# clinfo/kGCN

Hardware: AMD Instinct MI355X
Metric: graphs/sec GraphConv fwd+bwd, 32-node mol graphs x64 feat (higher is better)
Workload: dtype f32

## Files before the change

include/kgcn_hip.h:

```cpp
#ifndef KGCN_HIP_H_
#define KGCN_HIP_H_

#include <stdint.h>

#ifdef __cplusplus
extern "C" {
#endif

#define KGCN_HIP_ABI_VERSION 2

#define KGCN_PAD_COL 32

#define KGCN_ROW_PAD_COMPACT 0x104
#define KGCN_CSR_UNIT_VALUES 1


typedef struct kgcn_csr_batch {
  int32_t num_graphs;
  int32_t rows;
  int32_t cols;
  int32_t max_nnz_per_graph;
  int32_t row_pad;
  int32_t reserved_;
  int64_t nnz;
// ... 72 lines not shown
                        int64_t workspace_bytes, void* stream);

int kgcn_graph_maxpool_fwd_f32(const kgcn_csr_batch* a, const float* x, int32_t d, float* out,
                               float beta, void* stream);
int64_t kgcn_graph_maxpool_bwd_workspace_bytes(int32_t num_graphs, int32_t rows, int32_t d);
int kgcn_graph_maxpool_bwd_f32(const kgcn_csr_batch* a, const kgcn_csr_batch* at, const float* x,
                               const float* dout_grad, int32_t d, float* dx, float beta,
                               void* workspace, int64_t workspace_bytes, void* stream);

int64_t kgcn_gat_workspace_bytes(int32_t num_graphs, int32_t n_nodes, int32_t d);
int kgcn_gat_fwd_f32(const kgcn_csr_batch* a, const float* x, int32_t d, const float* weight_a, float* out,
                     float beta, void* workspace, int64_t workspace_bytes, void* stream);
int kgcn_gat_bwd_f32(const kgcn_csr_batch* a, const kgcn_csr_batch* at, const float* x, int32_t d,
                     const float* weight_a, const float* dout_grad, float* dx, float beta, float* dweight_a,
                     void* workspace, int64_t workspace_bytes, void* stream);

int64_t kgcn_gram_workspace_bytes(int32_t d);
int kgcn_gram_fwd_f32(const float* x, int32_t num_graphs, int32_t n_nodes, int32_t d, const float* w, float* out,
                      void* stream);
int kgcn_gram_bwd_f32(const float* x, int32_t num_graphs, int32_t n_nodes, int32_t d, const float* w,
                      const float* dout_grad, float* dx, float beta, float* dw, void* workspace,
                      int64_t workspace_bytes, void* stream);

int kgcn_graph_gather_fwd_f32(const float* x, int64_t batch, int32_t n_nodes, int32_t d,
                              float* out, void* stream);
int kgcn_graph_gather_fwd_ld_f32(const float* x, int64_t batch, int32_t n_nodes, int32_t d, float* out, int64_t out_ld,
                                 void* stream);
int kgcn_graph_gather_bwd_f32(const float* dout_grad, int64_t batch, int32_t n_nodes, int32_t d,
                              float* dx, void* stream);

int kgcn_graph_gather_bwd_add_f32(const float* dout_grad, const float* dx_in, int64_t batch, int32_t n_nodes, int32_t d,
                                  float* dx, void* stream);

int64_t kgcn_dot_workspace_bytes(int64_t n);
int kgcn_dot_f32(const float* a, const float* b, int64_t n, float* out, void* workspace,
                 int64_t workspace_bytes, void* stream);

#define KGCN_ACT_NONE 0
#define KGCN_ACT_SIGMOID 1
#define KGCN_ACT_RELU 2
#define KGCN_ACT_TANH 3
int kgcn_bconv_act_f32(const kgcn_csr_batch* a_ch, int32_t num_channels, const float* rhs, int64_t rhs_ld,
                       int64_t rhs_graph_stride, int64_t rhs_channel_stride, int32_t d, float* out, int64_t out_ld,
                       int64_t out_graph_stride, int32_t act, void* stream);

int kgcn_bconv_fanout_f32(const kgcn_csr_batch* at_ch, int32_t num_channels, const float* grad, const float* act_out, int64_t ld,
                          int64_t graph_stride, int32_t d, int32_t act, float* out, int64_t out_ld, int64_t out_graph_stride,
                          int64_t out_channel_stride, void* stream);
int kgcn_bspmm_dact_f32(const kgcn_csr_batch* a, const float* grad, const float* act_out, int64_t ld,
                        int64_t graph_stride, int32_t d, int32_t act, float* out, int64_t out_ld,
                        int64_t out_graph_stride, float beta, void* stream);
int kgcn_dense_fwd_act_f32(const float* x, int64_t m, int32_t din, int64_t x_ld, const float* w, int64_t w_ld,
                           int32_t trans_w, const float* bias, float* y, int32_t dout, int64_t y_ld, int32_t act,
                           void* stream);
int64_t kgcn_dense_fwd_workspace_bytes(int32_t din, int32_t dout);
int kgcn_dense_fwd_ws_f32(const float* x, int64_t m, int32_t din, int64_t x_ld, const float* w, int64_t w_ld,
                          int32_t trans_w, const float* bias, float* y, int32_t dout, int64_t y_ld, int32_t act,
                          void* workspace, int64_t workspace_bytes, void* stream);
#define KGCN_WTABLE_MAX_JOBS 16
typedef struct kgcn_wtable_job {
  const float* w;
  int64_t w_ld;
  int32_t trans_w, k, n;
  int32_t k_w;
  void* table;
  const float* extra_row;
} kgcn_wtable_job;
int kgcn_wtable_split_multi(const kgcn_wtable_job* jobs, int32_t num_jobs, void* stream);
int kgcn_dense_fwd_tab_f32(const float* x, int64_t m, int32_t din, int64_t x_ld, const float* w, int64_t w_ld,
                           int32_t trans_w, const float* bias, float* y, int32_t dout, int64_t y_ld, int32_t act,
                           const void* table, int64_t table_bytes, void* stream);
int kgcn_dense_dx_dact_f32(const float* grad, const float* act_out, int64_t m, int32_t dout, int64_t ld, const float* w,
                           int64_t w_ld, int32_t din, float* dx, int64_t dx_ld, int32_t act, float* dpre,
                           void* workspace, int64_t workspace_bytes, void* stream);
int kgcn_dense_dx_dact_tab_f32(const float* grad, const float* act_out, int64_t m, int32_t dout, int64_t ld, const float* w,
                               int64_t w_ld, int32_t din, float* dx, int64_t dx_ld, int32_t act, float* dpre, const void* table,
                               int64_t table_bytes, void* stream);
int kgcn_dense_dx_dact_gather_supported(int64_t m, int32_t din, int32_t dout);
int kgcn_dense_dx_dact_gather_f32(const float* grad, const float* pooled_grad, int64_t pooled_ld, int32_t n_nodes,
                                  const float* act_out, int64_t m, int32_t dout, int64_t ld, const float* w, int64_t w_ld,
                                  int32_t din, float* dx, int64_t dx_ld, int32_t act, float* dpre, void* table,
                                  int64_t table_bytes, int32_t table_ready, void* stream);
int kgcn_dense_bwd_supported(int64_t m, int32_t din, int32_t dout);
int kgcn_dense_bwd_f32(const float* grad, const float* pooled_grad, int64_t pooled_ld, int32_t n_nodes, const float* act_out,
                       int32_t act, int64_t ld, const float* x, int64_t x_ld, int64_t m, int32_t din, int32_t dout,
                       const float* w, int64_t w_ld, float* dx, int64_t dx_ld, float* dw, float* dbias, void* table,
                       int64_t table_bytes, int32_t table_ready, void* workspace, int64_t workspace_bytes, void* stream);
int kgcn_dense_bwd_dot_f32(const float* grad, const float* act_out, int32_t act, int64_t ld, const float* x, int64_t x_ld, int64_t m,
                           int32_t din, int32_t dout, const float* w, int64_t w_ld, const float* dotx, int64_t dotx_ld, float* dw,
                           float* dbias, float* dot_out, void* table, int64_t table_bytes, int32_t table_ready, void* workspace,
                           int64_t workspace_bytes, void* stream);
int kgcn_dense_dx_dact_dot_supported(int64_t m, int32_t din, int32_t dout);
int64_t kgcn_dense_dx_dact_dot_workspace_bytes(int64_t m, int32_t din);
int kgcn_dense_dx_dact_dot_f32(const float* grad, const float* act_out, int64_t m, int32_t dout, int64_t ld, const float* w,
                               int64_t w_ld, int32_t din, const float* dotx, int64_t dotx_ld, int32_t act, float* dpre,
                               void* table, int64_t table_bytes, int32_t table_ready, float* dot_out, void* workspace,
                               int64_t workspace_bytes, void* stream);
int kgcn_act_fwd_f32(const float* x, int64_t n, int32_t act, float* y, void* stream);
int kgcn_act_bwd_f32(const float* act_out, const float* grad, int64_t n, int32_t act, float* dpre, void* stream);

int64_t kgcn_graph_bn_workspace_bytes(int32_t d);
int kgcn_graph_bn_stats_f32(const float* x, int64_t graphs, int32_t n_nodes, int32_t d, const int32_t* enabled,
                            float* mean, float* var, void* workspace, int64_t workspace_bytes, void* stream);
int kgcn_graph_bn_apply_f32(const float* x, int64_t graphs, int32_t n_nodes, int32_t d, const int32_t* enabled,
                            const float* mean, const float* var, const float* gamma, const float* beta, float eps,
                            float* y, void* stream);
int kgcn_graph_bn_bwd_f32(const float* x, const float* grad, int64_t graphs, int32_t n_nodes, int32_t d,
                          const int32_t* enabled, const float* mean, const float* var, const float* gamma, float eps,
                          int32_t training, float* dx, float* dgamma, float* dbeta, void* workspace,
                          int64_t workspace_bytes, void* stream);

int kgcn_graph_bn_apply_act_f32(const float* x, int64_t graphs, int32_t n_nodes, int32_t d, const int32_t* enabled,
                                const float* mean, const float* var, const float* gamma, const float* beta, float eps,
                                int32_t act, float* y, void* stream);
int kgcn_graph_bn_bwd_dact_f32(const float* x, const float* grad, const float* act_out, int32_t act, int64_t graphs,
                               int32_t n_nodes, int32_t d, const int32_t* enabled, const float* mean, const float* var,
                               const float* gamma, float eps, int32_t training, float* dx, float* dgamma, float* dbeta,
                               void* workspace, int64_t workspace_bytes, void* stream);

int64_t kgcn_coo_pack_workspace_bytes(int64_t nnz, int32_t num_graphs, int32_t rows, int32_t cols);
int kgcn_coo_pack_f32(const int32_t* graph, const int32_t* row, const int32_t* col, const float* val, int64_t nnz,
                      int32_t num_graphs, int32_t rows, int32_t cols, int32_t transposed, int32_t* rowptr_out,
                      void* cv_out, int32_t* perm_out, int32_t* stats_out, void* workspace, int64_t workspace_bytes,
                      void* stream);
int64_t kgcn_csr_pad4_workspace_bytes(int32_t num_graphs, int32_t rows);
int kgcn_csr_pad4(const kgcn_csr_batch* a, int32_t* rowptr4_out, void* cv4_out, int64_t cv4_capacity,
                  int32_t* slots_out, int32_t* graph_ptr_out, int32_t* stats_out, void* workspace,
                  int64_t workspace_bytes, void* stream);
int64_t kgcn_compact_values_offset(int64_t nnz);
int64_t kgcn_compact_cv_words(int64_t nnz, int32_t with_values);
int kgcn_csr_compact4(const kgcn_csr_batch* a4, void* cv_out, int with_values, void* slots_out, int32_t* stats_out,
                      void* stream);
int kgcn_graphconv_fused_reads_compact(int32_t backward, int32_t num_graphs, int32_t n_nodes, int32_t din, int32_t dout,
                                       int32_t max_nnz_per_graph, int32_t with_dx);

int64_t kgcn_ragged_workspace_bytes(int32_t num_sel);
int kgcn_ragged_plan(const kgcn_csr_batch* src, const int32_t* sizes, const int32_t* sel, int32_t num_sel,
                     int32_t* graph_ptr, int32_t* entry_ptr, void* workspace, int64_t workspace_bytes, void* stream);
int kgcn_ragged_compact_csr(const kgcn_csr_batch* src, const int32_t* sel, int32_t num_sel, const int32_t* graph_ptr,
                            const int32_t* entry_ptr, int32_t capacity_rows, int32_t* dst_rowptr, int32_t* dst_cv,
                            int64_t dst_cv_capacity, int32_t* status, void* stream);
int kgcn_ragged_compact_csr_pair(const kgcn_csr_batch* src, const kgcn_csr_batch* src_t, const int32_t* sel, int32_t num_sel,
                                 const int32_t* graph_ptr, const int32_t* entry_ptr, int32_t capacity_rows, int32_t* dst_rowptr,
                                 int32_t* dst_cv, int64_t dst_cv_capacity, int32_t* dst_t_rowptr, int32_t* dst_t_cv,
                                 int64_t dst_t_cv_capacity, int32_t* status, void* stream);
#define KGCN_RAGGED_BLOCK_ROWS 32
int32_t kgcn_ragged_block_rows(void);
int32_t kgcn_ragged_num_blocks(int32_t capacity_rows);
int kgcn_ragged_blocks(const int32_t* graph_ptr, int32_t num_sel, int32_t capacity_rows, int32_t* block_ptr, void* stream);
int kgcn_ragged_compact_rows_f32(const float* src, const int32_t* sel, int32_t num_sel, int32_t n_nodes, int32_t d,
                                 const int32_t* graph_ptr, int32_t capacity_rows, float* dst, void* stream);
int kgcn_ragged_compact_rows_aug_f32(const float* src, const int32_t* sel, int32_t num_sel, int32_t n_nodes, int32_t d,
                                     const int32_t* graph_ptr, int32_t capacity_rows, float* dst, int32_t dst_ld, void* stream);
int kgcn_ragged_expand_rows_f32(const float* src, int32_t num_graphs, int32_t n_nodes, int32_t d,
                                const int32_t* graph_ptr, int32_t fill_row, float* dst, void* stream);
int kgcn_ragged_gather_fwd_f32(const float* x, const int32_t* graph_ptr, int64_t batch, int32_t n_nodes, int32_t d,
                               int32_t pad_row, float* out, void* stream);
int64_t kgcn_ragged_gather_bwd_workspace_bytes(int32_t d);
int kgcn_ragged_gather_bwd_f32(const float* dout_grad, const int32_t* graph_ptr, int64_t batch, int32_t n_nodes, int32_t d,
                               int32_t pad_row, int32_t capacity_rows, float* dx, void* workspace, int64_t workspace_bytes,
                               void* stream);

int64_t kgcn_loss_workspace_bytes(int64_t batch);
int kgcn_masked_sigmoid_ce_f32(const float* logits, const float* labels, const float* mask, const float* mask_label,
                               int64_t batch, int32_t tasks, int32_t weighted, float pos_weight,
                               const float* pos_weight_per_task, float* cost, float* dlogits, float* sums, void* workspace,
                               int64_t workspace_bytes, void* stream);
int kgcn_masked_softmax_ce_f32(const float* logits, const float* labels, const float* mask, int64_t batch, int32_t classes,
                               float* cost, float* dlogits, float* sums, void* workspace, int64_t workspace_bytes,
                               void* stream);
int kgcn_sparse_softmax_ce_f32(const float* logits, const int64_t* label_idx, const float* mask, int64_t batch,
                               int32_t classes, float* cost, float* dlogits, float* sums, void* workspace,
                               int64_t workspace_bytes, void* stream);
int kgcn_loss_grad_f32(const float* dlogits, const float* g_opt, const float* g_sum, int64_t batch, int64_t n, float* out,
                       void* stream);
int kgcn_adam_tf_f32(float* params, const float* grads, float* m, float* v, int64_t n, float lr, float beta1, float beta2,
                     float eps, int64_t* step_counter, void* stream);
#define KGCN_ADAM_MAX_SEGMENTS 32
typedef struct kgcn_adam_segment {
  const float* grad;
  int64_t offset, numel;
} kgcn_adam_segment;
int kgcn_adam_tf_multi_f32(float* params, float* m, float* v, int64_t n, const kgcn_adam_segment* segments, int32_t num_segments,
                           float lr, float beta1, float beta2, float eps, int64_t* step_counter, void* stream);

int kgcn_augment_ones_f32(const float* x, int64_t m, int32_t din, int64_t x_ld, float* out, int64_t out_ld, void* stream);
int kgcn_augment_ones_bwd_f32(const float* dout_grad, int64_t m, int32_t din, int64_t g_ld, float* dx, int64_t dx_ld,
                              void* stream);

#define KGCN_STACK_MAX_LAYERS 8
typedef struct kgcn_stack_layer {
  int32_t kind, act, din, dout;
  const float* w;
  const float* b;
  const float* mean;
  const float* var;
  float eps;
  int32_t route;
} kgcn_stack_layer;
int kgcn_gcn_stack_supported(int32_t n_nodes, int32_t max_nnz_per_graph, const kgcn_stack_layer* layers, int32_t num_layers);
int64_t kgcn_gcn_stack_param_floats(const kgcn_stack_layer* layers, int32_t num_layers);
int kgcn_gcn_stack_fwd_f32(const kgcn_csr_batch* a, const float* x, const int32_t* enabled, const kgcn_stack_layer* layers,
                           int32_t num_layers, float* const* layer_out, float* pooled, void* stream);
int64_t kgcn_gcn_stack_bwd_workspace_bytes(int32_t num_graphs, const kgcn_stack_layer* layers, int32_t num_layers);
int kgcn_gcn_stack_bwd_f32(const kgcn_csr_batch* at, const float* x, const int32_t* enabled, const kgcn_stack_layer* layers,
                           int32_t num_layers, float* const* layer_out, const float* dlast, int32_t gather, float* dx,
                           float* dparams, void* workspace, int64_t workspace_bytes, void* stream);

int kgcn_reduce_defer(int32_t on);
int kgcn_reduce_pending(void);
int kgcn_reduce_flush(void* stream);

int kgcn_dense_mfma_products(int32_t kind, int64_t m, int32_t din, int32_t dout);

enum {
  KGCN_SPMM_NONE = 0,
  KGCN_SPMM_TILE = 1,
  KGCN_SPMM_TILE_DOT = 2,
  KGCN_SPMM_SLICES = 3,
  KGCN_SPMM_BLOCK = 4,
  KGCN_SPMM_ROWS = 5,
  KGCN_SPMM_GATHER = 6,
  KGCN_SPMM_BCONV_LOOP = 7,
  KGCN_SPMM_BCONV_FANOUT = 8
};
#define KGCN_SPMM_DACT 1
#define KGCN_SPMM_SELF_SCALE 2
#define KGCN_SPMM_DOT 4
#define KGCN_SPMM_FANOUT 8
typedef struct kgcn_spmm_route {
  int32_t kernel;
  int32_t template_args[4];
  int32_t ds, slices;
  int32_t workgroup;
  int64_t grid;
  int64_t lds_bytes;
} kgcn_spmm_route;
int kgcn_spmm_route_query(const kgcn_csr_batch* a_ch, int32_t num_channels, int32_t d, int64_t rhs_ld, int64_t rhs_graph_stride,
                          int64_t channel_stride, int64_t out_ld, int64_t out_graph_stride, int32_t align_bytes, int32_t flags,
                          kgcn_spmm_route* route);

#define KGCN_COPY2D_MAX_JOBS 16
typedef struct kgcn_copy2d_job {
  const float* src;
  float* dst;
  int64_t rows, cols, src_ld, dst_ld;
} kgcn_copy2d_job;
int kgcn_copy2d_multi_f32(const kgcn_copy2d_job* jobs, int32_t num_jobs, void* stream);

int kgcn_hbm_probe(int32_t mix, const void* a, const void* a2, void* b, int64_t bytes, void* stream);

int kgcn_dense_wgrad_dact_supported(int32_t din, int32_t dout);
int kgcn_dense_wgrad_dact_f32(const float* x, int64_t x_ld, const float* dy, const float* act_out, int64_t dy_ld, int32_t act,
                              int64_t m, int32_t din, int32_t dout, float* dw, float* dbias, void* workspace,
                              int64_t workspace_bytes, void* stream);

int64_t kgcn_gin_aggregate_bwd_workspace_bytes(int32_t num_graphs, int32_t n_nodes, int32_t d);
int kgcn_gin_aggregate_bwd_f32(const kgcn_csr_batch* at_ch, int32_t num_channels, const float* grad, int32_t d,
                               const float* eps, const float* x, float* dx, float* deps, void* workspace,
                               int64_t workspace_bytes, void* stream);

#define KGCN_VAE_MAX_NODES 128
#define KGCN_VAE_MAX_CHANNELS 8
#define KGCN_VAE_MAX_DIM 64
int kgcn_philox4x64_raw(uint64_t seed, const int64_t* step, int64_t num_blocks, uint64_t* out, void* stream);
int kgcn_normal_f32(uint64_t seed, const int64_t* step, int64_t n, float* out, void* stream);
int kgcn_vae_sample_fwd_f32(const float* m_pre, const float* s_pre, int32_t num_graphs, int32_t n_nodes, int32_t d, int32_t ld,
                            const float* eps, uint64_t seed, const int64_t* step, float* z, float* kl, void* stream);
int kgcn_vae_sample_bwd_f32(const float* m_pre, const float* s_pre, int32_t num_graphs, int32_t n_nodes, int32_t d, int32_t ld,
                            const float* eps, uint64_t seed, const int64_t* step, const float* const* dz, int32_t num_dz,
                            const float* dkl, float* dm_pre, float* ds_pre, void* stream);
int64_t kgcn_vae_recon_workspace_bytes(int32_t num_graphs, int32_t num_channels, int32_t d);
int kgcn_vae_recon_fwd_f32(const kgcn_csr_batch* adj_ch, int32_t num_channels, const float* const* y, const float* const* w,
                           int32_t d, const float* feat_logits, const float* feat_target, int32_t f, const float* mask,
                           const float* kl, float* per_graph, float* sums, void* stream);
int kgcn_vae_recon_bwd_f32(const kgcn_csr_batch* adj_ch, int32_t num_channels, const float* const* y, const float* const* w,
                           int32_t d, const float* feat_logits, const float* feat_target, int32_t f, const float* mask,
                           const float* g_opt, const float* g_sum, float* const* dy, float* const* dw, float* dfeat,
                           float* dkl, void* workspace, int64_t workspace_bytes, void* stream);

#define KGCN_SEQ_MAX_EMBED 32
#define KGCN_SEQ_MAX_FILTERS 64
#define KGCN_SEQ_MAX_KERNEL 8
#define KGCN_SEQ_MAX_POOL 8
#define KGCN_SEQ_MAX_UNITS 64
#define KGCN_SEQ_MAX_LSTM_INPUT 64
#define KGCN_SEQ_MAX_SYMBOLS 1024
#define KGCN_SEQ_MAX_LENGTH 8192
#define KGCN_SEQ_ACT_HARD_SIGMOID 0
#define KGCN_SEQ_ACT_SIGMOID 1
int64_t kgcn_seq_convpool_workspace_bytes(int32_t batch, int32_t length, int32_t symbols, int32_t embed_dim, int32_t kernel_size,
                                          int32_t filters, int32_t pool);
int kgcn_seq_convpool_fwd_f32(const int32_t* tokens, int32_t batch, int32_t length, const float* table, int32_t symbols,
                              int32_t embed_dim, const float* w, const float* bias, int32_t kernel_size, int32_t filters,
// ... 100 lines not shown
```

kgcn_amd/_lib.py:

```python
import ctypes
import os

_HERE = os.path.dirname(os.path.abspath(__file__))
DEV_ENV_VARS = ("KGCN_HIP_LIB", "KGCN_GIN_JOIN", "KGCN_GIN_DOT")
LIB_PATH = os.environ.get("KGCN_HIP_LIB") or os.path.join(_HERE, "csrc", "libkgcn_hip.so")


def active_overrides():
    return {k: os.environ[k] for k in DEV_ENV_VARS if os.environ.get(k)}


if active_overrides():
    import warnings
    warnings.warn("kgcn_amd: development overrides active: %r (KGCN_HIP_LIB swaps the native library, the others "
                  "change kernel routing)" % (active_overrides(),), RuntimeWarning, stacklevel=2)

c_f32p = ctypes.c_void_p
c_i32p = ctypes.c_void_p
c_i64 = ctypes.c_int64
c_i32 = ctypes.c_int32


ABI_VERSION = 2

# ... 117 lines not shown
    "kgcn_gram_fwd_f32": (ctypes.c_int, [c_f32p, c_i32, c_i32, c_i32, c_f32p, c_f32p, ctypes.c_void_p]),
    "kgcn_gram_bwd_f32": (ctypes.c_int, [c_f32p, c_i32, c_i32, c_i32, c_f32p, c_f32p, c_f32p, ctypes.c_float, c_f32p,
                                         ctypes.c_void_p, c_i64, ctypes.c_void_p]),
    "kgcn_graph_gather_fwd_f32": (ctypes.c_int, [c_f32p, c_i64, c_i32, c_i32, c_f32p,
                                                 ctypes.c_void_p]),
    "kgcn_graph_gather_fwd_ld_f32": (ctypes.c_int, [c_f32p, c_i64, c_i32, c_i32, c_f32p, c_i64, ctypes.c_void_p]),
    "kgcn_graph_gather_bwd_f32": (ctypes.c_int, [c_f32p, c_i64, c_i32, c_i32, c_f32p,
                                                 ctypes.c_void_p]),
    "kgcn_bconv_fanout_f32": (ctypes.c_int, [_CSRP, c_i32, c_f32p, c_f32p, c_i64, c_i64, c_i32, c_i32, c_f32p, c_i64, c_i64, c_i64,
                                             ctypes.c_void_p]),
    "kgcn_bconv_act_f32": (ctypes.c_int, [_CSRP, c_i32, c_f32p, c_i64, c_i64, c_i64, c_i32, c_f32p, c_i64, c_i64, c_i32,
                                          ctypes.c_void_p]),
    "kgcn_bspmm_dact_f32": (ctypes.c_int, [_CSRP, c_f32p, c_f32p, c_i64, c_i64, c_i32, c_i32, c_f32p, c_i64, c_i64,
                                           ctypes.c_float, ctypes.c_void_p]),
    "kgcn_dense_fwd_act_f32": (ctypes.c_int, [c_f32p, c_i64, c_i32, c_i64, c_f32p, c_i64, c_i32, c_f32p, c_f32p, c_i32,
                                              c_i64, c_i32, ctypes.c_void_p]),
    "kgcn_dense_fwd_workspace_bytes": (c_i64, [c_i32, c_i32]),
    "kgcn_dense_fwd_ws_f32": (ctypes.c_int, [c_f32p, c_i64, c_i32, c_i64, c_f32p, c_i64, c_i32, c_f32p, c_f32p, c_i32,
                                             c_i64, c_i32, ctypes.c_void_p, c_i64, ctypes.c_void_p]),
    "kgcn_dense_dx_dact_f32": (ctypes.c_int, [c_f32p, c_f32p, c_i64, c_i32, c_i64, c_f32p, c_i64, c_i32, c_f32p, c_i64, c_i32,
                                              c_f32p, ctypes.c_void_p, c_i64, ctypes.c_void_p]),
    "kgcn_dense_dx_dact_tab_f32": (ctypes.c_int, [c_f32p, c_f32p, c_i64, c_i32, c_i64, c_f32p, c_i64, c_i32, c_f32p, c_i64,
                                                  c_i32, c_f32p, ctypes.c_void_p, c_i64, ctypes.c_void_p]),
    "kgcn_dense_dx_dact_gather_supported": (ctypes.c_int, [c_i64, c_i32, c_i32]),
    "kgcn_dense_dx_dact_gather_f32": (ctypes.c_int, [c_f32p, c_f32p, c_i64, c_i32, c_f32p, c_i64, c_i32, c_i64, c_f32p, c_i64, c_i32,
                                                     c_f32p, c_i64, c_i32, c_f32p, ctypes.c_void_p, c_i64, c_i32, ctypes.c_void_p]),
    "kgcn_dense_dx_dact_dot_supported": (ctypes.c_int, [c_i64, c_i32, c_i32]),
    "kgcn_dense_dx_dact_dot_workspace_bytes": (c_i64, [c_i64, c_i32]),
    "kgcn_dense_dx_dact_dot_f32": (ctypes.c_int, [c_f32p, c_f32p, c_i64, c_i32, c_i64, c_f32p, c_i64, c_i32, c_f32p, c_i64, c_i32,
                                                  c_f32p, ctypes.c_void_p, c_i64, c_i32, c_f32p, ctypes.c_void_p, c_i64,
                                                  ctypes.c_void_p]),
    "kgcn_dense_fwd_tab_f32": (ctypes.c_int, [c_f32p, c_i64, c_i32, c_i64, c_f32p, c_i64, c_i32, c_f32p, c_f32p, c_i32,
                                              c_i64, c_i32, ctypes.c_void_p, c_i64, ctypes.c_void_p]),
    "kgcn_wtable_split_multi": (ctypes.c_int, [ctypes.c_void_p, c_i32, ctypes.c_void_p]),
    "kgcn_act_fwd_f32": (ctypes.c_int, [c_f32p, c_i64, c_i32, c_f32p, ctypes.c_void_p]),
    "kgcn_act_bwd_f32": (ctypes.c_int, [c_f32p, c_f32p, c_i64, c_i32, c_f32p, ctypes.c_void_p]),
    "kgcn_graph_bn_workspace_bytes": (c_i64, [c_i32]),
    "kgcn_graph_bn_stats_f32": (ctypes.c_int, [c_f32p, c_i64, c_i32, c_i32, c_i32p, c_f32p, c_f32p, ctypes.c_void_p, c_i64,
                                               ctypes.c_void_p]),
    "kgcn_graph_bn_apply_f32": (ctypes.c_int, [c_f32p, c_i64, c_i32, c_i32, c_i32p, c_f32p, c_f32p, c_f32p, c_f32p,
                                               ctypes.c_float, c_f32p, ctypes.c_void_p]),
    "kgcn_graph_bn_bwd_f32": (ctypes.c_int, [c_f32p, c_f32p, c_i64, c_i32, c_i32, c_i32p, c_f32p, c_f32p, c_f32p,
                                             ctypes.c_float, c_i32, c_f32p, c_f32p, c_f32p, ctypes.c_void_p, c_i64,
                                             ctypes.c_void_p]),
    "kgcn_coo_pack_workspace_bytes": (c_i64, [c_i64, c_i32, c_i32, c_i32]),
    "kgcn_coo_pack_f32": (ctypes.c_int, [c_i32p, c_i32p, c_i32p, c_f32p, c_i64, c_i32, c_i32, c_i32, c_i32, c_i32p,
                                         ctypes.c_void_p, c_i32p, c_i32p, ctypes.c_void_p, c_i64, ctypes.c_void_p]),
    "kgcn_compact_values_offset": (c_i64, [c_i64]),
    "kgcn_compact_cv_words": (c_i64, [c_i64, c_i32]),
    "kgcn_csr_compact4": (ctypes.c_int, [_CSRP, ctypes.c_void_p, ctypes.c_int, ctypes.c_void_p, c_i32p, ctypes.c_void_p]),
    "kgcn_graphconv_fused_reads_compact": (ctypes.c_int, [c_i32, c_i32, c_i32, c_i32, c_i32, c_i32, c_i32]),
    "kgcn_csr_pad4_workspace_bytes": (c_i64, [c_i32, c_i32]),
    "kgcn_csr_pad4": (ctypes.c_int, [_CSRP, c_i32p, ctypes.c_void_p, c_i64, c_i32p, c_i32p, c_i32p, ctypes.c_void_p,
                                     c_i64, ctypes.c_void_p]),
    "kgcn_graph_bn_apply_act_f32": (ctypes.c_int, [c_f32p, c_i64, c_i32, c_i32, c_i32p, c_f32p, c_f32p, c_f32p, c_f32p,
                                                   ctypes.c_float, c_i32, c_f32p, ctypes.c_void_p]),
    "kgcn_graph_bn_bwd_dact_f32": (ctypes.c_int, [c_f32p, c_f32p, c_f32p, c_i32, c_i64, c_i32, c_i32, c_i32p, c_f32p, c_f32p,
                                                  c_f32p, ctypes.c_float, c_i32, c_f32p, c_f32p, c_f32p, ctypes.c_void_p,
                                                  c_i64, ctypes.c_void_p]),
    "kgcn_ragged_workspace_bytes": (c_i64, [c_i32]),
    "kgcn_ragged_plan": (ctypes.c_int, [_CSRP, c_i32p, c_i32p, c_i32, c_i32p, c_i32p, ctypes.c_void_p, c_i64,
                                        ctypes.c_void_p]),
    "kgcn_ragged_compact_csr": (ctypes.c_int, [_CSRP, c_i32p, c_i32, c_i32p, c_i32p, c_i32, c_i32p, c_i32p, c_i64, c_i32p,
                                               ctypes.c_void_p]),
    "kgcn_ragged_compact_csr_pair": (ctypes.c_int, [_CSRP, _CSRP, c_i32p, c_i32, c_i32p, c_i32p, c_i32, c_i32p, c_i32p, c_i64, c_i32p,
                                                    c_i32p, c_i64, c_i32p, ctypes.c_void_p]),
    "kgcn_ragged_block_rows": (c_i32, []),
    "kgcn_ragged_num_blocks": (c_i32, [c_i32]),
    "kgcn_ragged_blocks": (ctypes.c_int, [c_i32p, c_i32, c_i32, c_i32p, ctypes.c_void_p]),
    "kgcn_ragged_compact_rows_f32": (ctypes.c_int, [c_f32p, c_i32p, c_i32, c_i32, c_i32, c_i32p, c_i32, c_f32p,
                                                    ctypes.c_void_p]),
    "kgcn_ragged_compact_rows_aug_f32": (ctypes.c_int, [c_f32p, c_i32p, c_i32, c_i32, c_i32, c_i32p, c_i32, c_f32p, c_i32,
                                                        ctypes.c_void_p]),
    "kgcn_ragged_expand_rows_f32": (ctypes.c_int, [c_f32p, c_i32, c_i32, c_i32, c_i32p, c_i32, c_f32p, ctypes.c_void_p]),
    "kgcn_ragged_gather_fwd_f32": (ctypes.c_int, [c_f32p, c_i32p, c_i64, c_i32, c_i32, c_i32, c_f32p, ctypes.c_void_p]),
    "kgcn_ragged_gather_bwd_workspace_bytes": (c_i64, [c_i32]),
    "kgcn_ragged_gather_bwd_f32": (ctypes.c_int, [c_f32p, c_i32p, c_i64, c_i32, c_i32, c_i32, c_i32, c_f32p,
                                                  ctypes.c_void_p, c_i64, ctypes.c_void_p]),
    "kgcn_dense_mfma_products": (ctypes.c_int, [c_i32, c_i64, c_i32, c_i32]),
    "kgcn_spmm_route_query": (ctypes.c_int, [_CSRP, c_i32, c_i32, c_i64, c_i64, c_i64, c_i64, c_i64, c_i32, c_i32,
                                             ctypes.POINTER(SpmmRoute)]),
    "kgcn_copy2d_multi_f32": (ctypes.c_int, [ctypes.c_void_p, c_i32, ctypes.c_void_p]),
    "kgcn_hbm_probe": (ctypes.c_int, [c_i32, ctypes.c_void_p, ctypes.c_void_p, ctypes.c_void_p, c_i64, ctypes.c_void_p]),
    "kgcn_reduce_defer": (ctypes.c_int, [c_i32]),
    "kgcn_reduce_pending": (ctypes.c_int, []),
    "kgcn_reduce_flush": (ctypes.c_int, [ctypes.c_void_p]),
    "kgcn_loss_workspace_bytes": (c_i64, [c_i64]),
    "kgcn_masked_sigmoid_ce_f32": (ctypes.c_int, [c_f32p, c_f32p, c_f32p, c_f32p, c_i64, c_i32, c_i32, ctypes.c_float, c_f32p,
                                                  c_f32p, c_f32p, c_f32p, ctypes.c_void_p, c_i64, ctypes.c_void_p]),
    "kgcn_masked_softmax_ce_f32": (ctypes.c_int, [c_f32p, c_f32p, c_f32p, c_i64, c_i32, c_f32p, c_f32p, c_f32p,
                                                  ctypes.c_void_p, c_i64, ctypes.c_void_p]),
    "kgcn_sparse_softmax_ce_f32": (ctypes.c_int, [c_f32p, ctypes.c_void_p, c_f32p, c_i64, c_i32, c_f32p, c_f32p, c_f32p,
                                                  ctypes.c_void_p, c_i64, ctypes.c_void_p]),
    "kgcn_adam_tf_multi_f32": (ctypes.c_int, [c_f32p, c_f32p, c_f32p, c_i64, ctypes.c_void_p, c_i32, ctypes.c_float,
                                              ctypes.c_float, ctypes.c_float, ctypes.c_float, ctypes.c_void_p, ctypes.c_void_p]),
    "kgcn_loss_grad_f32": (ctypes.c_int, [c_f32p, c_f32p, c_f32p, c_i64, c_i64, c_f32p, ctypes.c_void_p]),
    "kgcn_adam_tf_f32": (ctypes.c_int, [c_f32p, c_f32p, c_f32p, c_f32p, c_i64, ctypes.c_float, ctypes.c_float,
                                        ctypes.c_float, ctypes.c_float, ctypes.c_void_p, ctypes.c_void_p]),
    "kgcn_augment_ones_f32": (ctypes.c_int, [c_f32p, c_i64, c_i32, c_i64, c_f32p, c_i64, ctypes.c_void_p]),
    "kgcn_augment_ones_bwd_f32": (ctypes.c_int, [c_f32p, c_i64, c_i32, c_i64, c_f32p, c_i64, ctypes.c_void_p]),
    "kgcn_gcn_stack_supported": (ctypes.c_int, [c_i32, c_i32, _STKP, c_i32]),
    "kgcn_gcn_stack_param_floats": (c_i64, [_STKP, c_i32]),
    "kgcn_gcn_stack_fwd_f32": (ctypes.c_int, [_CSRP, c_f32p, c_i32p, _STKP, c_i32, _PTRP, c_f32p, ctypes.c_void_p]),
    "kgcn_gcn_stack_bwd_workspace_bytes": (c_i64, [c_i32, _STKP, c_i32]),
    "kgcn_gcn_stack_bwd_f32": (ctypes.c_int, [_CSRP, c_f32p, c_i32p, _STKP, c_i32, _PTRP, c_f32p, c_i32, c_f32p, c_f32p,
                                              ctypes.c_void_p, c_i64, ctypes.c_void_p]),
    "kgcn_dense_wgrad_dact_supported": (ctypes.c_int, [c_i32, c_i32]),
    "kgcn_dense_wgrad_dact_f32": (ctypes.c_int, [c_f32p, c_i64, c_f32p, c_f32p, c_i64, c_i32, c_i64, c_i32, c_i32, c_f32p,
                                                 c_f32p, ctypes.c_void_p, c_i64, ctypes.c_void_p]),
    "kgcn_gin_aggregate_bwd_workspace_bytes": (c_i64, [c_i32, c_i32, c_i32]),
    "kgcn_gin_aggregate_bwd_f32": (ctypes.c_int, [_CSRP, c_i32, c_f32p, c_i32, c_f32p, c_f32p, c_f32p, c_f32p, ctypes.c_void_p,
                                                  c_i64, ctypes.c_void_p]),
    "kgcn_philox4x64_raw": (ctypes.c_int, [ctypes.c_uint64, ctypes.c_void_p, c_i64, ctypes.c_void_p, ctypes.c_void_p]),
    "kgcn_normal_f32": (ctypes.c_int, [ctypes.c_uint64, ctypes.c_void_p, c_i64, c_f32p, ctypes.c_void_p]),
    "kgcn_vae_sample_fwd_f32": (ctypes.c_int, [c_f32p, c_f32p, c_i32, c_i32, c_i32, c_i32, c_f32p, ctypes.c_uint64, ctypes.c_void_p,
                                               c_f32p, c_f32p, ctypes.c_void_p]),
    "kgcn_vae_sample_bwd_f32": (ctypes.c_int, [c_f32p, c_f32p, c_i32, c_i32, c_i32, c_i32, c_f32p, ctypes.c_uint64, ctypes.c_void_p,
                                               _PTRP, c_i32, c_f32p, c_f32p, c_f32p, ctypes.c_void_p]),
    "kgcn_vae_recon_workspace_bytes": (c_i64, [c_i32, c_i32, c_i32]),
    "kgcn_vae_recon_fwd_f32": (ctypes.c_int, [_CSRP, c_i32, _PTRP, _PTRP, c_i32, c_f32p, c_f32p, c_i32, c_f32p, c_f32p, c_f32p,
                                              c_f32p, ctypes.c_void_p]),
    "kgcn_vae_recon_bwd_f32": (ctypes.c_int, [_CSRP, c_i32, _PTRP, _PTRP, c_i32, c_f32p, c_f32p, c_i32, c_f32p, c_f32p, c_f32p,
                                              _PTRP, _PTRP, c_f32p, c_f32p, ctypes.c_void_p, c_i64, ctypes.c_void_p]),
    "kgcn_seq_convpool_workspace_bytes": (c_i64, [c_i32, c_i32, c_i32, c_i32, c_i32, c_i32, c_i32]),
    "kgcn_seq_convpool_fwd_f32": (ctypes.c_int, [ctypes.c_void_p, c_i32, c_i32, c_f32p, c_i32, c_i32, c_f32p, c_f32p, c_i32, c_i32,
                                                 c_i32, c_f32p, ctypes.c_void_p, ctypes.c_void_p]),
    "kgcn_seq_convpool_bwd_f32": (ctypes.c_int, [ctypes.c_void_p, c_i32, c_i32, c_f32p, c_i32, c_i32, c_f32p, c_i32, c_i32, c_i32,
                                                 c_f32p, ctypes.c_void_p, c_f32p, c_f32p, c_f32p, ctypes.c_void_p, c_i64,
                                                 ctypes.c_void_p]),
    "kgcn_seq_convpool_scaled_fwd_f32": (ctypes.c_int, [ctypes.c_void_p, c_i32, c_i32, c_f32p, c_i32, c_f32p, c_i32, c_i32, c_f32p,
                                                        c_f32p, c_i32, c_i32, c_i32, c_f32p, ctypes.c_void_p, ctypes.c_void_p]),
    "kgcn_seq_convpool_perturbed_fwd_f32": (ctypes.c_int, [ctypes.c_void_p, c_i32, c_i32, c_f32p, c_f32p, c_i32p, c_i32p, ctypes.c_uint64,
                                                           c_i32, c_f32p, c_i32, c_i32, c_f32p, c_f32p, c_i32, c_i32, c_i32, c_f32p,
                                                           ctypes.c_void_p, ctypes.c_void_p]),
    "kgcn_ig_perturb_rows_f32": (ctypes.c_int, [c_f32p, c_i64, c_i32, c_i32, c_i32, c_f32p, c_f32p, c_i32p, c_i32p, ctypes.c_uint32,
                                                ctypes.c_uint64, c_f32p, ctypes.c_void_p]),
    "kgcn_ig_perturb_values_f32": (ctypes.c_int, [c_i32p, c_i32, c_i32, c_i64, c_i32, c_f32p, c_f32p, c_f32p, c_i32p, c_i32p,
                                                  ctypes.c_uint32, ctypes.c_uint64, c_f32p, ctypes.c_void_p]),
    "kgcn_seq_convpool_input_grad_f32": (ctypes.c_int, [ctypes.c_void_p, c_i32, c_i32, c_i32, c_f32p, c_i32, c_i32, c_f32p, c_i32,
                                                        c_i32, c_i32, c_f32p, ctypes.c_void_p, c_f32p, c_i32, c_f32p,
                                                        ctypes.c_void_p]),
    "kgcn_seq_lstm_stash_floats": (c_i64, [c_i32, c_i32, c_i32]),
    "kgcn_seq_lstm_workspace_bytes": (c_i64, [c_i32, c_i32, c_i32, c_i32]),
    "kgcn_seq_lstm_fwd_f32": (ctypes.c_int, [c_f32p, c_i32, c_i32, c_i32, c_f32p, c_f32p, c_f32p, c_i32, c_i32, c_f32p, c_i64, c_f32p,
                                             ctypes.c_void_p]),
    "kgcn_seq_lstm_bwd_f32": (ctypes.c_int, [c_f32p, c_i32, c_i32, c_i32, c_f32p, c_f32p, c_f32p, c_i32, c_i32, c_f32p, c_i64, c_f32p,
                                             c_f32p, c_f32p, c_f32p, c_f32p, ctypes.c_void_p, c_i64, ctypes.c_void_p]),
    "kgcn_conv1d_pool_workspace_bytes": (c_i64, [c_i32, c_i32, c_i32, c_i32, c_i32, c_i32]),
    "kgcn_conv1d_pool_fwd_f32": (ctypes.c_int, [c_f32p, c_i32p, c_f32p, c_i32, c_i32, c_i32, c_i32, c_f32p, c_f32p, c_i32, c_i32,
                                                c_i32, c_i32, c_f32p, ctypes.c_void_p, ctypes.c_void_p]),
    "kgcn_conv1d_pool_bwd_f32": (ctypes.c_int, [c_f32p, c_i32p, c_f32p, c_i32, c_i32, c_i32, c_i32, c_f32p, c_i32, c_i32, c_i32,
                                                c_i32, c_f32p, ctypes.c_void_p, c_f32p, c_f32p, c_f32p, c_f32p, ctypes.c_void_p,
                                                c_i64, ctypes.c_void_p]),
    "kgcn_embedding_grad_f32": (ctypes.c_int, [c_i32p, c_i32, c_i32, c_f32p, c_i32, c_i32, c_f32p, ctypes.c_void_p]),
    "kgcn_linkpred_workspace_bytes": (c_i64, [c_i64, c_i32, c_i32, c_i32, c_i32]),
    "kgcn_linkpred_fwd_f32": (ctypes.c_int, [c_f32p, c_i64, c_i32, c_f32p, c_i32, c_i32, c_i32p, c_i32p, c_i64, c_i32, c_i32p, c_i32,
                                             ctypes.c_uint64, ctypes.c_void_p, c_i32p, c_f32p, c_f32p, c_f32p, ctypes.c_void_p]),
    "kgcn_linkpred_bwd_f32": (ctypes.c_int, [c_f32p, c_i64, c_i32, c_f32p, c_i32, c_i32, c_i32p, c_f32p, c_f32p, c_f32p, c_i32,
                                             c_f32p, c_f32p, c_f32p, c_f32p, ctypes.c_void_p, c_i64, ctypes.c_void_p]),
    "kgcn_kg_ig_f32": (ctypes.c_int, [c_i32p, c_i32p, c_f32p, c_i64, c_i32, c_i32, c_f32p, c_f32p, c_f32p, c_f32p, c_f32p, c_f32p,
                                      c_f32p, c_f32p, c_i32, c_i32p, c_i32, c_i32, c_i32, c_f32p, c_f32p, c_f32p, ctypes.c_void_p]),
    "kgcn_pair_rank_workspace_bytes": (c_i64, [c_i32, c_i32, c_i64, c_i64]),
    "kgcn_pair_rank_select_f32": (ctypes.c_int, [c_f32p, c_i32, c_i32, c_f32p, c_i64, ctypes.c_void_p, ctypes.c_void_p, c_i64,
                                                 ctypes.c_void_p]),
    "kgcn_pair_rank_emit_f32": (ctypes.c_int, [c_f32p, c_i32, c_i32, c_f32p, c_i64, ctypes.c_void_p, c_i64, c_f32p, c_i32p, c_i32p,
                                               ctypes.c_void_p, c_i64, ctypes.c_void_p]),
    "kgcn_pair_rank_table_i32": (ctypes.c_int, [c_f32p, c_i32p, c_i32p, c_i64, ctypes.c_void_p, c_i64, ctypes.c_void_p, c_i64,
                                                ctypes.POINTER(c_i64), c_i32, ctypes.c_void_p, ctypes.c_void_p, ctypes.c_void_p,
                                                ctypes.c_void_p, ctypes.c_void_p, ctypes.c_void_p, ctypes.c_void_p, c_i64,
                                                ctypes.c_void_p]),
    "kgcn_graph_gather_bwd_ld_f32": (ctypes.c_int, [c_f32p, c_i64, c_i64, c_i32, c_i32, c_f32p, ctypes.c_void_p]),
    "kgcn_graph_gather_bwd_add_f32": (ctypes.c_int, [c_f32p, c_f32p, c_i64, c_i32, c_i32, c_f32p, ctypes.c_void_p]),
    "kgcn_dot_workspace_bytes": (c_i64, [c_i64]),
    "kgcn_dot_f32": (ctypes.c_int, [c_f32p, c_f32p, c_i64, c_f32p, ctypes.c_void_p, c_i64,
                                    ctypes.c_void_p]),
}


# ... 63 lines not shown
```

kgcn_amd/csrc/dense.hip:

```cpp
#include <atomic>
#include <mutex>

#include "dense_kernels.h"

namespace kgcn {

constexpr int BM = 128;
constexpr int BN = 64;
constexpr int BK = 32;
constexpr int XS_LD = BK + 4;

__global__ __launch_bounds__(256) void dense_fwd_kernel(
    const float* __restrict__ x, long m, int din, long x_ld, const float* __restrict__ w,
    long w_ld, int trans_w, const float* __restrict__ bias, float* __restrict__ y, int dout,
    long y_ld, int act) {
  __shared__ __attribute__((aligned(16))) float Xs[BM * XS_LD];
  __shared__ __attribute__((aligned(16))) float Ws[BK * BN];

  const int tid = threadIdx.x;
  const int wave = tid >> 6, lane = tid & 63;
  const int li = lane & 31, hi = lane >> 5;
  const long m0 = (long)blockIdx.x * BM;
  const int n0 = blockIdx.y * BN;
  const bool x_vec = ((din & 3) == 0) && ((x_ld & 3) == 0) &&
// ... 252 lines not shown
  const long nwaves = (long)gridDim.x * P_WAVES;
  long tile = (long)blockIdx.x * P_WAVES + wave;
  if (tile < ntiles) {
    XChunk<VEC> fx, fg;
    issue_xchunk<VEC>(fx, x, m, din, x_ld, tile * 32, i0, lane);
    issue_xchunk<VEC>(fg, dy, m, dout, dy_ld, tile * 32, j0, lane);
    for (;;) {
      land_xchunk<VEC>(fx, xs, 64, lane);
      land_xchunk<VEC>(fg, gs, 64, lane);
      lds_handoff();
      const long tn = tile + nwaves;
      const bool more = tn < ntiles;
      issue_xchunk<VEC>(fx, x, m, din, x_ld, (more ? tn : tile) * 32, i0, lane);
      issue_xchunk<VEC>(fg, dy, m, dout, dy_ld, (more ? tn : tile) * 32, j0, lane);
#pragma unroll 4
      for (int s = 0; s < 16; ++s) {
        const int n = hi * 16 + s;
        const float a0 = xs[n * 64 + li], a1 = xs[n * 64 + 32 + li];
        const float f0 = gs[n * 64 + li], f1 = gs[n * 64 + 32 + li];
        d00 = __builtin_amdgcn_mfma_f32_32x32x2f32(a0, f0, d00, 0, 0, 0);
        d01 = __builtin_amdgcn_mfma_f32_32x32x2f32(a0, f1, d01, 0, 0, 0);
        d10 = __builtin_amdgcn_mfma_f32_32x32x2f32(a1, f0, d10, 0, 0, 0);
        d11 = __builtin_amdgcn_mfma_f32_32x32x2f32(a1, f1, d11, 0, 0, 0);
        cs0 += f0;
        cs1 += f1;
      }
      lds_handoff();
      if (!more) break;
      tile = tn;
    }
  }
  __syncthreads();
  float* park = reinterpret_cast<float*>(dsm) + (size_t)wave * (64 * 64 + 64);
#pragma unroll
  for (int r = 0; r < 16; ++r) {
    const int row = (r & 3) + 8 * (r >> 2) + 4 * hi;
    park[row * 64 + li] = d00[r];
    park[row * 64 + 32 + li] = d01[r];
    park[(32 + row) * 64 + li] = d10[r];
    park[(32 + row) * 64 + 32 + li] = d11[r];
  }
  cs0 += __shfl_xor(cs0, 32, 64);
  cs1 += __shfl_xor(cs1, 32, 64);
  if (hi == 0) { park[64 * 64 + li] = cs0; park[64 * 64 + 32 + li] = cs1; }
  __syncthreads();
  const float* base = reinterpret_cast<const float*>(dsm);
  float* pw = part_dw + (long)blockIdx.x * din * dout;
  for (int i = tid; i < 64 * 64; i += blockDim.x) {
    float sum = 0.f;
#pragma unroll
    for (int wv = 0; wv < P_WAVES; ++wv) sum += base[(size_t)wv * (64 * 64 + 64) + i];
    const int row = i0 + (i >> 6), col = j0 + (i & 63);
    if (row < din && col < dout) pw[(long)row * dout + col] = sum;
  }
  if (part_db && blockIdx.y == 0 && tid < 64) {
    float sum = 0.f;
#pragma unroll
    for (int wv = 0; wv < P_WAVES; ++wv) sum += base[(size_t)wv * (64 * 64 + 64) + 64 * 64 + tid];
    if (j0 + tid < dout) part_db[(long)blockIdx.x * dout + j0 + tid] = sum;
  }
}

static int persist_blocks(long m) {
  long tiles = (m + 31) / 32;
  long b = (tiles + P_WAVES - 1) / P_WAVES;
  if (b > kNumCU) b = kNumCU;
  return b < 1 ? 1 : (int)b;
}

int launch_reduce_partials(const float* part, int nparts, long n, float* out, hipStream_t s) {
  hipLaunchKernelGGL(reduce_partials_kernel, dim3((unsigned)((n + 31) / 32)), dim3(256), 0, s,
                     part, nparts, n, out, nullptr, 0L, nullptr);
  return check_launch("reduce_partials_kernel");
}

constexpr int kMaxReduceJobs = 24;
struct ReduceJobs {
  const float* part[kMaxReduceJobs];
  float* out[kMaxReduceJobs];
  long n[kMaxReduceJobs];
  int nparts[kMaxReduceJobs];
  int block0[kMaxReduceJobs + 1];
  int njobs;
};

__global__ __launch_bounds__(256) void reduce_partials_multi_kernel(ReduceJobs jb) {
  __shared__ float red[8][33];
  int j = 0;
  while (j + 1 < jb.njobs && (int)blockIdx.x >= jb.block0[j + 1]) ++j;
  const float* __restrict__ src = jb.part[j];
  const long nn = jb.n[j];
  const int nparts = jb.nparts[j];
  const int oi = threadIdx.x & 31, pg = threadIdx.x >> 5;
  const long o = (long)((int)blockIdx.x - jb.block0[j]) * 32 + oi;
  float s[8];
#pragma unroll
  for (int u = 0; u < 8; ++u) s[u] = 0.f;
  if (o < nn) {
    int p = pg;
    for (; p + 56 < nparts; p += 64) {
#pragma unroll
      for (int u = 0; u < 8; ++u) s[u] += src[(long)(p + 8 * u) * nn + o];
    }
    for (; p < nparts; p += 8) s[0] += src[(long)p * nn + o];
  }
  red[pg][oi] = ((s[0] + s[1]) + (s[2] + s[3])) + ((s[4] + s[5]) + (s[6] + s[7]));
  __syncthreads();
  if (pg == 0 && o < nn) {
    float t = 0.f;
#pragma unroll
    for (int q = 0; q < 8; ++q) t += red[q][oi];
    jb.out[j][o] = t;
  }
}

struct PendingReduce { const float* part; int nparts; long n; float* out; };
static std::atomic<bool> g_defer_reduce{false};
static std::mutex g_pending_mutex;
static PendingReduce g_pending[256];
static int g_npending = 0;

static int flush_pending_locked(hipStream_t s) {
  int done = 0;
  while (done < g_npending) {
    ReduceJobs jb{};
    int blocks = 0, nj = 0;
    for (; nj < kMaxReduceJobs && done + nj < g_npending; ++nj) {
      const PendingReduce& p = g_pending[done + nj];
      jb.part[nj] = p.part; jb.out[nj] = p.out; jb.n[nj] = p.n; jb.nparts[nj] = p.nparts; jb.block0[nj] = blocks;
      blocks += (int)((p.n + 31) / 32);
    }
    jb.block0[nj] = blocks;
    jb.njobs = nj;
    if (blocks > 0) {
      hipLaunchKernelGGL(reduce_partials_multi_kernel, dim3((unsigned)blocks), dim3(256), 0, s, jb);
      if (int rc = check_launch("reduce_partials_multi_kernel")) { g_npending = 0; return rc; }
    }
    done += nj;
  }
  g_npending = 0;
  return 0;
}

int reduce_or_defer(const float* part, int nparts, long n, float* out, hipStream_t s) {
  if (!g_defer_reduce.load()) return launch_reduce_partials(part, nparts, n, out, s);
  std::lock_guard<std::mutex> lock(g_pending_mutex);
  if (g_npending == 256)
    if (int rc = flush_pending_locked(s)) return rc;
  g_pending[g_npending++] = PendingReduce{part, nparts, n, out};
  return 0;
}

}

using namespace kgcn;

extern "C" int kgcn_reduce_defer(int32_t on) { return g_defer_reduce.exchange(on != 0) ? 1 : 0; }
extern "C" int kgcn_reduce_pending(void) { return g_npending; }
extern "C" int kgcn_reduce_flush(void* stream) {
  std::lock_guard<std::mutex> lock(g_pending_mutex);
  return flush_pending_locked(as_stream(stream));
}

struct RowFacts { bool a16; long a_ld; bool b16; long b_ld; };
static RowFacts aligned_rows(int din, int dout) { return RowFacts{true, (long)((din + 3) & ~3), true, (long)dout}; }
constexpr long kManyRows = 1L << 20;

enum class FwdRoute {
  SkinnyN, SkinnyK,
  Gemmh,
  Gemm3Table, Gemm3,
  Gemmn,
  Narrow,
  Persist, Tiled
};

static bool wide_layer(int din, int dout) { return dout > 128 && din >= 32; }
static size_t persist_fwd_lds(int din) { return (size_t)((din + 63) / 64) * 64 * 64 * 4 + (size_t)P_WAVES * PT_FLOATS * 4; }

static FwdRoute fwd_route(long m, int din, int dout, int trans_w, const RowFacts& f, bool have_table) {
  if (skinny_n_ok(din, dout, trans_w)) return FwdRoute::SkinnyN;
  if (skinny_k_ok(din, dout)) return FwdRoute::SkinnyK;
  const bool table = have_table && m >= 1024;
  if (wide_layer(din, dout)) {
    if (!table) return FwdRoute::Gemm3;
    return gemmh_fwd_ok(f.a16, m, din, f.a_ld, dout) ? FwdRoute::Gemmh : FwdRoute::Gemm3Table;
  }
  if (table && gemmn_pays(f.a16, din, f.a_ld, dout)) return FwdRoute::Gemmn;
  if (narrow_fwd_ok(f.a16, din, f.a_ld, f.b16, dout, f.b_ld)) return FwdRoute::Narrow;
  return persist_fwd_lds(din) <= (size_t)kLdsBytes ? FwdRoute::Persist : FwdRoute::Tiled;
}
static bool wide_table_route(FwdRoute r) { return r == FwdRoute::Gemmh || r == FwdRoute::Gemm3Table; }
static bool reads_table(FwdRoute r) { return wide_table_route(r) || r == FwdRoute::Gemmn; }

static int launch_fwd_persist(const float* x, long m, int din, long x_ld, const float* w, long w_ld, int trans_w,
                              const float* bias, float* y, int dout, long y_ld, int act, hipStream_t s) {
  const int kp = ((din + 63) / 64) * 64;
  const size_t lds = persist_fwd_lds(din);
  const bool vec = (din % 4 == 0) && (x_ld % 4 == 0) && aligned16(x);
  if (int rc = allow_full_lds<dense_fwd_persist_kernel<true>>(lds, "dense_fwd_persist_kernel")) return rc;
  if (int rc = allow_full_lds<dense_fwd_persist_kernel<false>>(lds, "dense_fwd_persist_kernel")) return rc;
  int blocks = persist_blocks(m);
  if (2 * lds <= (size_t)kLdsBytes && blocks == kNumCU) blocks = 2 * kNumCU;
  dim3 grid((unsigned)blocks, (unsigned)((dout + 63) / 64));
  hipLaunchKernelGGL(vec ? dense_fwd_persist_kernel<true> : dense_fwd_persist_kernel<false>, grid, dim3(64 * P_WAVES), lds, s, x,
                     m, din, x_ld, w, w_ld, trans_w, bias, y, dout, y_ld, kp, act);
  return check_launch("dense_fwd_persist_kernel");
}

static int dense_fwd_impl(const float* x, int64_t m, int32_t din, int64_t x_ld, const float* w, int64_t w_ld,
                          int32_t trans_w, const float* bias, float* y, int32_t dout, int64_t y_ld, int act,
                          void* workspace, int64_t workspace_bytes, void* stream, bool table_ready = false) {
  if (act < KGCN_ACT_NONE || act > KGCN_ACT_TANH) return fail("kgcn_dense_fwd_f32: unknown activation code %d", act);
  if (m < 0 || din <= 0 || dout <= 0)
    return fail("kgcn_dense_fwd_f32: bad shape m=%lld din=%d dout=%d", (long long)m, din, dout);
  if (m == 0) return 0;
  if (!x || !w || !y) return fail("kgcn_dense_fwd_f32: NULL operand");
  if (x_ld < din || y_ld < dout) return fail("kgcn_dense_fwd_f32: leading dimension too small");
  if (w_ld < (trans_w ? din : dout)) return fail("kgcn_dense_fwd_f32: w_ld too small");
  hipStream_t s = as_stream(stream);
  const FwdRoute route = fwd_route((long)m, din, dout, trans_w, RowFacts{aligned16(x), (long)x_ld, aligned16(y), (long)y_ld},
                                   workspace && workspace_bytes >= wtable_bytes(din, dout));
  if (reads_table(route) && !table_ready) launch_wtable_split(w, (long)w_ld, trans_w, din, dout, workspace, s);
  switch (route) {
    case FwdRoute::SkinnyN:
      return launch_skinny_n_fwd(x, (long)m, din, (long)x_ld, w, (long)w_ld, bias, y, dout, (long)y_ld, act, s);
    case FwdRoute::SkinnyK:
      return launch_skinny_k_fwd(x, (long)m, din, (long)x_ld, w, (long)w_ld, trans_w, bias, y, dout, (long)y_ld, act, s);
    case FwdRoute::Gemmh:
      return launch_gemmh_fwd(x, (long)m, din, (long)x_ld, static_cast<const char*>(workspace) + wtable_bf16_bytes(din, dout),
                              bias, y, dout, (long)y_ld, act, s);
    case FwdRoute::Gemm3Table:
    case FwdRoute::Gemm3:
      return launch_gemm3_fwd(x, (long)m, din, (long)x_ld, w, (long)w_ld, trans_w, bias, y, dout, (long)y_ld, act,
                              route == FwdRoute::Gemm3Table ? workspace : nullptr, s);
    case FwdRoute::Gemmn:
      return launch_gemmn_fwd(x, (long)m, din, (long)x_ld, workspace, bias, y, dout, (long)y_ld, act, s);
    case FwdRoute::Narrow:
      return launch_narrow_fwd(x, (long)m, din, w, (long)w_ld, trans_w, bias, y, dout, act, s);
    case FwdRoute::Persist:
      return launch_fwd_persist(x, (long)m, din, (long)x_ld, w, (long)w_ld, trans_w, bias, y, dout, (long)y_ld, act, s);
    case FwdRoute::Tiled: break;
  }
  const long gx = (m + BM - 1) / BM;
// ... 270 lines not shown
  const RowFacts f = aligned_rows(din, dout);
  if (kind == 0 || kind == 1) {
    switch (fwd_route((long)m, din, dout, kind, f, true)) {
      case FwdRoute::SkinnyN: case FwdRoute::SkinnyK: return kind == 0 ? 0 : 1;
      case FwdRoute::Gemmh: return 3;
      case FwdRoute::Gemm3Table: case FwdRoute::Gemm3: case FwdRoute::Gemmn: return 6;
      case FwdRoute::Narrow: case FwdRoute::Persist: case FwdRoute::Tiled: return 1;
    }
  }
  switch (wgrad_route((long)m, din, dout, false, f).route) {
    case WgradRoute::Skinny: return 0;
    case WgradRoute::Gemmh: return 3;
    case WgradRoute::Wgradx: case WgradRoute::Gemm3: case WgradRoute::Wgradn: return 6;
    case WgradRoute::Narrow: case WgradRoute::Persist: return 1;
  }
  return 1;
}

extern "C" int64_t kgcn_dense_wgrad_workspace_bytes(int64_t m, int32_t din, int32_t dout) {
  if (m <= 0 || din <= 0 || dout <= 0) return 0;
  const long target = (long)kNumCU * 4;
  long rpc = (((m + target - 1) / target + 31) / 32) * 32;
  if (rpc < 32) rpc = 32;
  int nchunks = (int)((m + rpc - 1) / rpc);
  if (nchunks < kNumCU) nchunks = kNumCU;
  if (wgrad_route((long)m, din, dout, false, aligned_rows(din, dout)).route == WgradRoute::Skinny && nchunks < 4 * kNumCU)
    nchunks = 4 * kNumCU;
  return (int64_t)nchunks * ((int64_t)din * dout + dout) * 4;
}

static int launch_wgrad_persist(const float* x, long x_ld, const float* dy, long dy_ld, long m, int din, int dout,
                                float* part_dw, float* part_db, int nblocks, hipStream_t s) {
  const size_t lds = (size_t)P_WAVES * (64 * 64 + 64) * 4;
  if (int rc = allow_full_lds<dense_wgrad_persist_kernel<true>>(lds, "dense_wgrad_persist_kernel")) return rc;
  if (int rc = allow_full_lds<dense_wgrad_persist_kernel<false>>(lds, "dense_wgrad_persist_kernel")) return rc;
  const bool vec = (din % 4 == 0) && (dout % 4 == 0) && (x_ld % 4 == 0) && (dy_ld % 4 == 0) && aligned16(x) && aligned16(dy);
  dim3 grid((unsigned)nblocks, (unsigned)((din + 63) / 64), (unsigned)((dout + 63) / 64));
  hipLaunchKernelGGL(vec ? dense_wgrad_persist_kernel<true> : dense_wgrad_persist_kernel<false>, grid, dim3(64 * P_WAVES), lds, s,
                     x, x_ld, dy, dy_ld, m, din, dout, part_dw, part_db);
  return check_launch("dense_wgrad_persist_kernel");
}

static int dense_wgrad_impl(const float* x, int64_t x_ld, const float* dy, int64_t dy_ld, int64_t m, int32_t din,
                            int32_t dout, float* dw, float* dbias, void* workspace, int64_t workspace_bytes, void* stream,
                            const float* yact, int act) {
  if (m < 0 || din <= 0 || dout <= 0)
    return fail("kgcn_dense_wgrad_f32: bad shape m=%lld din=%d dout=%d", (long long)m, din, dout);
  if (!dw && !dbias) return 0;
  hipStream_t s = as_stream(stream);
  if (m == 0) {
    if (dw) (void)hipMemsetAsync(dw, 0, (size_t)din * dout * 4, s);
    if (dbias) (void)hipMemsetAsync(dbias, 0, (size_t)dout * 4, s);
    return 0;
  }
  if (!x || !dy) return fail("kgcn_dense_wgrad_f32: NULL operand");
  const int64_t need = kgcn_dense_wgrad_workspace_bytes(m, din, dout);
  if (!workspace || workspace_bytes < need)
    return fail("kgcn_dense_wgrad_f32: workspace %lld < %lld bytes", (long long)workspace_bytes, (long long)need);
  const long M = (long)m, xl = (long)x_ld, gl = (long)dy_ld;
  const WgradPlan plan = wgrad_route(M, din, dout, yact != nullptr, RowFacts{aligned16(x), xl, aligned16(dy), gl});
  const int np = plan.nparts;
  float* part_dw = static_cast<float*>(workspace);
  float* part_db = part_dw + (long)np * din * dout;
  int rc = 0;
  switch (plan.route) {
    case WgradRoute::Skinny: rc = launch_skinny_n_wgrad(x, M, din, xl, dy, gl, dout, part_dw, part_db, np, s); break;
    case WgradRoute::Wgradx: rc = launch_wgradx(x, xl, dy, gl, M, din, dout, part_dw, part_db, np, s, yact, act); break;
    case WgradRoute::Gemmh: rc = launch_gemmh_wgrad(x, xl, dy, gl, M, din, dout, part_dw, part_db, np, s, yact, act); break;
    case WgradRoute::Gemm3: rc = launch_gemm3_wgrad(x, xl, dy, gl, M, din, dout, part_dw, part_db, np, s, yact, act); break;
    case WgradRoute::Wgradn: rc = launch_wgradn(x, xl, dy, gl, M, din, dout, part_dw, part_db, np, s); break;
    case WgradRoute::Narrow: rc = launch_narrow_wgrad(x, dy, M, din, dout, part_dw, part_db, np, s); break;
    case WgradRoute::Persist: rc = launch_wgrad_persist(x, xl, dy, gl, M, din, dout, part_dw, part_db, np, s); break;
  }
  return rc ? rc : launch_reduce_pair(part_dw, (long)din * dout, dw, part_db, dout, dbias, np, s);
}

extern "C" int kgcn_dense_wgrad_f32(const float* x, int64_t x_ld, const float* dy, int64_t dy_ld,
                                    int64_t m, int32_t din, int32_t dout, float* dw, float* dbias,
                                    void* workspace, int64_t workspace_bytes, void* stream) {
  return dense_wgrad_impl(x, x_ld, dy, dy_ld, m, din, dout, dw, dbias, workspace, workspace_bytes, stream, nullptr,
                          KGCN_ACT_NONE);
}

extern "C" int kgcn_dense_wgrad_dact_supported(int32_t din, int32_t dout) {
  return fuses_dact(wgrad_route(kManyRows, din, dout, true, aligned_rows(din, dout)).route) ? 1 : 0;
}

extern "C" int kgcn_dense_wgrad_dact_f32(const float* x, int64_t x_ld, const float* dy, const float* act_out, int64_t dy_ld,
                                         int32_t act, int64_t m, int32_t din, int32_t dout, float* dw, float* dbias,
                                         void* workspace, int64_t workspace_bytes, void* stream) {
  if (act <= KGCN_ACT_NONE || act > KGCN_ACT_TANH) return fail("kgcn_dense_wgrad_dact_f32: activation code %d", act);
  if (!kgcn_dense_wgrad_dact_supported(din, dout))
    return fail("kgcn_dense_wgrad_dact_f32: shape %d x %d is not a wide layer (run kgcn_act_bwd_f32 + kgcn_dense_wgrad_f32)",
                din, dout);
  if (m > 0 && !act_out) return fail("kgcn_dense_wgrad_dact_f32: act_out is NULL");
  return dense_wgrad_impl(x, x_ld, dy, dy_ld, m, din, dout, dw, dbias, workspace, workspace_bytes, stream, act_out, act);
}
```

kgcn_amd/csrc/dense_kernels.h:

```cpp
#pragma once

#include "kgcn_common.h"

namespace kgcn {

int64_t wtable_bf16_bytes(int din, int dout);
int64_t wtable_bytes(int din, int dout);
void launch_wtable_split(const float* w, long w_ld, int trans_w, int din, int dout, void* workspace, hipStream_t s);

int launch_gemm3_fwd(const float* x, long m, int din, long x_ld, const float* w, long w_ld, int trans_w, const float* bias,
                     float* y, int dout, long y_ld, int act, const void* table, hipStream_t s);
int launch_gemm3_dx_dact(const float* grad, const float* act_out, float* dpre, long m, int k, long ld, const void* table,
                         float* dx, int n, long dx_ld, int dact, hipStream_t s, const float* pooled_grad = nullptr,
                         int n_nodes = 0, long pooled_ld = 0);
int launch_gemm3_wgrad(const float* x, long x_ld, const float* dy, long dy_ld, long m, int din, int dout, float* part_dw,
                       float* part_db, int nblocks, hipStream_t s, const float* yact = nullptr, int act = KGCN_ACT_NONE);

bool gemmh_fwd_ok(bool x16, long m, int din, long x_ld, int dout);
int launch_gemmh_fwd(const float* x, long m, int din, long x_ld, const void* tabh, const float* bias, float* y, int dout,
                     long y_ld, int act, hipStream_t s);
int launch_gemmh_dx_dact(const float* grad, const float* act_out, float* dpre, long m, int k, long ld, const void* tabh,
                         float* dx, int n, long dx_ld, int dact, hipStream_t s, const float* pooled_grad, int n_nodes,
                         long pooled_ld, float* dot_part);
int gemmh_dot_parts(long m, int dout);
bool gemmh_wgrad_ok(int din, int dout, long m);
int launch_gemmh_wgrad(const float* x, long x_ld, const float* dy, long dy_ld, long m, int din, int dout, float* part_dw,
                       float* part_db, int nblocks, hipStream_t s, const float* yact, int act);

int launch_gemmb(const float* grad, const float* act_out, long m, int din, int dout, long ld, const float* x, long x_ld,
                 const void* tabh, float* dx, long dx_ld, float* part_dw, float* part_db, int dact, const float* pooled_grad,
                 int n_nodes, long pooled_ld, hipStream_t s, float* dot_part);

bool gemmn_pays(bool x16, int din, long x_ld, int dout);
int launch_gemmn_fwd(const float* x, long m, int din, long x_ld, const void* table, const float* bias, float* y, int dout,
                     long y_ld, int act, hipStream_t s);
bool wgradn_ok(bool x16, int din, long x_ld, int dout);
int launch_wgradn(const float* x, long x_ld, const float* dy, long dy_ld, long m, int din, int dout, float* part_dw,
                  float* part_db, int nblocks, hipStream_t s);

bool wgradx_ok(int din, int dout);
int launch_wgradx(const float* x, long x_ld, const float* dy, long dy_ld, long m, int din, int dout, float* part_dw,
                  float* part_db, int nparts, hipStream_t s, const float* yact, int act);

bool narrow_fwd_ok(bool x16, int din, long x_ld, bool y16, int dout, long y_ld);
int launch_narrow_fwd(const float* x, long m, int din, const float* w, long w_ld, int trans_w, const float* bias, float* y,
                      int dout, int act, hipStream_t s);
bool narrow_wgrad_ok(bool x16, int din, long x_ld, bool dy16, int dout, long dy_ld);
int launch_narrow_wgrad(const float* x, const float* dy, long m, int din, int dout, float* part_dw, float* part_db,
                        int nblocks, hipStream_t s);

bool skinny_n_ok(int din, int dout, int trans_w);
bool skinny_k_ok(int din, int dout);
int launch_skinny_n_fwd(const float* x, long m, int din, long x_ld, const float* w, long w_ld, const float* bias, float* y,
                        int dout, long y_ld, int act, hipStream_t s);
int launch_skinny_k_fwd(const float* x, long m, int din, long x_ld, const float* w, long w_ld, int trans_w, const float* bias,
                        float* y, int dout, long y_ld, int act, hipStream_t s);
int skinny_wgrad_parts(long m);
int launch_skinny_n_wgrad(const float* x, long m, int din, long x_ld, const float* g, long g_ld, int dout, float* part_dw,
                          float* part_db, int nparts, hipStream_t s);

}
```

kgcn_amd/csrc/pack.hip:

```cpp
#include "kgcn_common.h"

namespace kgcn {

constexpr int kScanBlock = 256;

__device__ __forceinline__ int graph_entries(const int* __restrict__ src_rowptr, int g, int M, int dummy_cnt) {
  return g < 0 ? dummy_cnt : src_rowptr[(long)(g + 1) * M] - src_rowptr[(long)g * M];
}

__device__ __forceinline__ int block_exclusive_scan(int v, int* total) {
  __shared__ int wave_tot[kScanBlock / kWave];
  const int lane = threadIdx.x & (kWave - 1), wave = threadIdx.x / kWave;
  int inc = v;
#pragma unroll
  for (int o = 1; o < kWave; o <<= 1) {
    int up = __shfl_up(inc, o, kWave);
    if (lane >= o) inc += up;
  }
  if (lane == kWave - 1) wave_tot[wave] = inc;
  __syncthreads();
  int base = 0, tot = 0;
#pragma unroll
  for (int w = 0; w < kScanBlock / kWave; ++w) {
    const int t = wave_tot[w];
// ... 41 lines not shown
  for (long t = wave0; t < T; t += nwaves) {
    const int g = sel[t];
    const int out_base = graph_ptr[t] + block_sums[t / kScanBlock];
    int* rp_out = dst_rowptr + t * M;
    int cnt;
    if (g >= 0) {
      const int* rp_in = src_rowptr + (long)g * M;
      const int src_base = rp_in[0];
      cnt = rp_in[M] - src_base;
      for (int r = lane; r < M; r += kWave) rp_out[r] = rp_in[r] - src_base + out_base;
      const int2* in = src_cv + src_base;
      int2* out = dst_cv + out_base;
      for (int i = lane; i < cnt; i += kWave) out[i] = in[i];
      if (row_pad) {
        const int* sl = src_slots + (long)g * M;
        for (int r = lane; r < M; r += kWave) dst_slots[t * M + r] = sl[r];
      }
    } else if (row_pad) {
      cnt = 4 * M;
      for (int r = lane; r < M; r += kWave) {
        rp_out[r] = out_base + 4 * r;
        dst_slots[t * M + r] = (4 * r) | (4 << 16) | (r << 24);
      }
      int2* out = dst_cv + out_base;
      for (int i = lane; i < cnt; i += kWave) out[i] = make_int2(KGCN_PAD_COL, 0);
    } else {
      cnt = 0;
      for (int r = lane; r < M; r += kWave) rp_out[r] = out_base;
    }
    if (lane == 0) {
      graph_ptr[t] = out_base;
      if (t == T - 1) dst_rowptr[(long)T * M] = out_base + cnt;
    }
  }
}


struct AssemblePlan {
  int num_csr, num_tables, nb;
  const int* src_rowptr[KGCN_ASSEMBLE_MAX_CSR];
  const int2* src_cv[KGCN_ASSEMBLE_MAX_CSR];
  const int* src_slots[KGCN_ASSEMBLE_MAX_CSR];
  int M[KGCN_ASSEMBLE_MAX_CSR], row_pad[KGCN_ASSEMBLE_MAX_CSR];
  int* graph_ptr[KGCN_ASSEMBLE_MAX_CSR];
  int* dst_rowptr[KGCN_ASSEMBLE_MAX_CSR];
  int2* dst_cv[KGCN_ASSEMBLE_MAX_CSR];
  int* dst_slots[KGCN_ASSEMBLE_MAX_CSR];
  const float* table[KGCN_ASSEMBLE_MAX_TABLES];
  float* table_out[KGCN_ASSEMBLE_MAX_TABLES];
  long row_floats[KGCN_ASSEMBLE_MAX_TABLES];
};

__global__ __launch_bounds__(kScanBlock) void assemble_count_kernel(AssemblePlan p, const int* __restrict__ sel, int T,
                                                                    int* __restrict__ block_sums) {
  const int c = blockIdx.y;
  const int t = blockIdx.x * kScanBlock + threadIdx.x;
  const int cnt = t < T ? graph_entries(p.src_rowptr[c], sel[t], p.M[c], p.row_pad[c] ? 4 * p.M[c] : 0) : 0;
  int tot;
  const int ex = block_exclusive_scan(cnt, &tot);
  if (t < T) p.graph_ptr[c][t] = ex;
  if (threadIdx.x == 0) block_sums[c * p.nb + blockIdx.x] = tot;
}

__global__ __launch_bounds__(256) void assemble_copy_kernel(AssemblePlan p, const int* __restrict__ sel, int T,
                                                            const int* __restrict__ block_sums) {
  const int lane = threadIdx.x & (kWave - 1);
  const long wave0 = ((long)blockIdx.x * 256 + threadIdx.x) / kWave;
  const long nwaves = (long)gridDim.x * 256 / kWave;
  if ((int)blockIdx.y >= p.num_csr) {
    const int k = blockIdx.y - p.num_csr;
    const long rf = p.row_floats[k];
    const float* __restrict__ src = p.table[k];
    float* __restrict__ dst = p.table_out[k];
    for (long t = wave0; t < T; t += nwaves) {
      const int g = sel[t];
      const float* in = src + (long)(g < 0 ? 0 : g) * rf;
      float* out = dst + t * rf;
      for (long i = lane; i < rf; i += kWave) out[i] = g < 0 ? 0.f : in[i];
    }
    return;
  }
  const int c = blockIdx.y, M = p.M[c], row_pad = p.row_pad[c];
  const int* __restrict__ src_rowptr = p.src_rowptr[c];
  const int* bs = block_sums + c * p.nb;
  int* graph_ptr = p.graph_ptr[c];
  int* dst_rowptr = p.dst_rowptr[c];
  int* dst_slots = p.dst_slots[c];
  for (long t = wave0; t < T; t += nwaves) {
    const int g = sel[t];
    const int b = (int)(t / kScanBlock);
    int off = 0;
    for (int i = lane; i < b; i += kWave) off += bs[i];
#pragma unroll
    for (int o = kWave / 2; o > 0; o >>= 1) off += __shfl_xor(off, o, kWave);
    const int out_base = graph_ptr[t] + off;
    int* rp_out = dst_rowptr + t * M;
    int cnt;
    if (g >= 0) {
      const int* rp_in = src_rowptr + (long)g * M;
      const int src_base = rp_in[0];
      cnt = rp_in[M] - src_base;
      for (int r = lane; r < M; r += kWave) rp_out[r] = rp_in[r] - src_base + out_base;
      const int2* in = p.src_cv[c] + src_base;
      int2* out = p.dst_cv[c] + out_base;
      for (int i = lane; i < cnt; i += kWave) out[i] = in[i];
      if (row_pad) {
        const int* sl = p.src_slots[c] + (long)g * M;
        for (int r = lane; r < M; r += kWave) dst_slots[t * M + r] = sl[r];
      }
    } else if (row_pad) {
      cnt = 4 * M;
      for (int r = lane; r < M; r += kWave) {
        rp_out[r] = out_base + 4 * r;
        dst_slots[t * M + r] = (4 * r) | (4 << 16) | (r << 24);
      }
      int2* out = p.dst_cv[c] + out_base;
      for (int i = lane; i < cnt; i += kWave) out[i] = make_int2(KGCN_PAD_COL, 0);
    } else {
      cnt = 0;
      for (int r = lane; r < M; r += kWave) rp_out[r] = out_base;
    }
    __builtin_amdgcn_wave_barrier();
    if (lane == 0) {
      graph_ptr[t] = out_base;
      if (t == T - 1) {
        dst_rowptr[(long)T * M] = out_base + cnt;
        graph_ptr[T] = out_base + cnt;
      }
    }
  }
}

}

using namespace kgcn;

extern "C" int64_t kgcn_csr_gather_workspace_bytes(int32_t num_sel) {
  if (num_sel <= 0) return 0;
  return (int64_t)((num_sel + kScanBlock - 1) / kScanBlock) * 4;
}

extern "C" int kgcn_csr_gather_graphs(const kgcn_csr_batch* src, const int32_t* sel, int32_t num_sel,
                                      int32_t* dst_rowptr, int32_t* dst_cv, int64_t dst_cv_capacity,
                                      int32_t* dst_slots, int32_t* dst_graph_ptr, void* workspace,
                                      int64_t workspace_bytes, void* stream) {
  if (int rc = validate_csr(src, "kgcn_csr_gather_graphs", true)) return rc;
  if (num_sel < 0) return fail("kgcn_csr_gather_graphs: negative num_sel");
  if (!dst_rowptr || !dst_graph_ptr) return fail("kgcn_csr_gather_graphs: dst_rowptr / dst_graph_ptr is NULL");
  if (src->row_pad == 4 && (!src->slots || (num_sel > 0 && src->rows > 0 && !dst_slots)))
    return fail("kgcn_csr_gather_graphs: a row-padded source needs slots and dst_slots");
  if ((int64_t)num_sel * src->rows >= (int64_t)INT32_MAX)
    return fail("kgcn_csr_gather_graphs: T*M exceeds int32 row indexing");
  hipStream_t s = as_stream(stream);
  if (num_sel == 0) {
    hipError_t e = hipMemsetAsync(dst_rowptr, 0, 4, s);
    if (e == hipSuccess) e = hipMemsetAsync(dst_graph_ptr, 0, 4, s);
    return e == hipSuccess ? 0 : fail("kgcn_csr_gather_graphs: memset failed: %s", hipGetErrorString(e));
  }
  if (!sel) return fail("kgcn_csr_gather_graphs: sel is NULL");
  const int64_t need = kgcn_csr_gather_workspace_bytes(num_sel);
  if (!workspace || workspace_bytes < need)
    return fail("kgcn_csr_gather_graphs: workspace %lld < %lld bytes", (long long)workspace_bytes, (long long)need);
  if (dst_cv_capacity < 0 || (dst_cv_capacity > 0 && !dst_cv))
    return fail("kgcn_csr_gather_graphs: dst_cv is NULL with capacity %lld", (long long)dst_cv_capacity);
  const int nb = (num_sel + kScanBlock - 1) / kScanBlock;
  int* block_sums = static_cast<int*>(workspace);
  const int dummy_cnt = src->row_pad ? 4 * src->rows : 0;
  hipLaunchKernelGGL(gather_count_kernel, dim3(nb), dim3(kScanBlock), 0, s, src->rowptr, sel, num_sel, src->rows,
                     dummy_cnt, dst_graph_ptr, block_sums);
  if (int rc = check_launch("gather_count_kernel")) return rc;
  hipLaunchKernelGGL(gather_scan_blocks_kernel, dim3(1), dim3(kScanBlock), 0, s, block_sums, nb,
                     dst_graph_ptr + num_sel);
  if (int rc = check_launch("gather_scan_blocks_kernel")) return rc;
  long blocks = ((long)num_sel + 3) / 4;
  if (blocks > (long)kNumCU * 32) blocks = (long)kNumCU * 32;
  hipLaunchKernelGGL(gather_copy_kernel, dim3((unsigned)blocks), dim3(256), 0, s, src->rowptr,
                     reinterpret_cast<const int2*>(src->cv), src->slots, sel, num_sel, src->rows, src->row_pad,
                     block_sums, dst_graph_ptr, dst_rowptr, reinterpret_cast<int2*>(dst_cv), dst_slots);
  return check_launch("gather_copy_kernel");
}

extern "C" int64_t kgcn_batch_assemble_workspace_bytes(int32_t num_sel) {
  if (num_sel <= 0) return 0;
  return (int64_t)KGCN_ASSEMBLE_MAX_CSR * ((num_sel + kScanBlock - 1) / kScanBlock) * 4;
}

extern "C" int kgcn_batch_assemble(const kgcn_assemble_plan* plan, const int32_t* sel, int32_t num_sel, void* workspace,
                                   int64_t workspace_bytes, void* stream) {
  if (!plan) return fail("kgcn_batch_assemble: plan is NULL");
  if (plan->num_csr < 0 || plan->num_csr > KGCN_ASSEMBLE_MAX_CSR || plan->num_tables < 0 ||
      plan->num_tables > KGCN_ASSEMBLE_MAX_TABLES)
    return fail("kgcn_batch_assemble: %d containers / %d tables (at most %d / %d)", plan->num_csr, plan->num_tables,
                KGCN_ASSEMBLE_MAX_CSR, KGCN_ASSEMBLE_MAX_TABLES);
  if (num_sel < 0) return fail("kgcn_batch_assemble: negative num_sel");
  AssemblePlan p{};
  p.num_csr = plan->num_csr;
  p.num_tables = plan->num_tables;
  p.nb = (num_sel + kScanBlock - 1) / kScanBlock;
  for (int c = 0; c < plan->num_csr; ++c) {
    const kgcn_csr_batch* src = plan->src[c];
    if (int rc = validate_csr(src, "kgcn_batch_assemble", true)) return rc;
    if (!plan->dst_rowptr[c] || !plan->dst_graph_ptr[c]) return fail("kgcn_batch_assemble: container %d: dst_rowptr / dst_graph_ptr is NULL", c);
    if (src->row_pad == 4 && (!src->slots || (num_sel > 0 && src->rows > 0 && !plan->dst_slots[c])))
      return fail("kgcn_batch_assemble: container %d: a row-padded source needs slots and dst_slots", c);
    if ((int64_t)num_sel * src->rows >= (int64_t)INT32_MAX) return fail("kgcn_batch_assemble: T*M exceeds int32 row indexing");
    const int64_t worst = (int64_t)num_sel * (src->row_pad && 4 * src->rows > src->max_nnz_per_graph ? 4 * src->rows
                                                                                                       : src->max_nnz_per_graph);
    if (plan->dst_cv_capacity[c] < worst || (worst > 0 && !plan->dst_cv[c]))
      return fail("kgcn_batch_assemble: container %d: dst_cv holds %lld entries, the worst case is %lld", c,
                  (long long)plan->dst_cv_capacity[c], (long long)worst);
    p.src_rowptr[c] = src->rowptr;
    p.src_cv[c] = reinterpret_cast<const int2*>(src->cv);
    p.src_slots[c] = src->slots;
    p.M[c] = src->rows;
    p.row_pad[c] = src->row_pad;
    p.graph_ptr[c] = plan->dst_graph_ptr[c];
    p.dst_rowptr[c] = plan->dst_rowptr[c];
    p.dst_cv[c] = reinterpret_cast<int2*>(plan->dst_cv[c]);
    p.dst_slots[c] = plan->dst_slots[c];
  }
  for (int k = 0; k < plan->num_tables; ++k) {
    if (plan->row_floats[k] < 0) return fail("kgcn_batch_assemble: table %d: negative row length", k);
    if (num_sel > 0 && plan->row_floats[k] > 0 && (!plan->table[k] || !plan->table_out[k]))
      return fail("kgcn_batch_assemble: table %d: NULL pointer", k);
    p.table[k] = plan->table[k];
    p.table_out[k] = plan->table_out[k];
    p.row_floats[k] = plan->row_floats[k];
  }
  hipStream_t s = as_stream(stream);
  if (num_sel == 0) {
    for (int c = 0; c < plan->num_csr; ++c) {
      hipError_t e = hipMemsetAsync(plan->dst_rowptr[c], 0, 4, s);
      if (e == hipSuccess) e = hipMemsetAsync(plan->dst_graph_ptr[c], 0, 4, s);
      if (e != hipSuccess) return fail("kgcn_batch_assemble: memset failed: %s", hipGetErrorString(e));
    }
    return 0;
  }
  if (!sel) return fail("kgcn_batch_assemble: sel is NULL");
  if (plan->num_csr + plan->num_tables == 0) return 0;
  const int64_t need = kgcn_batch_assemble_workspace_bytes(num_sel);
  if (!workspace || workspace_bytes < need)
    return fail("kgcn_batch_assemble: workspace %lld < %lld bytes", (long long)workspace_bytes, (long long)need);
  int* block_sums = static_cast<int*>(workspace);
  if (plan->num_csr > 0) {
    hipLaunchKernelGGL(assemble_count_kernel, dim3(p.nb, plan->num_csr), dim3(kScanBlock), 0, s, p, sel, num_sel, block_sums);
    if (int rc = check_launch("assemble_count_kernel")) return rc;
  }
  long blocks = ((long)num_sel + 3) / 4;
  if (blocks > (long)kNumCU * 8) blocks = (long)kNumCU * 8;
  hipLaunchKernelGGL(assemble_copy_kernel, dim3((unsigned)blocks, plan->num_csr + plan->num_tables), dim3(256), 0, s, p, sel,
                     num_sel, block_sums);
  return check_launch("assemble_copy_kernel");
}
```

kgcn_amd/csrc/skinny.hip:

```cpp
#include "dense_kernels.h"

namespace kgcn {

constexpr int SKN = 16;
constexpr int SK_KPL = 16;

template <int N>
__global__ __launch_bounds__(256) void skinny_n_fwd_kernel(const float* __restrict__ x, long m, int k, long x_ld,
                                                           const float* __restrict__ w, long w_ld, const float* __restrict__ bias,
                                                           float* __restrict__ y, long y_ld, int act, int n) {
  const int lane = threadIdx.x & 63;
  const long wave = ((long)blockIdx.x * 256 + threadIdx.x) >> 6, nwaves = ((long)gridDim.x * 256) >> 6;
  for (long r = wave; r < m; r += nwaves) {
    float acc[N];
#pragma unroll
    for (int j = 0; j < N; ++j) acc[j] = 0.f;
    const float* xr = x + r * x_ld;
    for (int c = lane; c < k; c += 64) {
      const float xv = xr[c];
      const float* wr = w + (long)c * w_ld;
#pragma unroll
      for (int j = 0; j < N; ++j) acc[j] = __builtin_fmaf(xv, j < n ? wr[j] : 0.f, acc[j]);
    }
#pragma unroll
    for (int j = 0; j < N; ++j) {
#pragma unroll
      for (int o = 32; o > 0; o >>= 1) acc[j] += __shfl_xor(acc[j], o, 64);
    }
    float out = 0.f;
#pragma unroll
    for (int j = 0; j < N; ++j) out = lane == j ? acc[j] : out;
    if (lane < n) y[r * y_ld + lane] = act_fwd(out + (bias ? bias[lane] : 0.f), act);
  }
}

template <int K>
__global__ __launch_bounds__(256) void skinny_k_fwd_kernel(const float* __restrict__ x, long m, long x_ld,
                                                           const float* __restrict__ w, long w_ld, int trans, int n,
                                                           const float* __restrict__ bias, float* __restrict__ y, long y_ld,
                                                           int act) {
  const int lane = threadIdx.x & 63;
  const long wave = ((long)blockIdx.x * 256 + threadIdx.x) >> 6, nwaves = ((long)gridDim.x * 256) >> 6;
  for (int c0 = 0; c0 < n; c0 += 64 * 4) {
    float wv[4][K], bv[4];
#pragma unroll
    for (int q = 0; q < 4; ++q) {
      const int c = c0 + 64 * q + lane;
      bv[q] = (bias && c < n) ? bias[c] : 0.f;
#pragma unroll
      for (int j = 0; j < K; ++j) wv[q][j] = c < n ? (trans ? w[(long)c * w_ld + j] : w[(long)j * w_ld + c]) : 0.f;
    }
    for (long r = wave; r < m; r += nwaves) {
      float xv[K];
#pragma unroll
      for (int j = 0; j < K; ++j) xv[j] = x[r * x_ld + j];
#pragma unroll
      for (int q = 0; q < 4; ++q) {
        const int c = c0 + 64 * q + lane;
        float s = bv[q];
#pragma unroll
        for (int j = 0; j < K; ++j) s = __builtin_fmaf(xv[j], wv[q][j], s);
        if (c < n) y[r * y_ld + c] = act_fwd(s, act);
      }
    }
  }
}

template <int N, int QK>
__global__ __launch_bounds__(256) void skinny_n_wgrad_kernel(const float* __restrict__ x, long m, int k, long x_ld,
                                                             const float* __restrict__ g, long g_ld,
                                                             float* __restrict__ part_dw, float* __restrict__ part_db, int n) {
  extern __shared__ float red[];
  const int lane = threadIdx.x & 63, wv = threadIdx.x >> 6;
  const long wave = ((long)blockIdx.x * 256 + threadIdx.x) >> 6, nwaves = ((long)gridDim.x * 256) >> 6;
  float acc[QK][N], bs[N];
#pragma unroll
  for (int q = 0; q < QK; ++q)
#pragma unroll
    for (int j = 0; j < N; ++j) acc[q][j] = 0.f;
#pragma unroll
  for (int j = 0; j < N; ++j) bs[j] = 0.f;
  for (long r = wave; r < m; r += 2 * nwaves) {
    const long r2 = r + nwaves;
    const bool two = r2 < m;
    float gv[N], gw[N];
#pragma unroll
    for (int j = 0; j < N; ++j) {
      gv[j] = j < n ? g[r * g_ld + j] : 0.f;
      gw[j] = (two && j < n) ? g[r2 * g_ld + j] : 0.f;
    }
    const float* xr = x + r * x_ld;
    const float* xs = x + (two ? r2 : r) * x_ld;
    float xa[QK], xb[QK];
#pragma unroll
    for (int q = 0; q < QK; ++q) {
      const int c = lane + 64 * q;
      xa[q] = c < k ? xr[c] : 0.f;
      xb[q] = c < k ? xs[c] : 0.f;
    }
#pragma unroll
    for (int q = 0; q < QK; ++q) {
#pragma unroll
      for (int j = 0; j < N; ++j) acc[q][j] = __builtin_fmaf(xb[q], gw[j], __builtin_fmaf(xa[q], gv[j], acc[q][j]));
    }
#pragma unroll
    for (int j = 0; j < N; ++j) bs[j] += gv[j] + gw[j];
  }
  float* mine = red + (long)wv * (k * n + n);
#pragma unroll
  for (int q = 0; q < QK; ++q) {
    const int c = lane + 64 * q;
    if (c < k) {
#pragma unroll
      for (int j = 0; j < N; ++j)
        if (j < n) mine[c * n + j] = acc[q][j];
    }
  }
  if (lane == 0) {
#pragma unroll
    for (int j = 0; j < N; ++j)
      if (j < n) mine[k * n + j] = bs[j];
  }
  __syncthreads();
  const int tot = k * n;
  for (int i = threadIdx.x; i < tot + n; i += 256) {
    const float s = (red[i] + red[(tot + n) + i]) + (red[2 * (tot + n) + i] + red[3 * (tot + n) + i]);
    if (i < tot) part_dw[(long)blockIdx.x * tot + i] = s;
    else if (part_db) part_db[(long)blockIdx.x * n + (i - tot)] = s;
  }
}

static int skinny_blocks(long m) {
  long b = (m + 3) / 4;
  if (b > (long)kNumCU * 8) b = (long)kNumCU * 8;
  return (int)(b < 1 ? 1 : b);
}

static int round_n(int n) { return n <= 2 ? 2 : (n <= 4 ? 4 : (n <= 8 ? 8 : (n <= 12 ? 12 : 16))); }
static int round_qk(int k) { const int q = (k + 63) / 64; return q <= 1 ? 1 : (q <= 2 ? 2 : (q <= 4 ? 4 : (q <= 8 ? 8 : 16))); }

bool skinny_n_ok(int din, int dout, int trans_w) {
  if (trans_w || dout > SKN || din < 32 || din > 64 * SK_KPL) return false;
  return round_qk(din) * round_n(dout) <= 128 && (size_t)4 * ((size_t)din * dout + dout) * 4 <= 64 * 1024;
}
bool skinny_k_ok(int din, int dout) { return din <= SKN && dout >= 32; }

int launch_skinny_n_fwd(const float* x, long m, int din, long x_ld, const float* w, long w_ld, const float* bias, float* y,
                        int dout, long y_ld, int act, hipStream_t s) {
  const dim3 grid(skinny_blocks(m));
#define KGCN_CASE(NN) case NN: hipLaunchKernelGGL(skinny_n_fwd_kernel<NN>, grid, dim3(256), 0, s, x, m, din, x_ld, w, w_ld, bias, y, y_ld, act, dout); break;
  switch (round_n(dout)) {
    KGCN_CASE(2) KGCN_CASE(4) KGCN_CASE(8) KGCN_CASE(12) KGCN_CASE(16)
    default: return fail("skinny_n_fwd: dout=%d", dout);
  }
#undef KGCN_CASE
  return check_launch("skinny_n_fwd_kernel");
}

int launch_skinny_k_fwd(const float* x, long m, int din, long x_ld, const float* w, long w_ld, int trans_w, const float* bias,
                        float* y, int dout, long y_ld, int act, hipStream_t s) {
  const dim3 grid(skinny_blocks(m));
#define KGCN_CASE(KK) case KK: hipLaunchKernelGGL(skinny_k_fwd_kernel<KK>, grid, dim3(256), 0, s, x, m, x_ld, w, w_ld, trans_w, dout, bias, y, y_ld, act); break;
  switch (din) {
    KGCN_CASE(1) KGCN_CASE(2) KGCN_CASE(3) KGCN_CASE(4) KGCN_CASE(5) KGCN_CASE(6) KGCN_CASE(7) KGCN_CASE(8)
    KGCN_CASE(9) KGCN_CASE(10) KGCN_CASE(11) KGCN_CASE(12) KGCN_CASE(13) KGCN_CASE(14) KGCN_CASE(15) KGCN_CASE(16)
    default: return fail("skinny_k_fwd: din=%d", din);
  }
#undef KGCN_CASE
  return check_launch("skinny_k_fwd_kernel");
}

int skinny_wgrad_parts(long m) {
  long b = (m + 15) / 16;
  if (b > 4L * kNumCU) b = 4L * kNumCU;
  return (int)(b < 1 ? 1 : b);
}

int launch_skinny_n_wgrad(const float* x, long m, int din, long x_ld, const float* g, long g_ld, int dout, float* part_dw,
                          float* part_db, int nparts, hipStream_t s) {
  const dim3 grid(nparts);
  const size_t lds = (size_t)4 * ((size_t)din * dout + dout) * 4;
  const int nn = round_n(dout), qk = round_qk(din);
#define KGCN_W(NN, QQ)                                                                                                \
  if (nn == NN && qk == QQ) {                                                                                         \
    hipLaunchKernelGGL((skinny_n_wgrad_kernel<NN, QQ>), grid, dim3(256), lds, s, x, m, din, x_ld, g, g_ld, part_dw,   \
                       part_db, dout);                                                                                \
    return check_launch("skinny_n_wgrad_kernel");                                                                     \
  }
  KGCN_W(2, 1) KGCN_W(2, 2) KGCN_W(2, 4) KGCN_W(2, 8) KGCN_W(2, 16)
  KGCN_W(4, 1) KGCN_W(4, 2) KGCN_W(4, 4) KGCN_W(4, 8) KGCN_W(4, 16)
  KGCN_W(8, 1) KGCN_W(8, 2) KGCN_W(8, 4) KGCN_W(8, 8) KGCN_W(8, 16)
  KGCN_W(12, 1) KGCN_W(12, 2) KGCN_W(12, 4) KGCN_W(12, 8)
  KGCN_W(16, 1) KGCN_W(16, 2) KGCN_W(16, 4) KGCN_W(16, 8)
#undef KGCN_W
  return fail("skinny_n_wgrad: unsupported shape %d x %d", din, dout);
}

}
```

kgcn_amd/csrc/train.hip:

```cpp
#include "kgcn_common.h"

namespace kgcn {

constexpr int kLossBlock = 256;

__device__ __forceinline__ float block_sum_256(float v, float* red) {
  red[threadIdx.x] = v;
  __syncthreads();
#pragma unroll
  for (int off = 128; off > 0; off >>= 1) {
    if ((int)threadIdx.x < off) red[threadIdx.x] += red[threadIdx.x + off];
    __syncthreads();
  }
  const float s = red[0];
  __syncthreads();
  return s;
}

__global__ __launch_bounds__(kLossBlock) void sigmoid_ce_kernel(const float* __restrict__ logits, const float* __restrict__ labels,
                                                               const float* __restrict__ mask, const float* __restrict__ mask_label,
                                                               long B, int T, int weighted, float q,
                                                               const float* __restrict__ qvec, float* __restrict__ cost,
                                                               float* __restrict__ dlogits, float* __restrict__ part,
                                                               float* __restrict__ sums_direct) {
  __shared__ float red[kLossBlock];
  const long b = (long)blockIdx.x * kLossBlock + threadIdx.x;
  float c = 0.f;
  if (b < B) {
    const float mk = mask[b];
    for (int t = 0; t < T; ++t) {
      const long i = b * T + t;
      const float x = logits[i], z = labels[i], ml = mask_label ? mask_label[i] : 1.f;
      const float sp = log1pf(__expf(-fabsf(x)));
      const float sg = 1.0f / (1.0f + __expf(-x));
      float ce, dce;
      if (!weighted) {
        ce = fmaxf(x, 0.f) - x * z + sp;
        dce = sg - z;
      } else {
        const float lw = 1.f + ((qvec ? qvec[t] : q) - 1.f) * z;
        ce = (1.f - z) * x + lw * (sp + fmaxf(-x, 0.f));
        dce = (1.f - z) - lw * (1.f - sg);
      }
      c += ml * ce;
      dlogits[i] = mk * ml * dce;
    }
    c *= mk;
    if (cost) cost[b] = c;
  }
  const float s = block_sum_256(c, red);
  if (threadIdx.x == 0) {
    part[blockIdx.x] = s;
    if (sums_direct) {
      sums_direct[0] = s;
      sums_direct[1] = s / (float)B;
    }
  }
}

__global__ __launch_bounds__(kLossBlock) void softmax_ce_kernel(const float* __restrict__ logits, const float* __restrict__ labels,
                                                               const long long* __restrict__ label_idx,
                                                               const float* __restrict__ mask, long B, int C,
                                                               float* __restrict__ cost, float* __restrict__ dlogits,
                                                               float* __restrict__ part, float* __restrict__ sums_direct) {
  __shared__ float red[kLossBlock];
  const long b = (long)blockIdx.x * kLossBlock + threadIdx.x;
  float c = 0.f;
  if (b < B) {
    const float* x = logits + b * C;
    const float* z = labels ? labels + b * C : nullptr;
    const int li = label_idx ? (int)label_idx[b] : -1;
    float mx = -INFINITY;
    for (int k = 0; k < C; ++k) mx = fmaxf(mx, x[k]);
    float se = 0.f, zs = 0.f, zx = 0.f;
    for (int k = 0; k < C; ++k) {
      const float zk = z ? z[k] : (k == li ? 1.f : 0.f);
      se += __expf(x[k] - mx);
      zs += zk;
      zx += zk * (x[k] - mx);
    }
    const float lse = __logf(se);
    const float mk = mask ? mask[b] : 1.f;
    c = mk * (zs * lse - zx);
    const float inv = 1.0f / se;
    for (int k = 0; k < C; ++k)
      dlogits[b * C + k] = mk * (__expf(x[k] - mx) * inv * zs - (z ? z[k] : (k == li ? 1.f : 0.f)));
    if (cost) cost[b] = c;
  }
  const float s = block_sum_256(c, red);
  if (threadIdx.x == 0) {
    part[blockIdx.x] = s;
    if (sums_direct) {
      sums_direct[0] = s;
      sums_direct[1] = s / (float)B;
    }
  }
}

__global__ __launch_bounds__(kLossBlock) void loss_finish_kernel(const float* __restrict__ part, int nparts, long B,
                                                                float* __restrict__ sums) {
  __shared__ float red[kLossBlock];
  float a = 0.f;
  for (int i = threadIdx.x; i < nparts; i += kLossBlock) a += part[i];
  const float s = block_sum_256(a, red);
  if (threadIdx.x == 0) {
    sums[0] = s;
    sums[1] = s / (float)B;
  }
}

__global__ __launch_bounds__(256) void loss_grad_kernel(const float* __restrict__ dlogits, const float* __restrict__ g_opt,
                                                        const float* __restrict__ g_sum, float inv_batch, long n,
                                                        float* __restrict__ out) {
  const float sc = (g_opt ? *g_opt * inv_batch : 0.f) + (g_sum ? *g_sum : 0.f);
  for (long i = (long)blockIdx.x * 256 + threadIdx.x; i < n; i += (long)gridDim.x * 256) out[i] = dlogits[i] * sc;
}

__device__ __forceinline__ void adam_tf_update(float& p, float& m, float& v, float g, float lr_t, float b1, float b2, float c1,
                                               float c2, float eps) {
  m = __builtin_fmaf(m, b1, g * c1);
  v = __builtin_fmaf(v, b2, (g * g) * c2);
  p = __builtin_fmaf(-lr_t, m / (__builtin_sqrtf(v) + eps), p);
}

__device__ __forceinline__ long long adam_step_of(const long long* counter) { return *counter + 1; }

template <bool VEC>
__global__ __launch_bounds__(256) void adam_tf_kernel(float* __restrict__ p, const float* __restrict__ g, float* __restrict__ m,
                                                      float* __restrict__ v, long n, float lr, float b1, float b2, float eps,
                                                      const long long* __restrict__ counter) {
  __shared__ float lr_s;
  if (threadIdx.x == 0) {
    const double t = (double)adam_step_of(counter);
    lr_s = (float)((double)lr * sqrt(1.0 - pow((double)b2, t)) / (1.0 - pow((double)b1, t)));
  }
  __syncthreads();
  const float lr_t = lr_s;
  const float c1 = 1.0f - b1, c2 = 1.0f - b2;
  if constexpr (VEC) {
    const long n4 = n >> 2;
    for (long i = (long)blockIdx.x * 256 + threadIdx.x; i < n4; i += (long)gridDim.x * 256) {
      f32x4 pv = reinterpret_cast<f32x4*>(p)[i], mv = reinterpret_cast<f32x4*>(m)[i], vv = reinterpret_cast<f32x4*>(v)[i];
      const f32x4 gv = reinterpret_cast<const f32x4*>(g)[i];
#pragma unroll
      for (int j = 0; j < 4; ++j) {
        float pj = pv[j], mj = mv[j], vj = vv[j];
        adam_tf_update(pj, mj, vj, gv[j], lr_t, b1, b2, c1, c2, eps);
        pv[j] = pj; mv[j] = mj; vv[j] = vj;
      }
      reinterpret_cast<f32x4*>(p)[i] = pv;
      reinterpret_cast<f32x4*>(m)[i] = mv;
      reinterpret_cast<f32x4*>(v)[i] = vv;
    }
  } else {
    for (long i = (long)blockIdx.x * 256 + threadIdx.x; i < n; i += (long)gridDim.x * 256) {
      float pj = p[i], mj = m[i], vj = v[i];
      adam_tf_update(pj, mj, vj, g[i], lr_t, b1, b2, c1, c2, eps);
      p[i] = pj; m[i] = mj; v[i] = vj;
    }
  }
}

__global__ void adam_tick_kernel(long long* counter) { *counter += 1; }

}

using namespace kgcn;

extern "C" int64_t kgcn_loss_workspace_bytes(int64_t batch) {
  if (batch <= 0) return 4;
  return ((batch + kLossBlock - 1) / kLossBlock) * 4;
}

static int loss_args(const char* who, const void* logits, const void* labels, const void* mask, int64_t batch, int32_t width,
                     const void* dlogits, const void* sums, const void* ws, int64_t wsb) {
  if (batch <= 0 || width <= 0) return fail("%s: bad shape batch=%lld width=%d", who, (long long)batch, width);
  if (!logits || !labels || !mask || !dlogits || !sums) return fail("%s: NULL operand", who);
  if (!ws || wsb < kgcn_loss_workspace_bytes(batch))
    return fail("%s: workspace %lld < %lld bytes", who, (long long)wsb, (long long)kgcn_loss_workspace_bytes(batch));
  if ((batch + kLossBlock - 1) / kLossBlock > 0x7fffffffLL) return fail("%s: batch too large", who);
  return 0;
}

extern "C" int kgcn_masked_sigmoid_ce_f32(const float* logits, const float* labels, const float* mask,
                                          const float* mask_label, int64_t batch, int32_t tasks, int32_t weighted,
                                          float pos_weight, const float* pos_weight_per_task, float* cost, float* dlogits,
                                          float* sums, void* workspace, int64_t workspace_bytes, void* stream) {
  if (int rc = loss_args("kgcn_masked_sigmoid_ce_f32", logits, labels, mask, batch, tasks, dlogits, sums, workspace,
                         workspace_bytes))
    return rc;
  const int nb = (int)((batch + kLossBlock - 1) / kLossBlock);
  float* part = static_cast<float*>(workspace);
  hipStream_t s = as_stream(stream);
  hipLaunchKernelGGL(sigmoid_ce_kernel, dim3(nb), dim3(kLossBlock), 0, s, logits, labels, mask, mask_label, (long)batch, tasks,
                     weighted ? 1 : 0, pos_weight, weighted ? pos_weight_per_task : nullptr, cost, dlogits, part,
                     nb == 1 ? sums : nullptr);
  if (int rc = check_launch("sigmoid_ce_kernel")) return rc;
  if (nb == 1) return 0;
  hipLaunchKernelGGL(loss_finish_kernel, dim3(1), dim3(kLossBlock), 0, s, part, nb, (long)batch, sums);
  return check_launch("loss_finish_kernel");
}

extern "C" int kgcn_masked_softmax_ce_f32(const float* logits, const float* labels, const float* mask, int64_t batch,
                                          int32_t classes, float* cost, float* dlogits, float* sums, void* workspace,
                                          int64_t workspace_bytes, void* stream) {
  if (int rc = loss_args("kgcn_masked_softmax_ce_f32", logits, labels, mask, batch, classes, dlogits, sums, workspace,
                         workspace_bytes))
    return rc;
  const int nb = (int)((batch + kLossBlock - 1) / kLossBlock);
  float* part = static_cast<float*>(workspace);
  hipStream_t s = as_stream(stream);
  hipLaunchKernelGGL(softmax_ce_kernel, dim3(nb), dim3(kLossBlock), 0, s, logits, labels, nullptr, mask, (long)batch, classes,
                     cost, dlogits, part, nb == 1 ? sums : nullptr);
  if (int rc = check_launch("softmax_ce_kernel")) return rc;
  if (nb == 1) return 0;
  hipLaunchKernelGGL(loss_finish_kernel, dim3(1), dim3(kLossBlock), 0, s, part, nb, (long)batch, sums);
  return check_launch("loss_finish_kernel");
}

extern "C" int kgcn_sparse_softmax_ce_f32(const float* logits, const int64_t* label_idx, const float* mask, int64_t batch,
                                          int32_t classes, float* cost, float* dlogits, float* sums, void* workspace,
                                          int64_t workspace_bytes, void* stream) {
  if (batch <= 0 || classes <= 0) return fail("kgcn_sparse_softmax_ce_f32: bad shape batch=%lld classes=%d", (long long)batch, classes);
  if (!logits || !label_idx || !dlogits || !sums) return fail("kgcn_sparse_softmax_ce_f32: NULL operand");
  if (!workspace || workspace_bytes < kgcn_loss_workspace_bytes(batch)) return fail("kgcn_sparse_softmax_ce_f32: workspace too small");
  const int nb = (int)((batch + kLossBlock - 1) / kLossBlock);
  float* part = static_cast<float*>(workspace);
  hipStream_t s = as_stream(stream);
  hipLaunchKernelGGL(softmax_ce_kernel, dim3(nb), dim3(kLossBlock), 0, s, logits, nullptr,
                     reinterpret_cast<const long long*>(label_idx), mask, (long)batch, classes, cost, dlogits, part,
                     nb == 1 ? sums : nullptr);
  if (int rc = check_launch("softmax_ce_kernel")) return rc;
  if (nb == 1) return 0;
  hipLaunchKernelGGL(loss_finish_kernel, dim3(1), dim3(kLossBlock), 0, s, part, nb, (long)batch, sums);
  return check_launch("loss_finish_kernel");
}

extern "C" int kgcn_loss_grad_f32(const float* dlogits, const float* g_opt, const float* g_sum, int64_t batch, int64_t n,
                                  float* out, void* stream) {
  if (n < 0 || batch <= 0) return fail("kgcn_loss_grad_f32: bad shape n=%lld batch=%lld", (long long)n, (long long)batch);
  if (n == 0) return 0;
  if (!dlogits || !out) return fail("kgcn_loss_grad_f32: NULL operand");
  long blocks = (n + 255) / 256;
  if (blocks > 4L * kNumCU) blocks = 4L * kNumCU;
  hipLaunchKernelGGL(loss_grad_kernel, dim3((unsigned)blocks), dim3(256), 0, as_stream(stream), dlogits, g_opt, g_sum,
                     1.0f / (float)batch, (long)n, out);
  return check_launch("loss_grad_kernel");
}

struct AdamSegs {
  const float* grad[KGCN_ADAM_MAX_SEGMENTS];
  long offset[KGCN_ADAM_MAX_SEGMENTS], numel[KGCN_ADAM_MAX_SEGMENTS];
};

__global__ __launch_bounds__(256) void adam_tf_multi_kernel(float* __restrict__ p, float* __restrict__ m, float* __restrict__ v,
                                                            AdamSegs sg, float lr, float b1, float b2, float eps,
                                                            const long long* __restrict__ counter) {
  __shared__ float lr_s;
  if (threadIdx.x == 0) {
    const double t = (double)adam_step_of(counter);
    lr_s = (float)((double)lr * sqrt(1.0 - pow((double)b2, t)) / (1.0 - pow((double)b1, t)));
  }
  __syncthreads();
  const float lr_t = lr_s;
  const float c1 = 1.0f - b1, c2 = 1.0f - b2;
  const int q = blockIdx.y;
  const float* __restrict__ g = sg.grad[q];
  const long off = sg.offset[q], n = sg.numel[q];
  for (long i = (long)blockIdx.x * 256 + threadIdx.x; i < n; i += (long)gridDim.x * 256) {
    float pj = p[off + i], mj = m[off + i], vj = v[off + i];
    adam_tf_update(pj, mj, vj, g[i], lr_t, b1, b2, c1, c2, eps);
    p[off + i] = pj; m[off + i] = mj; v[off + i] = vj;
  }
}

extern "C" int kgcn_adam_tf_multi_f32(float* params, float* m, float* v, int64_t n, const kgcn_adam_segment* segments,
                                      int32_t num_segments, float lr, float beta1, float beta2, float eps, int64_t* step_counter,
                                      void* stream) {
  if (n < 0 || num_segments < 0) return fail("kgcn_adam_tf_multi_f32: negative size");
  if (!step_counter) return fail("kgcn_adam_tf_multi_f32: step_counter is NULL");
  if (num_segments > 0 && (!params || !m || !v || !segments)) return fail("kgcn_adam_tf_multi_f32: NULL operand");
  hipStream_t s = as_stream(stream);
  for (int base = 0; base < num_segments; base += KGCN_ADAM_MAX_SEGMENTS) {
    const int cnt = num_segments - base < KGCN_ADAM_MAX_SEGMENTS ? num_segments - base : KGCN_ADAM_MAX_SEGMENTS;
    AdamSegs sg{};
    long most = 1;
    for (int q = 0; q < cnt; ++q) {
      const kgcn_adam_segment& e = segments[base + q];
      if (e.offset < 0 || e.numel < 0 || e.offset + e.numel > n || (e.numel > 0 && !e.grad))
        return fail("kgcn_adam_tf_multi_f32: segment %d: offset %lld + %lld floats of %lld", base + q, (long long)e.offset,
                    (long long)e.numel, (long long)n);
      sg.grad[q] = e.grad; sg.offset[q] = (long)e.offset; sg.numel[q] = (long)e.numel;
      if (e.numel > most) most = (long)e.numel;
    }
    long blocks = (most + 255) / 256;
    if (blocks > 2L * kNumCU) blocks = 2L * kNumCU;
    hipLaunchKernelGGL(adam_tf_multi_kernel, dim3((unsigned)blocks, cnt), dim3(256), 0, s, params, m, v, sg, lr, beta1, beta2, eps,
                       reinterpret_cast<const long long*>(step_counter));
    if (int rc = check_launch("adam_tf_multi_kernel")) return rc;
  }
  hipLaunchKernelGGL(adam_tick_kernel, dim3(1), dim3(1), 0, s, reinterpret_cast<long long*>(step_counter));
  return check_launch("adam_tick_kernel");
}

extern "C" int kgcn_adam_tf_f32(float* params, const float* grads, float* m, float* v, int64_t n, float lr, float beta1,
                                float beta2, float eps, int64_t* step_counter, void* stream) {
  if (n < 0) return fail("kgcn_adam_tf_f32: n < 0");
  if (!step_counter) return fail("kgcn_adam_tf_f32: step_counter is NULL");
  hipStream_t s = as_stream(stream);
  if (n > 0) {
    if (!params || !grads || !m || !v) return fail("kgcn_adam_tf_f32: NULL operand");
    const bool vec = (n % 4 == 0) && aligned16(params) && aligned16(grads) && aligned16(m) && aligned16(v);
    long blocks = ((vec ? n / 4 : n) + 255) / 256;
    if (blocks > (long)kNumCU * 8) blocks = (long)kNumCU * 8;
    if (blocks < 1) blocks = 1;
    const long long* ctr = reinterpret_cast<const long long*>(step_counter);
    if (vec)
      hipLaunchKernelGGL(adam_tf_kernel<true>, dim3((unsigned)blocks), dim3(256), 0, s, params, grads, m, v, (long)n, lr,
                         beta1, beta2, eps, ctr);
    else
      hipLaunchKernelGGL(adam_tf_kernel<false>, dim3((unsigned)blocks), dim3(256), 0, s, params, grads, m, v, (long)n, lr,
                         beta1, beta2, eps, ctr);
    if (int rc = check_launch("adam_tf_kernel")) return rc;
  }
  hipLaunchKernelGGL(adam_tick_kernel, dim3(1), dim3(1), 0, s, reinterpret_cast<long long*>(step_counter));
  return check_launch("adam_tick_kernel");
}
```

kgcn_amd/ops.py:

```python
import contextlib
import ctypes

import torch

from . import _lib
from ._lib import check, current_stream, lib, ptr, require_gpu
from .batched_csr import BatchedAdjacency, BatchedCSR


ACT_CODES = {None: 0, "none": 0, "linear": 0, "sigmoid": 1, "relu": 2, "tanh": 3}
wgrad_dact_fusion = True
side_stream_wgrad = False
side_wgrad_min_rows = 16384
_side_streams = {}
_side_pending = set()


def _side_stream(device):
    key = (device.type, device.index)
    if key not in _side_streams:
        _side_streams[key] = torch.cuda.Stream(device=device)
    return _side_streams[key]


_deferred_keep = []


class deferred_reductions:

    def __init__(self, root=None):
        self.root = root

    def __enter__(self):
        _no_defer_params.clear()
        if self.root is not None:
            _no_defer_params.update(_readers_inside_backward(self.root))
        self.prev = lib.kgcn_reduce_defer(1)
        return self

    def __exit__(self, *exc):
        try:
            flush_reductions()
        finally:
            lib.kgcn_reduce_defer(self.prev)
            _no_defer_params.clear()
        return False


_no_defer_params = set()


def _readers_inside_backward(root):
    roots = root if isinstance(root, (list, tuple)) else (root,)
    edges, seen, stack = {}, set(), [t.grad_fn for t in roots if t is not None and t.grad_fn is not None]
    while stack:
        fn = stack.pop()
        if fn in seen:
            continue
        seen.add(fn)
        for nxt, _ in fn.next_functions:
            if nxt is None:
                continue
            if hasattr(nxt, "variable"):
                edges[nxt] = edges.get(nxt, 0) + 1
            elif nxt not in seen:
                stack.append(nxt)
    out = set()
    for acc, n in edges.items():
        v = acc.variable
        if n > 1 or v.grad is not None or getattr(v, "_backward_hooks", None) or getattr(v, "_post_accumulate_grad_hooks", None):
            out.add(id(v))
    return out


def flush_reductions():
    check(lib.kgcn_reduce_flush(current_stream()), "kgcn_reduce_flush")
    _deferred_keep.clear()


_param_uses = {}


def _record_params(ctx, *params, when=True):
    ps = []
    for p in params:
        if p is not None:
            ps.extend(getattr(p, "_kgcn_defer_params", (p,)))
    for p in ps:
        _param_uses[id(p)] = _param_uses.get(id(p), 0) + 1
    ctx.defer_params = tuple(ps) if when else ()


class _param_grad_stage:

    __slots__ = ("ok", "ws", "prev")

    def __init__(self, ctx, nbytes, device, when=True):
        self.ws = _lib.workspace(nbytes, device)
        ps = ctx.defer_params
        self.ok = bool(when and ps and not torch.is_grad_enabled() and all(
            p.is_leaf and p.requires_grad and _param_uses.get(id(p), 0) == 1 and id(p) not in _no_defer_params for p in ps))

    def __enter__(self):
        self.prev = None if self.ok else lib.kgcn_reduce_defer(0)
        return self.ws

    def __exit__(self, *exc):
        if self.prev is not None:
            lib.kgcn_reduce_defer(self.prev)
        if lib.kgcn_reduce_pending() > 0:
            _deferred_keep.append(self.ws)
        return False


def join_side_streams():
    for key in list(_side_pending):
        torch.cuda.current_stream(torch.device(*key)).wait_stream(_side_streams[key])
    _side_pending.clear()


def _fork_side(device):
    side = _side_stream(device)
    side.wait_stream(torch.cuda.current_stream(device))
    key = (device.type, device.index)
    if key not in _side_pending:
        _side_pending.add(key)
        try:
            torch.autograd.Variable._execution_engine.queue_callback(join_side_streams)
        except RuntimeError:
            pass
    return side


def act_code(activation):
    try:
        return ACT_CODES[activation]
    except KeyError:
        raise ValueError("unsupported activation %r (None, 'sigmoid', 'relu', 'tanh')" % (activation,)) from None


def _f32c(t, name):
    require_gpu(t, name)
    if t.dtype != torch.float32:
        raise _lib.KgcnHipError("%s must be float32 (the path computes in fp32), got %s" % (name, t.dtype))
    return t.contiguous()


def bspmm_raw(csr, rhs2d, d, out2d, rhs_ld=None, rhs_gs=None, out_ld=None, out_gs=None, beta=0.0,
              rhs_col=0, out_col=0):
    rhs_ld = rhs2d.stride(0) if rhs_ld is None else rhs_ld
    out_ld = out2d.stride(0) if out_ld is None else out_ld
    rhs_gs = csr.cols * rhs_ld if rhs_gs is None else rhs_gs
    out_gs = csr.rows * out_ld if out_gs is None else out_gs
    check(lib.kgcn_bspmm_f32(csr.desc(), rhs2d.data_ptr() + 4 * rhs_col, rhs_ld, rhs_gs, d,
                             out2d.data_ptr() + 4 * out_col, out_ld, out_gs, float(beta),
                             current_stream()), "kgcn_bspmm_f32")
    return out2d


class _SpMM(torch.autograd.Function):
# ... 374 lines not shown

enabled_weight_tables = True
weight_tables = WeightTables()


dense_bwd_fusion = True


def _dense_bwd_fused_ok(x2d, w, gy, yact, gp=None, gp_ld=0, n_nodes=0, act_is_smooth=False):
    m, din = x2d.shape
    dout = w.shape[1]
    if not (dense_bwd_fusion and lib.kgcn_dense_bwd_supported(m, din, dout)):
        return False
    ts = [t for t in (x2d, gy, yact) if t is not None]
    if not all(t.is_contiguous() and t.data_ptr() % 16 == 0 for t in ts):
        return False
    if gp is None:
        return True
    if gy is not None and yact is not None and act_is_smooth:
        return False
    return gp.data_ptr() % 16 == 0 and gp_ld % 4 == 0 and n_nodes >= 8


def _dense_bwd_fused(ctx, x2d, w, gy, yact, act, need_b, gp=None, gp_ld=0, n_nodes=0):
    m, din = x2d.shape
    dout = w.shape[1]
    dx = torch.empty_like(x2d)
    dw = torch.empty_like(w)
    db = torch.empty((dout,), device=x2d.device, dtype=torch.float32) if need_b else None
    tab, tb = weight_tables.lookup(w, 1)
    ready = 1
    if tab is None:
        tb, tab = _dense_ws(dout, din, x2d.device)
        ready = 0
    wsb = lib.kgcn_dense_wgrad_workspace_bytes(m, din, dout)
    with _param_grad_stage(ctx, wsb, x2d.device) as wsp:
        check(lib.kgcn_dense_bwd_f32(ptr(gy), None if gp is None else gp.data_ptr(), gp_ld, n_nodes, ptr(yact) if act else None,
                                     int(act), dout, ptr(x2d), din, m, din, dout, ptr(w), dout, ptr(dx), din, ptr(dw), ptr(db),
                                     ptr(tab), tb, ready, ptr(wsp), wsb, current_stream()), "kgcn_dense_bwd_f32")
    if db is not None:
        db = db.reshape(ctx.bias_shape)
    return dx, dw, db


class _Dense(torch.autograd.Function):
    @staticmethod
    def forward(ctx, x2d, w, bias, act=0):
        _record_params(ctx, w, bias)
        x2d, w = _f32c(x2d, "x"), _f32c(w, "w")
        m, din = x2d.shape
        dout = w.shape[1]
        if w.shape[0] != din:
            raise _lib.KgcnHipError("kernel is %s but inputs have %d features" % (tuple(w.shape), din))
        b = None if bias is None else _f32c(bias, "bias").reshape(-1)
        if b is not None and b.numel() != dout:
            raise _lib.KgcnHipError("bias has %d elements, expected %d" % (b.numel(), dout))
        y = torch.empty((m, dout), device=x2d.device, dtype=torch.float32)
        tab, tb = weight_tables.lookup(w, 0)
        if tab is not None:
            check(lib.kgcn_dense_fwd_tab_f32(ptr(x2d), m, din, din, ptr(w), dout, 0, ptr(b), ptr(y), dout,
                                             dout, int(act), ptr(tab), tb, current_stream()), "kgcn_dense_fwd_tab_f32")
        else:
            weight_tables.register(w)
            wsb, wsp = _dense_ws(din, dout, x2d.device)
            check(lib.kgcn_dense_fwd_ws_f32(ptr(x2d), m, din, din, ptr(w), dout, 0, ptr(b), ptr(y), dout,
                                            dout, int(act), ptr(wsp), wsb, current_stream()), "kgcn_dense_fwd_ws_f32")
        ctx.act = int(act)
        ctx.save_for_backward(x2d, w, y if act else x2d)
        ctx.bias_shape = None if bias is None else tuple(bias.shape)
        return y

    @staticmethod
    def backward(ctx, gy):
        x2d, w, yact = ctx.saved_tensors
        gy = _f32c(gy, "grad")
        m, din = x2d.shape
        dout = w.shape[1]
        dx = dw = db = None
        need_b = ctx.bias_shape is not None and ctx.needs_input_grad[2]
        if ctx.needs_input_grad[0] and ctx.needs_input_grad[1] and not (side_stream_wgrad and m >= side_wgrad_min_rows) and \
                _dense_bwd_fused_ok(x2d, w, gy, yact if ctx.act else None):
            dx, dw, db = _dense_bwd_fused(ctx, x2d, w, gy, yact, ctx.act, need_b)
            return dx, dw, db, None
        fuse_dact = bool(ctx.act) and not ctx.needs_input_grad[0] and wgrad_dact_fusion and \
            bool(lib.kgcn_dense_wgrad_dact_supported(din, dout))
        if ctx.act and ctx.needs_input_grad[0]:
            dx = torch.empty_like(x2d)
            dpre = torch.empty_like(gy)
            tab, tb = weight_tables.lookup(w, 1)
            if tab is not None:
                check(lib.kgcn_dense_dx_dact_tab_f32(ptr(gy), ptr(yact), m, dout, dout, ptr(w), dout, din, ptr(dx), din, ctx.act,
                                                     ptr(dpre), ptr(tab), tb, current_stream()), "kgcn_dense_dx_dact_tab_f32")
            else:
                wsb, wsp = _dense_ws(dout, din, gy.device)
                check(lib.kgcn_dense_dx_dact_f32(ptr(gy), ptr(yact), m, dout, dout, ptr(w), dout, din, ptr(dx), din, ctx.act,
                                                 ptr(dpre), ptr(wsp), wsb, current_stream()), "kgcn_dense_dx_dact_f32")
            gy = dpre
        else:
            if ctx.act and not fuse_dact:
                gy = activation_backward(yact, gy, ctx.act)
            if ctx.needs_input_grad[0]:
                dx = torch.empty_like(x2d)
                tab, tb = weight_tables.lookup(w, 1)
                if tab is not None:
                    check(lib.kgcn_dense_fwd_tab_f32(ptr(gy), m, dout, dout, ptr(w), dout, 1, None, ptr(dx),
                                                     din, din, 0, ptr(tab), tb, current_stream()), "kgcn_dense_fwd_tab_f32(dx)")
                else:
                    wsb, wsp = _dense_ws(dout, din, gy.device)
                    check(lib.kgcn_dense_fwd_ws_f32(ptr(gy), m, dout, dout, ptr(w), dout, 1, None, ptr(dx),
                                                    din, din, 0, ptr(wsp), wsb, current_stream()), "kgcn_dense_fwd_ws_f32(dx)")
        need_w = ctx.needs_input_grad[1]
        need_b = ctx.bias_shape is not None and ctx.needs_input_grad[2]
        if need_w or need_b:
            side = None
            if side_stream_wgrad and m >= side_wgrad_min_rows:
                side = _fork_side(gy.device)
                for t in (gy, x2d, yact):
                    t.record_stream(side)
            with torch.cuda.stream(side) if side is not None else contextlib.nullcontext():
                dw, db = _Dense._wgrad(ctx, x2d, w, gy, yact, m, din, dout, need_w, need_b, fuse_dact)
        return dx, dw, db, None

    @staticmethod
    def _wgrad(ctx, x2d, w, gy, yact, m, din, dout, need_w, need_b, fuse_dact):
        wsb = lib.kgcn_dense_wgrad_workspace_bytes(m, din, dout)
        dw = torch.empty_like(w) if need_w else None
        db = torch.empty((dout,), device=gy.device, dtype=torch.float32) if need_b else None
        with _param_grad_stage(ctx, wsb, gy.device) as wsp:
            if fuse_dact:
                check(lib.kgcn_dense_wgrad_dact_f32(ptr(x2d), din, ptr(gy), ptr(yact), dout, ctx.act, m, din, dout, ptr(dw),
                                                    ptr(db), ptr(wsp), wsb, current_stream()), "kgcn_dense_wgrad_dact_f32")
            else:
                check(lib.kgcn_dense_wgrad_f32(ptr(x2d), din, ptr(gy), dout, m, din, dout, ptr(dw),
                                               ptr(db), ptr(wsp), wsb, current_stream()),
                      "kgcn_dense_wgrad_f32")
        if db is not None:
            db = db.reshape(ctx.bias_shape)
        return dw, db


class _StackRows(torch.autograd.Function):

    @staticmethod
    def forward(ctx, w, bias, pad):
        ctx.rows = (w.shape[0], bias.shape[0])
        return torch.cat([w, bias, pad], dim=0)

    @staticmethod
    def backward(ctx, g):
        n0, n1 = ctx.rows
        return g[:n0], g[n0:n0 + n1], None


def stack_rows(w, bias, pad):
    out = _StackRows.apply(w, bias, pad)
    out._kgcn_defer_params = (w, bias)
    return out


class _DenseStacked(torch.autograd.Function):

    @staticmethod
    def forward(ctx, x2d, w, bias, act, tab, tb):
        m, rows = x2d.shape
        dout = w.shape[1]
        y = torch.empty((m, dout), device=x2d.device, dtype=torch.float32)
# ... 661 lines not shown


class _AugmentOnes(torch.autograd.Function):
    @staticmethod
    def forward(ctx, x2d, width):
        x2d = _f32c(x2d, "inputs")
        m, din = x2d.shape
        out = torch.empty((m, width), device=x2d.device, dtype=torch.float32)
        check(lib.kgcn_augment_ones_f32(ptr(x2d), m, din, din, ptr(out), width, current_stream()), "kgcn_augment_ones_f32")
        ctx.shape = (m, din)
        return out

    @staticmethod
    def backward(ctx, g):
        g = _f32c(g, "grad")
        m, din = ctx.shape
        dx = torch.empty((m, din), device=g.device, dtype=torch.float32)
        check(lib.kgcn_augment_ones_bwd_f32(ptr(g), m, din, g.shape[1], ptr(dx), din, current_stream()),
              "kgcn_augment_ones_bwd_f32")
        return dx, None


def augment_ones(x2d, width):
    return _AugmentOnes.apply(x2d, width)


def _loss_grad(dlog, g_opt, g_sum, batch):
    if g_opt is None and g_sum is None:
        return None
    go = None if g_opt is None else _f32c(g_opt.reshape(1), "grad")
    gs = None if g_sum is None else _f32c(g_sum.reshape(1), "grad")
    out = torch.empty_like(dlog)
    check(lib.kgcn_loss_grad_f32(ptr(dlog), ptr(go), ptr(gs), batch, dlog.numel(), ptr(out), current_stream()), "kgcn_loss_grad_f32")
    return out


_pos_weight_cache = {}


def _pos_weight_operand(pos_weight, W, device):
    if pos_weight is None:
        return 0.0, None
    if torch.is_tensor(pos_weight) and pos_weight.is_cuda:
        qv = pos_weight.detach().to(torch.float32).reshape(-1)
        if qv.numel() == 1:
            qv = qv.expand(W)
        if qv.numel() != W:
            raise _lib.KgcnHipError("pos_weight has %d entries for %d tasks" % (qv.numel(), W))
        return 0.0, qv.contiguous()
    if not (torch.is_tensor(pos_weight) or hasattr(pos_weight, "__len__")):
        return float(pos_weight), None
    host = torch.as_tensor(pos_weight, dtype=torch.float32).reshape(-1)
    if host.numel() == 1:
        return float(host), None
    if host.numel() != W:
        raise _lib.KgcnHipError("pos_weight has %d entries for %d tasks" % (host.numel(), W))
    content = host.numpy().tobytes()
    hit = _pos_weight_cache.get(id(pos_weight))
    if hit is not None and hit[0] is pos_weight and hit[1] == content and hit[2] == device:
        return 0.0, hit[3]
    if torch.cuda.is_current_stream_capturing():
        raise _lib.KgcnHipError("a host pos_weight was first seen (or changed) while a hipGraph is being captured: pass a device "
                                "tensor, or run one eager step with this pos_weight before the capture")
    if len(_pos_weight_cache) >= 64:
        _pos_weight_cache.clear()
    qv = host.to(device).contiguous()
    _pos_weight_cache[id(pos_weight)] = (pos_weight, content, device, qv)
    return 0.0, qv


class _MaskedCE(torch.autograd.Function):
    @staticmethod
    def forward(ctx, logits, labels, mask, mask_label, kind, pos_weight):
        x = _f32c(logits, "logits")
        if x.dim() != 2:
            raise _lib.KgcnHipError("logits must be [batch, width], got %s" % (tuple(x.shape),))
        B, W = x.shape
        z = _f32c(labels.to(torch.float32), "labels")
        mk = _f32c(mask.to(torch.float32).reshape(-1), "mask")
        ml = None if mask_label is None else _f32c(mask_label.to(torch.float32), "mask_label")
        if tuple(z.shape) != (B, W) or mk.numel() != B or (ml is not None and tuple(ml.shape) != (B, W)):
            raise _lib.KgcnHipError("labels / mask / mask_label do not match logits %s" % (tuple(x.shape),))
        dlog = torch.empty_like(x)
        sums = torch.empty((2,), device=x.device, dtype=torch.float32)
        wsb = lib.kgcn_loss_workspace_bytes(B)
        ws = _lib.workspace(wsb, x.device)
        if kind == "sigmoid":
            qs, qv = _pos_weight_operand(pos_weight, W, x.device)
            check(lib.kgcn_masked_sigmoid_ce_f32(ptr(x), ptr(z), ptr(mk), ptr(ml), B, W, 0 if pos_weight is None else 1,
                                                 qs, ptr(qv), None, ptr(dlog), ptr(sums), ptr(ws), wsb, current_stream()),
                  "kgcn_masked_sigmoid_ce_f32")
        else:
            check(lib.kgcn_masked_softmax_ce_f32(ptr(x), ptr(z), ptr(mk), B, W, None, ptr(dlog), ptr(sums), ptr(ws), wsb,
                                                 current_stream()), "kgcn_masked_softmax_ce_f32")
        ctx.save_for_backward(dlog)
        ctx.batch = B
        ctx.set_materialize_grads(False)
        return sums[1], sums[0]

    @staticmethod
    def backward(ctx, g_opt, g_sum):
        (dlog,) = ctx.saved_tensors
        return _loss_grad(dlog, g_opt, g_sum, ctx.batch), None, None, None, None, None


class _SparseCE(torch.autograd.Function):
    @staticmethod
    def forward(ctx, logits, label_idx):
        x = _f32c(logits, "logits")
        B, W = x.shape
        idx = label_idx.reshape(-1).to(torch.int64).contiguous()
        require_gpu(idx, "labels")
        if idx.numel() != B:
            raise _lib.KgcnHipError("labels have %d entries for %d rows of logits" % (idx.numel(), B))
        dlog = torch.empty_like(x)
        sums = torch.empty((2,), device=x.device, dtype=torch.float32)
        wsb = lib.kgcn_loss_workspace_bytes(B)
        ws = _lib.workspace(wsb, x.device)
        check(lib.kgcn_sparse_softmax_ce_f32(ptr(x), ptr(idx), None, B, W, None, ptr(dlog), ptr(sums), ptr(ws), wsb,
                                             current_stream()), "kgcn_sparse_softmax_ce_f32")
        ctx.save_for_backward(dlog)
        return sums[0]

    @staticmethod
    def backward(ctx, g):
        (dlog,) = ctx.saved_tensors
        return _loss_grad(dlog, None, g, 1), None


def sparse_softmax_ce_sum(logits, label_idx):
    return _SparseCE.apply(logits, label_idx)


def masked_sigmoid_ce(logits, labels, mask, mask_label=None, pos_weight=None):
    return _MaskedCE.apply(logits, labels, mask, mask_label, "sigmoid", pos_weight)


def masked_softmax_ce(logits, labels, mask):
    return _MaskedCE.apply(logits, labels, mask, None, "softmax", None)


__all__ = ["BatchedCSR", "BatchedAdjacency", "bspmm", "bspmm_raw", "bconv", "dense", "activation", "act_code",
           "graphconv_fused", "graphconv_fused_supported", "gin_aggregate", "graph_gather",
           "graph_maxpool", "gat", "gram", "ragged_gather", "ragged_compact_rows",
           "masked_sigmoid_ce", "masked_softmax_ce", "sparse_softmax_ce_sum", "augment_ones",
           "gcn_stack", "gcn_stack_supported", "graph_gather_tee"]


def graph_bn_stats(x, enabled=None):
    x = _f32c(x, "inputs")
    T, N, D = x.shape
    mean = torch.empty((D,), device=x.device, dtype=torch.float32)
    var = torch.empty_like(mean)
    wsb = lib.kgcn_graph_bn_workspace_bytes(D)
    wsp = _lib.workspace(wsb, x.device)
    check(lib.kgcn_graph_bn_stats_f32(ptr(x), T, N, D, ptr(enabled), ptr(mean), ptr(var), ptr(wsp), wsb,
                                      current_stream()), "kgcn_graph_bn_stats_f32")
    return mean, var


class _GraphBN(torch.autograd.Function):
    @staticmethod
    def forward(ctx, x, gamma, beta, mean, var, enabled, eps, training, act=0):
        x = _f32c(x, "inputs")
        T, N, D = x.shape
        _record_params(ctx, gamma, beta, when=not training)
        gamma, beta = _f32c(gamma, "gamma"), _f32c(beta, "beta")
        y = torch.empty_like(x)
        check(lib.kgcn_graph_bn_apply_act_f32(ptr(x), T, N, D, ptr(enabled), ptr(mean), ptr(var), ptr(gamma), ptr(beta),
                                              float(eps), int(act), ptr(y), current_stream()), "kgcn_graph_bn_apply_act_f32")
        ctx.save_for_backward(x, gamma, mean, var, y if act else x)
        ctx.enabled, ctx.eps, ctx.training, ctx.act = enabled, float(eps), bool(training), int(act)
        return y

    @staticmethod
    def backward(ctx, g):
        x, gamma, mean, var, yact = ctx.saved_tensors
        g = _f32c(g, "grad")
        T, N, D = x.shape
        dx = torch.empty_like(x) if ctx.needs_input_grad[0] else None
        dgamma = torch.empty((D,), device=x.device, dtype=torch.float32)
        dbeta = torch.empty_like(dgamma)
        wsb = lib.kgcn_graph_bn_workspace_bytes(D)
        with _param_grad_stage(ctx, wsb, x.device, when=dx is not None) as wsp:
            check(lib.kgcn_graph_bn_bwd_dact_f32(ptr(x), ptr(g), ptr(yact) if ctx.act else None, ctx.act, T, N, D,
                                                 ptr(ctx.enabled), ptr(mean), ptr(var), ptr(gamma), ctx.eps, int(ctx.training),
                                                 ptr(dx), ptr(dgamma), ptr(dbeta), ptr(wsp), wsb, current_stream()),
                  "kgcn_graph_bn_bwd_dact_f32")
        return dx, dgamma, dbeta, None, None, None, None, None, None


def graph_bn(x, gamma, beta, mean, var, enabled=None, eps=1e-3, training=False, activation=None):
    return _GraphBN.apply(x, gamma, beta, mean, var, enabled, eps, training, act_code(activation))


VAE_MAX_NODES, VAE_MAX_CHANNELS, VAE_MAX_DIM = 128, 8, 64


def _step_ptr(step):
    if step is None:
        return None
    if not (torch.is_tensor(step) and step.is_cuda and step.dtype == torch.int64 and step.numel() == 1):
        raise _lib.KgcnHipError("step must be a one-element int64 device tensor (or None)")
    return step


def philox4x64_raw(seed, step, num_blocks, device):
    out = torch.empty((int(num_blocks), 4), device=device, dtype=torch.int64)
    check(lib.kgcn_philox4x64_raw(int(seed) & (2 ** 64 - 1), ptr(_step_ptr(step)), int(num_blocks), ptr(out), current_stream()),
# ... 758 lines not shown
```

kgcn_amd/train.py:

```python
import torch


class FlatParameters:
    ALIGN = 64

    def __init__(self, params):
        self.params = [p for p in params]
        if not self.params:
            raise ValueError("FlatParameters: empty parameter list -- the layers create their parameters on the first forward "
                             "pass (Keras build semantics); run one forward before collecting model.parameters()")
        dev = self.params[0].device
        if dev.type != "cuda":
            raise ValueError("the fused optimiser needs device-resident parameters (kgcn_amd has no CPU path)")
        self.offsets, off = [], 0
        for p in self.params:
            if p.dtype != torch.float32 or p.device != dev:
                raise ValueError("all parameters must be float32 on one device")
            self.offsets.append(off)
            off += -(-p.numel() // self.ALIGN) * self.ALIGN
        self.total = off
        self.data = torch.zeros(off, device=dev, dtype=torch.float32)
        self.grad = torch.zeros(off, device=dev, dtype=torch.float32)
        self.views, self.grad_views = [], []
        with torch.no_grad():
            for p, o in zip(self.params, self.offsets):
                v = self.data[o:o + p.numel()].view(p.shape)
                v.copy_(p.data)
                p.data = v
                self.views.append(v)
                self.grad_views.append(self.grad[o:o + p.numel()].view(p.shape))

    def pack_grads(self):
        from . import ops
        ops.join_side_streams()
        grads = [p.grad for p in self.params]
        if any(g is None for g in grads):
            raise RuntimeError("FlatParameters: a parameter has no gradient")
        torch._foreach_copy_(self.grad_views, grads)
        return self.grad


class TFAdam:

    def __init__(self, params, lr=1e-3, beta1=0.9, beta2=0.999, eps=1e-8, capturable=True):
        params = [p for p in params]
        if not params:
            raise ValueError("TFAdam: empty parameter list -- the layers create their parameters on the first forward "
                             "pass (Keras build semantics); run one forward before collecting model.parameters()")
        self.flat = FlatParameters(params)
        self.params = self.flat.params
        self.lr, self.b1, self.b2, self.eps = lr, beta1, beta2, eps
        self.t = 0
        self._m = torch.zeros_like(self.flat.data)
        self._v = torch.zeros_like(self.flat.data)
        self.m = [self._m[o:o + p.numel()].view(p.shape) for p, o in zip(self.params, self.flat.offsets)]
        self.v = [self._v[o:o + p.numel()].view(p.shape) for p, o in zip(self.params, self.flat.offsets)]
        self.capturable = True
        self._t_dev = torch.zeros((), dtype=torch.int64, device=self.flat.data.device)

    def zero_grad(self, set_to_none=True):
        if set_to_none or any(p.grad is None for p in self.params):
            for p in self.params:
                p.grad = None
        else:
            torch._foreach_zero_([p.grad for p in self.params])

    @torch.no_grad()
    def step(self, packed=False):
        from . import _lib
        from . import ops
        ops.weight_tables.invalidate()
        self.t += 1
        if not packed:
            import ctypes
            ops.join_side_streams()
            segs = (_lib.AdamSegment * len(self.params))()
            keep = []
            for i, (p, o) in enumerate(zip(self.params, self.flat.offsets)):
                g = p.grad
                if g is None:
                    raise RuntimeError("TFAdam: a parameter has no gradient")
                if g.dtype != torch.float32 or not g.is_contiguous():
                    g = g.to(torch.float32).contiguous()
                    keep.append(g)
                segs[i] = _lib.AdamSegment(g.data_ptr(), o, p.numel())
            _lib.check(_lib.lib.kgcn_adam_tf_multi_f32(_lib.ptr(self.flat.data), _lib.ptr(self._m), _lib.ptr(self._v),
                                                       self.flat.total, ctypes.cast(segs, ctypes.c_void_p), len(self.params),
                                                       float(self.lr), float(self.b1), float(self.b2), float(self.eps),
                                                       _lib.ptr(self._t_dev), _lib.current_stream()), "kgcn_adam_tf_multi_f32")
            return
        _lib.check(_lib.lib.kgcn_adam_tf_f32(_lib.ptr(self.flat.data), _lib.ptr(self.flat.grad), _lib.ptr(self._m),
                                             _lib.ptr(self._v), self.flat.total, float(self.lr), float(self.b1),
                                             float(self.b2), float(self.eps), _lib.ptr(self._t_dev), _lib.current_stream()),
                   "kgcn_adam_tf_f32")


def _exchange(bucket, optimizer, shard_weight):
    if bucket is None:
        return False
    shared = getattr(bucket, "flat_params", None) is optimizer.flat
    bucket.all_reduce_mean(weight=shard_weight, unpack=not shared)
    return shared


def train_step(model, optimizer, loss_fn, features, adjs, labels, mask, bucket=None, shard_weight=None,
               **fwd_kwargs):
    from . import ops
    optimizer.zero_grad()
    ops.weight_tables.refresh()
    logits = model(features, adjs, **fwd_kwargs)
    cost_opt, cost_sum = loss_fn(logits, labels, mask)
    with ops.deferred_reductions(root=cost_opt):
        cost_opt.backward()
    optimizer.step(packed=_exchange(bucket, optimizer, shard_weight))
    return float(cost_sum.detach()), logits.detach()


def capture_mode():
    import torch.distributed as dist
    if dist.is_available() and dist.is_initialized():
        import time
        time.sleep(0.25)
        return {"capture_error_mode": "thread_local"}
    return {}


class GraphedTrainStep:

    def __init__(self, model, optimizer, loss_fn, static_batch, labels, mask, warmup=3, bucket=None,
                 shard_weight=None, capture_assembly=False, **fwd_kwargs):
        if not optimizer.capturable:
            raise ValueError("GraphedTrainStep needs TFAdam(capturable=True)")
        self.bucket, self.shard_weight = bucket, shard_weight
        self.model, self.opt, self.loss_fn, self.sb = model, optimizer, loss_fn, static_batch
        self.labels, self.mask, self.kw = labels, mask, fwd_kwargs
        self.cost_sum = self.logits = self._seed = None
        self.capture_assembly = bool(capture_assembly)
        if self.capture_assembly and not hasattr(static_batch, "assemble"):
            raise ValueError("capture_assembly needs a static batch with stage() / assemble()")
        if hasattr(static_batch, "reset_usage"):
            static_batch.reset_usage()
        saved = [t.detach().clone() for t in list(optimizer.params) + optimizer.m + optimizer.v]
        saved_t = optimizer.t
        side = torch.cuda.Stream()
        side.wait_stream(torch.cuda.current_stream())
        with torch.cuda.stream(side):
            for _ in range(warmup):
                self._eager()
        torch.cuda.current_stream().wait_stream(side)
        torch.cuda.synchronize()
        self.graph = torch.cuda.CUDAGraph()
        with torch.cuda.graph(self.graph, **capture_mode()):
            self._eager()
        with torch.no_grad():
            for dst, src in zip(list(optimizer.params) + optimizer.m + optimizer.v, saved):
                dst.copy_(src)
            optimizer._t_dev.fill_(saved_t)
        optimizer.t = saved_t
        if hasattr(static_batch, "prune_unused"):
            static_batch.prune_unused()

    def _eager(self):
        from . import ops
        self.opt.zero_grad(set_to_none=True)
        ops.weight_tables.refresh()
        if self.capture_assembly:
            self.sb.assemble()
        logits = self.model(self.sb.features, self.sb.adjacency, **self.kw)
        cost_opt, cost_sum = self.loss_fn(logits, self.labels, self.mask)
        if self._seed is None or self._seed.shape != cost_opt.shape:
            self._seed = torch.ones_like(cost_opt)
        with ops.deferred_reductions(root=cost_opt):
            cost_opt.backward(self._seed)
        self.opt.step(packed=_exchange(self.bucket, self.opt, self.shard_weight))
        self.cost_sum, self.logits = cost_sum.detach(), logits.detach()

    def replay(self):
        self.graph.replay()
        self.opt.t += 1
        return self.cost_sum, self.logits
```

Before: 130.3 million.

## Fuse dx into skinny wgrad, fold loss mean, tick Adam step in reduce, skip assemble count

Adds a skinny backward kernel that computes the input gradient alongside the weight-gradient partials for activation-free read-out layers. Loss kernels now emit a pre-scaled mean gradient, which is returned directly when the backward seed is a unit tensor, skipping the separate loss-grad kernel. The Adam step counter is incremented inside the deferred reduction kernel so the optimizer can use a 'ticked' variant without its own increment. Batch assembly skips the block-count kernel for small selections. Together these cut several small kernel launches per step, at the cost of extra code paths and implicit coupling between the reduce flush and the optimizer.

```diff
diff --git a/include/kgcn_hip.h b/include/kgcn_hip.h
--- a/include/kgcn_hip.h
+++ b/include/kgcn_hip.h
@@ -178,6 +178,10 @@
                                   int32_t din, float* dx, int64_t dx_ld, int32_t act, float* dpre, void* table,
                                   int64_t table_bytes, int32_t table_ready, void* stream);
 int kgcn_dense_bwd_supported(int64_t m, int32_t din, int32_t dout);
+int kgcn_dense_skinny_bwd_supported(int64_t m, int32_t din, int32_t dout);
+int kgcn_dense_skinny_bwd_f32(const float* x, int64_t x_ld, const float* dy, int64_t dy_ld, int64_t m, int32_t din, int32_t dout,
+                              const float* w, int64_t w_ld, float* dx, int64_t dx_ld, float* dw, float* dbias, void* workspace,
+                              int64_t workspace_bytes, void* stream);
 int kgcn_dense_bwd_f32(const float* grad, const float* pooled_grad, int64_t pooled_ld, int32_t n_nodes, const float* act_out,
                        int32_t act, int64_t ld, const float* x, int64_t x_ld, int64_t m, int32_t din, int32_t dout,
                        const float* w, int64_t w_ld, float* dx, int64_t dx_ld, float* dw, float* dbias, void* table,
@@ -270,6 +274,16 @@
                                int64_t workspace_bytes, void* stream);
 int kgcn_loss_grad_f32(const float* dlogits, const float* g_opt, const float* g_sum, int64_t batch, int64_t n, float* out,
                        void* stream);
+int kgcn_masked_sigmoid_ce_mean_f32(const float* logits, const float* labels, const float* mask, const float* mask_label,
+                                    int64_t batch, int32_t tasks, int32_t weighted, float pos_weight,
+                                    const float* pos_weight_per_task, float* cost, float* dlogits, float* dlogits_mean,
+                                    float* sums, void* workspace, int64_t workspace_bytes, void* stream);
+int kgcn_masked_softmax_ce_mean_f32(const float* logits, const float* labels, const float* mask, int64_t batch,
+                                    int32_t classes, float* cost, float* dlogits, float* dlogits_mean, float* sums,
+                                    void* workspace, int64_t workspace_bytes, void* stream);
+int kgcn_sparse_softmax_ce_mean_f32(const float* logits, const int64_t* label_idx, const float* mask, int64_t batch,
+                                    int32_t classes, float* cost, float* dlogits, float* dlogits_mean, float* sums,
+                                    void* workspace, int64_t workspace_bytes, void* stream);
 int kgcn_adam_tf_f32(float* params, const float* grads, float* m, float* v, int64_t n, float lr, float beta1, float beta2,
                      float eps, int64_t* step_counter, void* stream);
 #define KGCN_ADAM_MAX_SEGMENTS 32
@@ -279,6 +293,11 @@
 } kgcn_adam_segment;
 int kgcn_adam_tf_multi_f32(float* params, float* m, float* v, int64_t n, const kgcn_adam_segment* segments, int32_t num_segments,
                            float lr, float beta1, float beta2, float eps, int64_t* step_counter, void* stream);
+int kgcn_adam_tf_ticked_f32(float* params, const float* grads, float* m, float* v, int64_t n, float lr, float beta1,
+                            float beta2, float eps, const int64_t* step_counter, void* stream);
+int kgcn_adam_tf_multi_ticked_f32(float* params, float* m, float* v, int64_t n, const kgcn_adam_segment* segments,
+                                  int32_t num_segments, float lr, float beta1, float beta2, float eps,
+                                  const int64_t* step_counter, void* stream);
 
 int kgcn_augment_ones_f32(const float* x, int64_t m, int32_t din, int64_t x_ld, float* out, int64_t out_ld, void* stream);
 int kgcn_augment_ones_bwd_f32(const float* dout_grad, int64_t m, int32_t din, int64_t g_ld, float* dx, int64_t dx_ld,
@@ -306,6 +325,7 @@
 int kgcn_reduce_defer(int32_t on);
 int kgcn_reduce_pending(void);
 int kgcn_reduce_flush(void* stream);
+int kgcn_reduce_flush_tick(void* stream, int64_t* step_counter, int32_t* ticked);
 
 int kgcn_dense_mfma_products(int32_t kind, int64_t m, int32_t din, int32_t dout);
 
diff --git a/kgcn_amd/_lib.py b/kgcn_amd/_lib.py
--- a/kgcn_amd/_lib.py
+++ b/kgcn_amd/_lib.py
@@ -223,9 +223,13 @@
                                              ctypes.POINTER(SpmmRoute)]),
     "kgcn_copy2d_multi_f32": (ctypes.c_int, [ctypes.c_void_p, c_i32, ctypes.c_void_p]),
     "kgcn_hbm_probe": (ctypes.c_int, [c_i32, ctypes.c_void_p, ctypes.c_void_p, ctypes.c_void_p, c_i64, ctypes.c_void_p]),
+    "kgcn_dense_skinny_bwd_supported": (ctypes.c_int, [c_i64, c_i32, c_i32]),
+    "kgcn_dense_skinny_bwd_f32": (ctypes.c_int, [c_f32p, c_i64, c_f32p, c_i64, c_i64, c_i32, c_i32, c_f32p, c_i64, c_f32p, c_i64,
+                                                 c_f32p, c_f32p, ctypes.c_void_p, c_i64, ctypes.c_void_p]),
     "kgcn_reduce_defer": (ctypes.c_int, [c_i32]),
     "kgcn_reduce_pending": (ctypes.c_int, []),
     "kgcn_reduce_flush": (ctypes.c_int, [ctypes.c_void_p]),
+    "kgcn_reduce_flush_tick": (ctypes.c_int, [ctypes.c_void_p, ctypes.c_void_p, ctypes.POINTER(c_i32)]),
     "kgcn_loss_workspace_bytes": (c_i64, [c_i64]),
     "kgcn_masked_sigmoid_ce_f32": (ctypes.c_int, [c_f32p, c_f32p, c_f32p, c_f32p, c_i64, c_i32, c_i32, ctypes.c_float, c_f32p,
                                                   c_f32p, c_f32p, c_f32p, ctypes.c_void_p, c_i64, ctypes.c_void_p]),
@@ -235,6 +239,17 @@
                                                   ctypes.c_void_p, c_i64, ctypes.c_void_p]),
     "kgcn_adam_tf_multi_f32": (ctypes.c_int, [c_f32p, c_f32p, c_f32p, c_i64, ctypes.c_void_p, c_i32, ctypes.c_float,
                                               ctypes.c_float, ctypes.c_float, ctypes.c_float, ctypes.c_void_p, ctypes.c_void_p]),
+    "kgcn_masked_sigmoid_ce_mean_f32": (ctypes.c_int, [c_f32p, c_f32p, c_f32p, c_f32p, c_i64, c_i32, c_i32, ctypes.c_float, c_f32p,
+                                                       c_f32p, c_f32p, c_f32p, c_f32p, ctypes.c_void_p, c_i64, ctypes.c_void_p]),
+    "kgcn_masked_softmax_ce_mean_f32": (ctypes.c_int, [c_f32p, c_f32p, c_f32p, c_i64, c_i32, c_f32p, c_f32p, c_f32p, c_f32p,
+                                                       ctypes.c_void_p, c_i64, ctypes.c_void_p]),
+    "kgcn_sparse_softmax_ce_mean_f32": (ctypes.c_int, [c_f32p, ctypes.c_void_p, c_f32p, c_i64, c_i32, c_f32p, c_f32p, c_f32p,
+                                                       c_f32p, ctypes.c_void_p, c_i64, ctypes.c_void_p]),
+    "kgcn_adam_tf_multi_ticked_f32": (ctypes.c_int, [c_f32p, c_f32p, c_f32p, c_i64, ctypes.c_void_p, c_i32, ctypes.c_float,
+                                                     ctypes.c_float, ctypes.c_float, ctypes.c_float, ctypes.c_void_p,
+                                                     ctypes.c_void_p]),
+    "kgcn_adam_tf_ticked_f32": (ctypes.c_int, [c_f32p, c_f32p, c_f32p, c_f32p, c_i64, ctypes.c_float, ctypes.c_float,
+                                               ctypes.c_float, ctypes.c_float, ctypes.c_void_p, ctypes.c_void_p]),
     "kgcn_loss_grad_f32": (ctypes.c_int, [c_f32p, c_f32p, c_f32p, c_i64, c_i64, c_f32p, ctypes.c_void_p]),
     "kgcn_adam_tf_f32": (ctypes.c_int, [c_f32p, c_f32p, c_f32p, c_f32p, c_i64, ctypes.c_float, ctypes.c_float,
                                         ctypes.c_float, ctypes.c_float, ctypes.c_void_p, ctypes.c_void_p]),
diff --git a/kgcn_amd/csrc/dense.hip b/kgcn_amd/csrc/dense.hip
--- a/kgcn_amd/csrc/dense.hip
+++ b/kgcn_amd/csrc/dense.hip
@@ -358,10 +358,12 @@
   int nparts[kMaxReduceJobs];
   int block0[kMaxReduceJobs + 1];
   int njobs;
+  long long* tick;
 };
 
 __global__ __launch_bounds__(256) void reduce_partials_multi_kernel(ReduceJobs jb) {
   __shared__ float red[8][33];
+  if (jb.tick && blockIdx.x == 0 && threadIdx.x == 0) *jb.tick += 1;
   int j = 0;
   while (j + 1 < jb.njobs && (int)blockIdx.x >= jb.block0[j + 1]) ++j;
   const float* __restrict__ src = jb.part[j];
@@ -396,8 +398,9 @@
 static PendingReduce g_pending[256];
 static int g_npending = 0;
 
-static int flush_pending_locked(hipStream_t s) {
+static int flush_pending_locked(hipStream_t s, long long* tick = nullptr, int32_t* ticked = nullptr) {
   int done = 0;
+  if (ticked) *ticked = 0;
   while (done < g_npending) {
     ReduceJobs jb{};
     int blocks = 0, nj = 0;
@@ -409,8 +412,11 @@
     jb.block0[nj] = blocks;
     jb.njobs = nj;
     if (blocks > 0) {
+      jb.tick = tick;
       hipLaunchKernelGGL(reduce_partials_multi_kernel, dim3((unsigned)blocks), dim3(256), 0, s, jb);
       if (int rc = check_launch("reduce_partials_multi_kernel")) { g_npending = 0; return rc; }
+      if (tick && ticked) *ticked = 1;
+      tick = nullptr;
     }
     done += nj;
   }
@@ -436,6 +442,11 @@
 extern "C" int kgcn_reduce_flush(void* stream) {
   std::lock_guard<std::mutex> lock(g_pending_mutex);
   return flush_pending_locked(as_stream(stream));
+}
+extern "C" int kgcn_reduce_flush_tick(void* stream, int64_t* step_counter, int32_t* ticked) {
+  if (!step_counter || !ticked) return fail("kgcn_reduce_flush_tick: NULL operand");
+  std::lock_guard<std::mutex> lock(g_pending_mutex);
+  return flush_pending_locked(as_stream(stream), reinterpret_cast<long long*>(step_counter), ticked);
 }
 
 struct RowFacts { bool a16; long a_ld; bool b16; long b_ld; };
@@ -872,6 +883,30 @@
                           KGCN_ACT_NONE);
 }
 
+extern "C" int kgcn_dense_skinny_bwd_supported(int64_t m, int32_t din, int32_t dout) {
+  return m > 0 && din > 0 && dout > 0 && skinny_bwd_ok(din, dout) ? 1 : 0;
+}
+
+extern "C" int kgcn_dense_skinny_bwd_f32(const float* x, int64_t x_ld, const float* dy, int64_t dy_ld, int64_t m, int32_t din,
+                                         int32_t dout, const float* w, int64_t w_ld, float* dx, int64_t dx_ld, float* dw,
+                                         float* dbias, void* workspace, int64_t workspace_bytes, void* stream) {
+  if (!kgcn_dense_skinny_bwd_supported(m, din, dout))
+    return fail("kgcn_dense_skinny_bwd_f32: shape m=%lld %d -> %d is not a read-out layer of this route", (long long)m, din, dout);
+  if (!x || !dy || !w || !dx || !dw) return fail("kgcn_dense_skinny_bwd_f32: NULL operand");
+  if (x_ld < din || dy_ld < dout || w_ld < dout || dx_ld < din) return fail("kgcn_dense_skinny_bwd_f32: leading dimension too small");
+  const int64_t need = kgcn_dense_wgrad_workspace_bytes(m, din, dout);
+  if (!workspace || workspace_bytes < need)
+    return fail("kgcn_dense_skinny_bwd_f32: workspace %lld < %lld bytes", (long long)workspace_bytes, (long long)need);
+  hipStream_t s = as_stream(stream);
+  const int np = skinny_wgrad_parts((long)m);
+  float* part_dw = static_cast<float*>(workspace);
+  float* part_db = part_dw + (long)np * din * dout;
+  if (int rc = launch_skinny_n_wgrad(x, (long)m, din, (long)x_ld, dy, (long)dy_ld, dout, part_dw, part_db, np, s, w, (long)w_ld,
+                                     dx, (long)dx_ld))
+    return rc;
+  return launch_reduce_pair(part_dw, (long)din * dout, dw, part_db, dout, dbias, np, s);
+}
+
 extern "C" int kgcn_dense_wgrad_dact_supported(int32_t din, int32_t dout) {
   return fuses_dact(wgrad_route(kManyRows, din, dout, true, aligned_rows(din, dout)).route) ? 1 : 0;
 }
diff --git a/kgcn_amd/csrc/dense_kernels.h b/kgcn_amd/csrc/dense_kernels.h
--- a/kgcn_amd/csrc/dense_kernels.h
+++ b/kgcn_amd/csrc/dense_kernels.h
@@ -56,7 +56,9 @@
 int launch_skinny_k_fwd(const float* x, long m, int din, long x_ld, const float* w, long w_ld, int trans_w, const float* bias,
                         float* y, int dout, long y_ld, int act, hipStream_t s);
 int skinny_wgrad_parts(long m);
+bool skinny_bwd_ok(int din, int dout);
 int launch_skinny_n_wgrad(const float* x, long m, int din, long x_ld, const float* g, long g_ld, int dout, float* part_dw,
-                          float* part_db, int nparts, hipStream_t s);
+                          float* part_db, int nparts, hipStream_t s, const float* w = nullptr, long w_ld = 0, float* dx = nullptr,
+                          long dx_ld = 0);
 
 }
diff --git a/kgcn_amd/csrc/pack.hip b/kgcn_amd/csrc/pack.hip
--- a/kgcn_amd/csrc/pack.hip
+++ b/kgcn_amd/csrc/pack.hip
@@ -147,18 +147,26 @@
   }
   const int c = blockIdx.y, M = p.M[c], row_pad = p.row_pad[c];
   const int* __restrict__ src_rowptr = p.src_rowptr[c];
-  const int* bs = block_sums + c * p.nb;
+  const int* bs = block_sums ? block_sums + c * p.nb : nullptr;
   int* graph_ptr = p.graph_ptr[c];
   int* dst_rowptr = p.dst_rowptr[c];
   int* dst_slots = p.dst_slots[c];
   for (long t = wave0; t < T; t += nwaves) {
     const int g = sel[t];
-    const int b = (int)(t / kScanBlock);
     int off = 0;
-    for (int i = lane; i < b; i += kWave) off += bs[i];
+    if (block_sums) {
+      const int b = (int)(t / kScanBlock);
+      for (int i = lane; i < b; i += kWave) off += bs[i];
+    } else {
+#pragma unroll
+      for (int u = 0; u < kScanBlock / kWave; ++u) {
+        const int i = lane + u * kWave;
+        if (i < t) off += graph_entries(src_rowptr, sel[i], M, row_pad ? 4 * M : 0);
+      }
+    }
 #pragma unroll
     for (int o = kWave / 2; o > 0; o >>= 1) off += __shfl_xor(off, o, kWave);
-    const int out_base = graph_ptr[t] + off;
+    const int out_base = block_sums ? graph_ptr[t] + off : off;
     int* rp_out = dst_rowptr + t * M;
     int cnt;
     if (g >= 0) {
@@ -307,7 +315,9 @@
   if (!workspace || workspace_bytes < need)
     return fail("kgcn_batch_assemble: workspace %lld < %lld bytes", (long long)workspace_bytes, (long long)need);
   int* block_sums = static_cast<int*>(workspace);
-  if (plan->num_csr > 0) {
+  if (num_sel <= kScanBlock) {
+    block_sums = nullptr;
+  } else if (plan->num_csr > 0) {
     hipLaunchKernelGGL(assemble_count_kernel, dim3(p.nb, plan->num_csr), dim3(kScanBlock), 0, s, p, sel, num_sel, block_sums);
     if (int rc = check_launch("assemble_count_kernel")) return rc;
   }
diff --git a/kgcn_amd/csrc/skinny.hip b/kgcn_amd/csrc/skinny.hip
--- a/kgcn_amd/csrc/skinny.hip
+++ b/kgcn_amd/csrc/skinny.hip
@@ -66,14 +66,26 @@
   }
 }
 
-template <int N, int QK>
+template <int N, int QK, bool DX>
 __global__ __launch_bounds__(256) void skinny_n_wgrad_kernel(const float* __restrict__ x, long m, int k, long x_ld,
                                                              const float* __restrict__ g, long g_ld,
-                                                             float* __restrict__ part_dw, float* __restrict__ part_db, int n) {
+                                                             float* __restrict__ part_dw, float* __restrict__ part_db, int n,
+                                                             const float* __restrict__ w, long w_ld, float* __restrict__ dx,
+                                                             long dx_ld) {
   extern __shared__ float red[];
   const int lane = threadIdx.x & 63, wv = threadIdx.x >> 6;
   const long wave = ((long)blockIdx.x * 256 + threadIdx.x) >> 6, nwaves = ((long)gridDim.x * 256) >> 6;
   float acc[QK][N], bs[N];
+  float wr[DX ? QK : 1][DX ? N : 1];
+  (void)wr;
+  if constexpr (DX) {
+#pragma unroll
+    for (int q = 0; q < QK; ++q) {
+      const int c = lane + 64 * q;
+#pragma unroll
+      for (int j = 0; j < N; ++j) wr[q][j] = (c < k && j < n) ? w[(long)c * w_ld + j] : 0.f;
+    }
+  }
 #pragma unroll
   for (int q = 0; q < QK; ++q)
 #pragma unroll
@@ -105,6 +117,24 @@
     }
 #pragma unroll
     for (int j = 0; j < N; ++j) bs[j] += gv[j] + gw[j];
+    if constexpr (DX) {
+#pragma unroll
+      for (int q = 0; q < QK; ++q) {
+        const int c = lane + 64 * q;
+        float sa = 0.f, sb = 0.f;
+#pragma unroll
+        for (int j = 0; j < N; ++j) {
+          if (j < n) {
+            sa = __builtin_fmaf(gv[j], wr[q][j], sa);
+            sb = __builtin_fmaf(gw[j], wr[q][j], sb);
+          }
+        }
+        if (c < k) {
+          dx[r * dx_ld + c] = sa;
+          if (two) dx[r2 * dx_ld + c] = sb;
+        }
+      }
+    }
   }
   float* mine = red + (long)wv * (k * n + n);
 #pragma unroll
@@ -176,15 +206,32 @@
   return (int)(b < 1 ? 1 : b);
 }
 
+bool skinny_bwd_ok(int din, int dout) { return skinny_n_ok(din, dout, 0) && round_qk(din) * round_n(dout) <= 64; }
+
+template <int NN, int QQ>
+static void skinny_wgrad_launch(dim3 grid, size_t lds, hipStream_t s, const float* x, long m, int din, long x_ld, const float* g,
+                                long g_ld, float* part_dw, float* part_db, int dout, const float* w, long w_ld, float* dx,
+                                long dx_ld) {
+  if constexpr (NN * QQ <= 64) {
+    if (w) {
+      hipLaunchKernelGGL((skinny_n_wgrad_kernel<NN, QQ, true>), grid, dim3(256), lds, s, x, m, din, x_ld, g, g_ld, part_dw,
+                         part_db, dout, w, w_ld, dx, dx_ld);
+      return;
+    }
+  }
+  hipLaunchKernelGGL((skinny_n_wgrad_kernel<NN, QQ, false>), grid, dim3(256), lds, s, x, m, din, x_ld, g, g_ld, part_dw, part_db,
+                     dout, (const float*)nullptr, 0L, (float*)nullptr, 0L);
+}
+
 int launch_skinny_n_wgrad(const float* x, long m, int din, long x_ld, const float* g, long g_ld, int dout, float* part_dw,
-                          float* part_db, int nparts, hipStream_t s) {
+                          float* part_db, int nparts, hipStream_t s, const float* w, long w_ld, float* dx, long dx_ld) {
   const dim3 grid(nparts);
   const size_t lds = (size_t)4 * ((size_t)din * dout + dout) * 4;
   const int nn = round_n(dout), qk = round_qk(din);
+  if (w && (!dx || !skinny_bwd_ok(din, dout))) return fail("skinny_n_wgrad: no dX form for %d x %d", din, dout);
 #define KGCN_W(NN, QQ)                                                                                                \
   if (nn == NN && qk == QQ) {                                                                                         \
-    hipLaunchKernelGGL((skinny_n_wgrad_kernel<NN, QQ>), grid, dim3(256), lds, s, x, m, din, x_ld, g, g_ld, part_dw,   \
-                       part_db, dout);                                                                                \
+    skinny_wgrad_launch<NN, QQ>(grid, lds, s, x, m, din, x_ld, g, g_ld, part_dw, part_db, dout, w, w_ld, dx, dx_ld);  \
     return check_launch("skinny_n_wgrad_kernel");                                                                     \
   }
   KGCN_W(2, 1) KGCN_W(2, 2) KGCN_W(2, 4) KGCN_W(2, 8) KGCN_W(2, 16)
diff --git a/kgcn_amd/csrc/train.hip b/kgcn_amd/csrc/train.hip
--- a/kgcn_amd/csrc/train.hip
+++ b/kgcn_amd/csrc/train.hip
@@ -22,7 +22,8 @@
                                                                long B, int T, int weighted, float q,
                                                                const float* __restrict__ qvec, float* __restrict__ cost,
                                                                float* __restrict__ dlogits, float* __restrict__ part,
-                                                               float* __restrict__ sums_direct) {
+                                                               float* __restrict__ sums_direct, float* __restrict__ dmean,
+                                                               float inv_batch) {
   __shared__ float red[kLossBlock];
   const long b = (long)blockIdx.x * kLossBlock + threadIdx.x;
   float c = 0.f;
@@ -43,7 +44,9 @@
         dce = (1.f - z) - lw * (1.f - sg);
       }
       c += ml * ce;
-      dlogits[i] = mk * ml * dce;
+      const float d = mk * ml * dce;
+      dlogits[i] = d;
+      if (dmean) dmean[i] = d * inv_batch;
     }
     c *= mk;
     if (cost) cost[b] = c;
@@ -62,7 +65,8 @@
                                                                const long long* __restrict__ label_idx,
                                                                const float* __restrict__ mask, long B, int C,
                                                                float* __restrict__ cost, float* __restrict__ dlogits,
-                                                               float* __restrict__ part, float* __restrict__ sums_direct) {
+                                                               float* __restrict__ part, float* __restrict__ sums_direct,
+                                                               float* __restrict__ dmean, float inv_batch) {
   __shared__ float red[kLossBlock];
   const long b = (long)blockIdx.x * kLossBlock + threadIdx.x;
   float c = 0.f;
@@ -83,8 +87,11 @@
     const float mk = mask ? mask[b] : 1.f;
     c = mk * (zs * lse - zx);
     const float inv = 1.0f / se;
-    for (int k = 0; k < C; ++k)
-      dlogits[b * C + k] = mk * (__expf(x[k] - mx) * inv * zs - (z ? z[k] : (k == li ? 1.f : 0.f)));
+    for (int k = 0; k < C; ++k) {
+      const float d = mk * (__expf(x[k] - mx) * inv * zs - (z ? z[k] : (k == li ? 1.f : 0.f)));
+      dlogits[b * C + k] = d;
+      if (dmean) dmean[b * C + k] = d * inv_batch;
+    }
     if (cost) cost[b] = c;
   }
   const float s = block_sum_256(c, red);
@@ -123,15 +130,17 @@
   p = __builtin_fmaf(-lr_t, m / (__builtin_sqrtf(v) + eps), p);
 }
 
-__device__ __forceinline__ long long adam_step_of(const long long* counter) { return *counter + 1; }
+__device__ __forceinline__ long long adam_step_of(const long long* counter, int advanced) {
+  return advanced ? *counter : *counter + 1;
+}
 
 template <bool VEC>
 __global__ __launch_bounds__(256) void adam_tf_kernel(float* __restrict__ p, const float* __restrict__ g, float* __restrict__ m,
                                                       float* __restrict__ v, long n, float lr, float b1, float b2, float eps,
-                                                      const long long* __restrict__ counter) {
+                                                      const long long* __restrict__ counter, int advanced) {
   __shared__ float lr_s;
   if (threadIdx.x == 0) {
-    const double t = (double)adam_step_of(counter);
+    const double t = (double)adam_step_of(counter, advanced);
     lr_s = (float)((double)lr * sqrt(1.0 - pow((double)b2, t)) / (1.0 - pow((double)b1, t)));
   }
   __syncthreads();
@@ -182,58 +191,91 @@
   return 0;
 }
 
-extern "C" int kgcn_masked_sigmoid_ce_f32(const float* logits, const float* labels, const float* mask,
-                                          const float* mask_label, int64_t batch, int32_t tasks, int32_t weighted,
-                                          float pos_weight, const float* pos_weight_per_task, float* cost, float* dlogits,
-                                          float* sums, void* workspace, int64_t workspace_bytes, void* stream) {
-  if (int rc = loss_args("kgcn_masked_sigmoid_ce_f32", logits, labels, mask, batch, tasks, dlogits, sums, workspace,
-                         workspace_bytes))
-    return rc;
+static int sigmoid_ce(const char* who, const float* logits, const float* labels, const float* mask, const float* mask_label,
+                      int64_t batch, int32_t tasks, int32_t weighted, float pos_weight, const float* pos_weight_per_task,
+                      float* cost, float* dlogits, float* dmean, float* sums, void* workspace, int64_t workspace_bytes,
+                      void* stream) {
+  if (int rc = loss_args(who, logits, labels, mask, batch, tasks, dlogits, sums, workspace, workspace_bytes)) return rc;
   const int nb = (int)((batch + kLossBlock - 1) / kLossBlock);
   float* part = static_cast<float*>(workspace);
   hipStream_t s = as_stream(stream);
   hipLaunchKernelGGL(sigmoid_ce_kernel, dim3(nb), dim3(kLossBlock), 0, s, logits, labels, mask, mask_label, (long)batch, tasks,
                      weighted ? 1 : 0, pos_weight, weighted ? pos_weight_per_task : nullptr, cost, dlogits, part,
-                     nb == 1 ? sums : nullptr);
+                     nb == 1 ? sums : nullptr, dmean, 1.0f / (float)batch);
   if (int rc = check_launch("sigmoid_ce_kernel")) return rc;
   if (nb == 1) return 0;
   hipLaunchKernelGGL(loss_finish_kernel, dim3(1), dim3(kLossBlock), 0, s, part, nb, (long)batch, sums);
   return check_launch("loss_finish_kernel");
 }
 
-extern "C" int kgcn_masked_softmax_ce_f32(const float* logits, const float* labels, const float* mask, int64_t batch,
-                                          int32_t classes, float* cost, float* dlogits, float* sums, void* workspace,
-                                          int64_t workspace_bytes, void* stream) {
-  if (int rc = loss_args("kgcn_masked_softmax_ce_f32", logits, labels, mask, batch, classes, dlogits, sums, workspace,
-                         workspace_bytes))
+static int softmax_ce(const char* who, bool sparse, const float* logits, const float* labels, const int64_t* label_idx,
+                      const float* mask, int64_t batch, int32_t classes, float* cost, float* dlogits, float* dmean, float* sums, void* workspace,
+                      int64_t workspace_bytes, void* stream) {
+  if (sparse) {
+    if (batch <= 0 || classes <= 0) return fail("%s: bad shape batch=%lld classes=%d", who, (long long)batch, classes);
+    if (!logits || !label_idx || !dlogits || !sums) return fail("%s: NULL operand", who);
+    if (!workspace || workspace_bytes < kgcn_loss_workspace_bytes(batch)) return fail("%s: workspace too small", who);
+  } else if (int rc = loss_args(who, logits, labels, mask, batch, classes, dlogits, sums, workspace, workspace_bytes)) {
     return rc;
+  }
   const int nb = (int)((batch + kLossBlock - 1) / kLossBlock);
   float* part = static_cast<float*>(workspace);
   hipStream_t s = as_stream(stream);
-  hipLaunchKernelGGL(softmax_ce_kernel, dim3(nb), dim3(kLossBlock), 0, s, logits, labels, nullptr, mask, (long)batch, classes,
-                     cost, dlogits, part, nb == 1 ? sums : nullptr);
+  hipLaunchKernelGGL(softmax_ce_kernel, dim3(nb), dim3(kLossBlock), 0, s, logits, labels,
+                     reinterpret_cast<const long long*>(label_idx), mask, (long)batch, classes, cost, dlogits, part,
+                     nb == 1 ? sums : nullptr, dmean, 1.0f / (float)batch);
   if (int rc = check_launch("softmax_ce_kernel")) return rc;
   if (nb == 1) return 0;
   hipLaunchKernelGGL(loss_finish_kernel, dim3(1), dim3(kLossBlock), 0, s, part, nb, (long)batch, sums);
   return check_launch("loss_finish_kernel");
 }
 
+extern "C" int kgcn_masked_sigmoid_ce_f32(const float* logits, const float* labels, const float* mask,
+                                          const float* mask_label, int64_t batch, int32_t tasks, int32_t weighted,
+                                          float pos_weight, const float* pos_weight_per_task, float* cost, float* dlogits,
+                                          float* sums, void* workspace, int64_t workspace_bytes, void* stream) {
+  return sigmoid_ce("kgcn_masked_sigmoid_ce_f32", logits, labels, mask, mask_label, batch, tasks, weighted, pos_weight,
+                    pos_weight_per_task, cost, dlogits, nullptr, sums, workspace, workspace_bytes, stream);
+}
+
+extern "C" int kgcn_masked_softmax_ce_f32(const float* logits, const float* labels, const float* mask, int64_t batch,
+                                          int32_t classes, float* cost, float* dlogits, float* sums, void* workspace,
+                                          int64_t workspace_bytes, void* stream) {
+  return softmax_ce("kgcn_masked_softmax_ce_f32", false, logits, labels, nullptr, mask, batch, classes, cost, dlogits, nullptr, sums,
+                    workspace, workspace_bytes, stream);
+}
+
 extern "C" int kgcn_sparse_softmax_ce_f32(const float* logits, const int64_t* label_idx, const float* mask, int64_t batch,
                                           int32_t classes, float* cost, float* dlogits, float* sums, void* workspace,
                                           int64_t workspace_bytes, void* stream) {
-  if (batch <= 0 || classes <= 0) return fail("kgcn_sparse_softmax_ce_f32: bad shape batch=%lld classes=%d", (long long)batch, classes);
-  if (!logits || !label_idx || !dlogits || !sums) return fail("kgcn_sparse_softmax_ce_f32: NULL operand");
-  if (!workspace || workspace_bytes < kgcn_loss_workspace_bytes(batch)) return fail("kgcn_sparse_softmax_ce_f32: workspace too small");
-  const int nb = (int)((batch + kLossBlock - 1) / kLossBlock);
-  float* part = static_cast<float*>(workspace);
-  hipStream_t s = as_stream(stream);
-  hipLaunchKernelGGL(softmax_ce_kernel, dim3(nb), dim3(kLossBlock), 0, s, logits, nullptr,
-                     reinterpret_cast<const long long*>(label_idx), mask, (long)batch, classes, cost, dlogits, part,
-                     nb == 1 ? sums : nullptr);
-  if (int rc = check_launch("softmax_ce_kernel")) return rc;
-  if (nb == 1) return 0;
-  hipLaunchKernelGGL(loss_finish_kernel, dim3(1), dim3(kLossBlock), 0, s, part, nb, (long)batch, sums);
-  return check_launch("loss_finish_kernel");
+  return softmax_ce("kgcn_sparse_softmax_ce_f32", true, logits, nullptr, label_idx, mask, batch, classes, cost, dlogits, nullptr, sums,
+                    workspace, workspace_bytes, stream);
+}
+
+extern "C" int kgcn_masked_sigmoid_ce_mean_f32(const float* logits, const float* labels, const float* mask,
+                                               const float* mask_label, int64_t batch, int32_t tasks, int32_t weighted,
+                                               float pos_weight, const float* pos_weight_per_task, float* cost, float* dlogits,
+                                               float* dlogits_mean, float* sums, void* workspace, int64_t workspace_bytes,
+                                               void* stream) {
+  if (!dlogits_mean) return fail("kgcn_masked_sigmoid_ce_mean_f32: NULL operand");
+  return sigmoid_ce("kgcn_masked_sigmoid_ce_mean_f32", logits, labels, mask, mask_label, batch, tasks, weighted, pos_weight,
+                    pos_weight_per_task, cost, dlogits, dlogits_mean, sums, workspace, workspace_bytes, stream);
+}
+
+extern "C" int kgcn_masked_softmax_ce_mean_f32(const float* logits, const float* labels, const float* mask, int64_t batch,
+                                               int32_t classes, float* cost, float* dlogits, float* dlogits_mean, float* sums,
+                                               void* workspace, int64_t workspace_bytes, void* stream) {
+  if (!dlogits_mean) return fail("kgcn_masked_softmax_ce_mean_f32: NULL operand");
+  return softmax_ce("kgcn_masked_softmax_ce_mean_f32", false, logits, labels, nullptr, mask, batch, classes, cost, dlogits, dlogits_mean,
+                    sums, workspace, workspace_bytes, stream);
+}
+
+extern "C" int kgcn_sparse_softmax_ce_mean_f32(const float* logits, const int64_t* label_idx, const float* mask, int64_t batch,
+                                               int32_t classes, float* cost, float* dlogits, float* dlogits_mean, float* sums,
+                                               void* workspace, int64_t workspace_bytes, void* stream) {
+  if (!dlogits_mean) return fail("kgcn_sparse_softmax_ce_mean_f32: NULL operand");
+  return softmax_ce("kgcn_sparse_softmax_ce_mean_f32", true, logits, nullptr, label_idx, mask, batch, classes, cost, dlogits,
+                    dlogits_mean, sums, workspace, workspace_bytes, stream);
 }
 
 extern "C" int kgcn_loss_grad_f32(const float* dlogits, const float* g_opt, const float* g_sum, int64_t batch, int64_t n,
@@ -255,10 +297,10 @@
 
 __global__ __launch_bounds__(256) void adam_tf_multi_kernel(float* __restrict__ p, float* __restrict__ m, float* __restrict__ v,
                                                             AdamSegs sg, float lr, float b1, float b2, float eps,
-                                                            const long long* __restrict__ counter) {
+                                                            const long long* __restrict__ counter, int advanced) {
   __shared__ float lr_s;
   if (threadIdx.x == 0) {
-    const double t = (double)adam_step_of(counter);
+    const double t = (double)adam_step_of(counter, advanced);
     lr_s = (float)((double)lr * sqrt(1.0 - pow((double)b2, t)) / (1.0 - pow((double)b1, t)));
   }
   __syncthreads();
@@ -274,9 +316,8 @@
   }
 }
 
-extern "C" int kgcn_adam_tf_multi_f32(float* params, float* m, float* v, int64_t n, const kgcn_adam_segment* segments,
-                                      int32_t num_segments, float lr, float beta1, float beta2, float eps, int64_t* step_counter,
-                                      void* stream) {
+static int adam_tf_multi(float* params, float* m, float* v, int64_t n, const kgcn_adam_segment* segments, int32_t num_segments,
+                         float lr, float beta1, float beta2, float eps, int64_t* step_counter, bool ticked, void* stream) {
   if (n < 0 || num_segments < 0) return fail("kgcn_adam_tf_multi_f32: negative size");
   if (!step_counter) return fail("kgcn_adam_tf_multi_f32: step_counter is NULL");
   if (num_segments > 0 && (!params || !m || !v || !segments)) return fail("kgcn_adam_tf_multi_f32: NULL operand");
@@ -296,15 +337,29 @@
     long blocks = (most + 255) / 256;
     if (blocks > 2L * kNumCU) blocks = 2L * kNumCU;
     hipLaunchKernelGGL(adam_tf_multi_kernel, dim3((unsigned)blocks, cnt), dim3(256), 0, s, params, m, v, sg, lr, beta1, beta2, eps,
-                       reinterpret_cast<const long long*>(step_counter));
+                       reinterpret_cast<const long long*>(step_counter), ticked ? 1 : 0);
     if (int rc = check_launch("adam_tf_multi_kernel")) return rc;
   }
+  if (ticked) return 0;
   hipLaunchKernelGGL(adam_tick_kernel, dim3(1), dim3(1), 0, s, reinterpret_cast<long long*>(step_counter));
   return check_launch("adam_tick_kernel");
 }
 
-extern "C" int kgcn_adam_tf_f32(float* params, const float* grads, float* m, float* v, int64_t n, float lr, float beta1,
-                                float beta2, float eps, int64_t* step_counter, void* stream) {
+extern "C" int kgcn_adam_tf_multi_f32(float* params, float* m, float* v, int64_t n, const kgcn_adam_segment* segments,
+                                      int32_t num_segments, float lr, float beta1, float beta2, float eps, int64_t* step_counter,
+                                      void* stream) {
+  return adam_tf_multi(params, m, v, n, segments, num_segments, lr, beta1, beta2, eps, step_counter, false, stream);
+}
+
+extern "C" int kgcn_adam_tf_multi_ticked_f32(float* params, float* m, float* v, int64_t n, const kgcn_adam_segment* segments,
+                                             int32_t num_segments, float lr, float beta1, float beta2, float eps,
+                                             const int64_t* step_counter, void* stream) {
+  return adam_tf_multi(params, m, v, n, segments, num_segments, lr, beta1, beta2, eps, const_cast<int64_t*>(step_counter), true,
+                       stream);
+}
+
+static int adam_tf(float* params, const float* grads, float* m, float* v, int64_t n, float lr, float beta1, float beta2,
+                   float eps, int64_t* step_counter, bool ticked, void* stream) {
   if (n < 0) return fail("kgcn_adam_tf_f32: n < 0");
   if (!step_counter) return fail("kgcn_adam_tf_f32: step_counter is NULL");
   hipStream_t s = as_stream(stream);
@@ -317,12 +372,23 @@
     const long long* ctr = reinterpret_cast<const long long*>(step_counter);
     if (vec)
       hipLaunchKernelGGL(adam_tf_kernel<true>, dim3((unsigned)blocks), dim3(256), 0, s, params, grads, m, v, (long)n, lr,
-                         beta1, beta2, eps, ctr);
+                         beta1, beta2, eps, ctr, ticked ? 1 : 0);
     else
       hipLaunchKernelGGL(adam_tf_kernel<false>, dim3((unsigned)blocks), dim3(256), 0, s, params, grads, m, v, (long)n, lr,
-                         beta1, beta2, eps, ctr);
+                         beta1, beta2, eps, ctr, ticked ? 1 : 0);
     if (int rc = check_launch("adam_tf_kernel")) return rc;
   }
+  if (ticked) return 0;
   hipLaunchKernelGGL(adam_tick_kernel, dim3(1), dim3(1), 0, s, reinterpret_cast<long long*>(step_counter));
   return check_launch("adam_tick_kernel");
 }
+
+extern "C" int kgcn_adam_tf_f32(float* params, const float* grads, float* m, float* v, int64_t n, float lr, float beta1,
+                                float beta2, float eps, int64_t* step_counter, void* stream) {
+  return adam_tf(params, grads, m, v, n, lr, beta1, beta2, eps, step_counter, false, stream);
+}
+
+extern "C" int kgcn_adam_tf_ticked_f32(float* params, const float* grads, float* m, float* v, int64_t n, float lr, float beta1,
+                                       float beta2, float eps, const int64_t* step_counter, void* stream) {
+  return adam_tf(params, grads, m, v, n, lr, beta1, beta2, eps, const_cast<int64_t*>(step_counter), true, stream);
+}
diff --git a/kgcn_amd/ops.py b/kgcn_amd/ops.py
--- a/kgcn_amd/ops.py
+++ b/kgcn_amd/ops.py
@@ -28,22 +28,26 @@
 
 class deferred_reductions:
 
-    def __init__(self, root=None):
-        self.root = root
+    def __init__(self, root=None, unit_seed=False, tick=None):
+        self.root, self.unit_seed, self.tick = root, bool(unit_seed), tick
 
     def __enter__(self):
+        global _unit_seed_node
         _no_defer_params.clear()
         if self.root is not None:
             _no_defer_params.update(_readers_inside_backward(self.root))
+        _unit_seed_node = self.root.grad_fn if self.unit_seed and torch.is_tensor(self.root) else None
         self.prev = lib.kgcn_reduce_defer(1)
         return self
 
     def __exit__(self, *exc):
+        global _unit_seed_node
         try:
-            flush_reductions()
+            flush_reductions(tick=self.tick if exc[0] is None else None)
         finally:
             lib.kgcn_reduce_defer(self.prev)
             _no_defer_params.clear()
+            _unit_seed_node = None
         return False
 
 
@@ -73,9 +77,31 @@
     return out
 
 
-def flush_reductions():
-    check(lib.kgcn_reduce_flush(current_stream()), "kgcn_reduce_flush")
+_unit_seed_node = None
+_ticked = set()
+
+
+def _unit_seeded(ctx, out_index, root_index):
+    return _unit_seed_node is ctx and out_index == root_index
+
+
+def flush_reductions(tick=None):
+    if tick is None:
+        check(lib.kgcn_reduce_flush(current_stream()), "kgcn_reduce_flush")
+    else:
+        done = ctypes.c_int32(0)
+        check(lib.kgcn_reduce_flush_tick(current_stream(), ptr(tick), ctypes.byref(done)), "kgcn_reduce_flush_tick")
+        if done.value:
+            _ticked.add(tick.data_ptr())
     _deferred_keep.clear()
+
+
+def take_tick(counter):
+    key = counter.data_ptr()
+    if key in _ticked:
+        _ticked.discard(key)
+        return True
+    return False
 
 
 _param_uses = {}
@@ -616,6 +642,16 @@
                 _dense_bwd_fused_ok(x2d, w, gy, yact if ctx.act else None):
             dx, dw, db = _dense_bwd_fused(ctx, x2d, w, gy, yact, ctx.act, need_b)
             return dx, dw, db, None
+        if not ctx.act and ctx.needs_input_grad[0] and ctx.needs_input_grad[1] and \
+                not (side_stream_wgrad and m >= side_wgrad_min_rows) and lib.kgcn_dense_skinny_bwd_supported(m, din, dout):
+            dx = torch.empty_like(x2d)
+            dw = torch.empty_like(w)
+            db = torch.empty((dout,), device=gy.device, dtype=torch.float32) if need_b else None
+            wsb = lib.kgcn_dense_wgrad_workspace_bytes(m, din, dout)
+            with _param_grad_stage(ctx, wsb, gy.device) as wsp:
+                check(lib.kgcn_dense_skinny_bwd_f32(ptr(x2d), din, ptr(gy), dout, m, din, dout, ptr(w), dout, ptr(dx), din, ptr(dw),
+                                                    ptr(db), ptr(wsp), wsb, current_stream()), "kgcn_dense_skinny_bwd_f32")
+            return dx, dw, None if db is None else db.reshape(ctx.bias_shape), None
         fuse_dact = bool(ctx.act) and not ctx.needs_input_grad[0] and wgrad_dact_fusion and \
             bool(lib.kgcn_dense_wgrad_dact_supported(din, dout))
         if ctx.act and ctx.needs_input_grad[0]:
@@ -1443,25 +1479,39 @@
         if tuple(z.shape) != (B, W) or mk.numel() != B or (ml is not None and tuple(ml.shape) != (B, W)):
             raise _lib.KgcnHipError("labels / mask / mask_label do not match logits %s" % (tuple(x.shape),))
         dlog = torch.empty_like(x)
+        dmean = torch.empty_like(x) if ctx.needs_input_grad[0] else None
         sums = torch.empty((2,), device=x.device, dtype=torch.float32)
         wsb = lib.kgcn_loss_workspace_bytes(B)
         ws = _lib.workspace(wsb, x.device)
         if kind == "sigmoid":
             qs, qv = _pos_weight_operand(pos_weight, W, x.device)
-            check(lib.kgcn_masked_sigmoid_ce_f32(ptr(x), ptr(z), ptr(mk), ptr(ml), B, W, 0 if pos_weight is None else 1,
-                                                 qs, ptr(qv), None, ptr(dlog), ptr(sums), ptr(ws), wsb, current_stream()),
-                  "kgcn_masked_sigmoid_ce_f32")
-        else:
+            wt = 0 if pos_weight is None else 1
+            if dmean is None:
+                check(lib.kgcn_masked_sigmoid_ce_f32(ptr(x), ptr(z), ptr(mk), ptr(ml), B, W, wt, qs, ptr(qv), None, ptr(dlog),
+                                                     ptr(sums), ptr(ws), wsb, current_stream()), "kgcn_masked_sigmoid_ce_f32")
+            else:
+                check(lib.kgcn_masked_sigmoid_ce_mean_f32(ptr(x), ptr(z), ptr(mk), ptr(ml), B, W, wt, qs, ptr(qv), None,
+                                                          ptr(dlog), ptr(dmean), ptr(sums), ptr(ws), wsb, current_stream()),
+                      "kgcn_masked_sigmoid_ce_mean_f32")
+        elif dmean is None:
             check(lib.kgcn_masked_softmax_ce_f32(ptr(x), ptr(z), ptr(mk), B, W, None, ptr(dlog), ptr(sums), ptr(ws), wsb,
                                                  current_stream()), "kgcn_masked_softmax_ce_f32")
-        ctx.save_for_backward(dlog)
+        else:
+            check(lib.kgcn_masked_softmax_ce_mean_f32(ptr(x), ptr(z), ptr(mk), B, W, None, ptr(dlog), ptr(dmean), ptr(sums),
+                                                      ptr(ws), wsb, current_stream()), "kgcn_masked_softmax_ce_mean_f32")
+        if dmean is None:
+            ctx.save_for_backward(dlog)
+        else:
+            ctx.save_for_backward(dlog, dmean)
         ctx.batch = B
         ctx.set_materialize_grads(False)
         return sums[1], sums[0]
 
     @staticmethod
     def backward(ctx, g_opt, g_sum):
-        (dlog,) = ctx.saved_tensors
+        dlog = ctx.saved_tensors[0]
+        if g_sum is None and g_opt is not None and len(ctx.saved_tensors) == 2 and _unit_seeded(ctx, 0, 0):
+            return ctx.saved_tensors[1], None, None, None, None, None
         return _loss_grad(dlog, g_opt, g_sum, ctx.batch), None, None, None, None, None
 
 
@@ -1486,6 +1536,8 @@
     @staticmethod
     def backward(ctx, g):
         (dlog,) = ctx.saved_tensors
+        if g is not None and _unit_seeded(ctx, 0, 0):
+            return dlog, None
         return _loss_grad(dlog, None, g, 1), None
 
 
diff --git a/kgcn_amd/train.py b/kgcn_amd/train.py
--- a/kgcn_amd/train.py
+++ b/kgcn_amd/train.py
@@ -71,6 +71,9 @@
         from . import ops
         ops.weight_tables.invalidate()
         self.t += 1
+        ticked = ops.take_tick(self._t_dev)
+        multi, flat = ((_lib.lib.kgcn_adam_tf_multi_ticked_f32, _lib.lib.kgcn_adam_tf_ticked_f32) if ticked else
+                       (_lib.lib.kgcn_adam_tf_multi_f32, _lib.lib.kgcn_adam_tf_f32))
         if not packed:
             import ctypes
             ops.join_side_streams()
@@ -84,15 +87,15 @@
                     g = g.to(torch.float32).contiguous()
                     keep.append(g)
                 segs[i] = _lib.AdamSegment(g.data_ptr(), o, p.numel())
-            _lib.check(_lib.lib.kgcn_adam_tf_multi_f32(_lib.ptr(self.flat.data), _lib.ptr(self._m), _lib.ptr(self._v),
-                                                       self.flat.total, ctypes.cast(segs, ctypes.c_void_p), len(self.params),
-                                                       float(self.lr), float(self.b1), float(self.b2), float(self.eps),
-                                                       _lib.ptr(self._t_dev), _lib.current_stream()), "kgcn_adam_tf_multi_f32")
+            _lib.check(multi(_lib.ptr(self.flat.data), _lib.ptr(self._m), _lib.ptr(self._v), self.flat.total,
+                             ctypes.cast(segs, ctypes.c_void_p), len(self.params), float(self.lr), float(self.b1),
+                             float(self.b2), float(self.eps), _lib.ptr(self._t_dev), _lib.current_stream()),
+                       "kgcn_adam_tf_multi_ticked_f32" if ticked else "kgcn_adam_tf_multi_f32")
             return
-        _lib.check(_lib.lib.kgcn_adam_tf_f32(_lib.ptr(self.flat.data), _lib.ptr(self.flat.grad), _lib.ptr(self._m),
-                                             _lib.ptr(self._v), self.flat.total, float(self.lr), float(self.b1),
-                                             float(self.b2), float(self.eps), _lib.ptr(self._t_dev), _lib.current_stream()),
-                   "kgcn_adam_tf_f32")
+        _lib.check(flat(_lib.ptr(self.flat.data), _lib.ptr(self.flat.grad), _lib.ptr(self._m), _lib.ptr(self._v),
+                        self.flat.total, float(self.lr), float(self.b1), float(self.b2), float(self.eps),
+                        _lib.ptr(self._t_dev), _lib.current_stream()),
+                   "kgcn_adam_tf_ticked_f32" if ticked else "kgcn_adam_tf_f32")
 
 
 def _exchange(bucket, optimizer, shard_weight):
@@ -110,7 +113,7 @@
     ops.weight_tables.refresh()
     logits = model(features, adjs, **fwd_kwargs)
     cost_opt, cost_sum = loss_fn(logits, labels, mask)
-    with ops.deferred_reductions(root=cost_opt):
+    with ops.deferred_reductions(root=cost_opt, unit_seed=True, tick=getattr(optimizer, "_t_dev", None)):
         cost_opt.backward()
     optimizer.step(packed=_exchange(bucket, optimizer, shard_weight))
     return float(cost_sum.detach()), logits.detach()
@@ -170,7 +173,7 @@
         cost_opt, cost_sum = self.loss_fn(logits, self.labels, self.mask)
         if self._seed is None or self._seed.shape != cost_opt.shape:
             self._seed = torch.ones_like(cost_opt)
-        with ops.deferred_reductions(root=cost_opt):
+        with ops.deferred_reductions(root=cost_opt, unit_seed=True, tick=self.opt._t_dev):
             cost_opt.backward(self._seed)
         self.opt.step(packed=_exchange(self.bucket, self.opt, self.shard_weight))
         self.cost_sum, self.logits = cost_sum.detach(), logits.detach()
```

Result: no change. 130.2 million (-0.0%).
